# jqsl2012/RL_CTR_Prediction

Measured on NVIDIA B200. Metric: train samples/sec, higher is better.
Workload: dtype f32

## Files before the change

### include/rlctr.h

```cpp
#ifndef RLCTR_H_
#define RLCTR_H_

#include <stddef.h>
#include <stdint.h>

#ifdef __cplusplus
extern "C" {
#endif

#define RLCTR_VERSION 100

#define RLCTR_OK            0
#define RLCTR_EINVAL       (-1)
#define RLCTR_EUNSUPPORTED (-2)
#define RLCTR_EWORKSPACE   (-3)
#define RLCTR_EALIGN       (-4)

typedef struct CUstream_st* rlctr_stream_t;

#define RLCTR_MAX_WORLD 8
typedef struct rlctr_table {
    float*  data;
    int64_t n_rows;
    int32_t row_stride;
// ... 16 lines not shown
    double         beta1, beta2, eps, weight_decay;
    const float*   stage;
} rlctr_adam;

typedef struct rlctr_lookup {
    float*   stage;
    int32_t  world;
    uint32_t n_per_rank;
    float*   gathered[RLCTR_MAX_WORLD];
} rlctr_lookup;

#define RLCTR_STAGED_PARTNER 1
#define RLCTR_DZ_IN_SUMS     2
typedef struct rlctr_rowgrad {
    const float* staged;
    const float* dlogit;
    const float* sums;
    const float* extra;
    int32_t      fields;
    int32_t      flags;
    int32_t      world;
    uint32_t     n_per_rank;
    const float* peer_staged[RLCTR_MAX_WORLD];
    const float* peer_dlogit[RLCTR_MAX_WORLD];
    const float* peer_sums[RLCTR_MAX_WORLD];
    const float* peer_extra[RLCTR_MAX_WORLD];
} rlctr_rowgrad;

int         rlctr_version(void);
unsigned long long rlctr_launch_count(void);
const char* rlctr_strerror(int code);

#define RLCTR_FM_TERM 1
int rlctr_embed_fwd(const int64_t* ids, const rlctr_table* table, const float* bias,
                    float* logit, float* pctr, int64_t pctr_stride, float* sums, float* rows_out,
                    int64_t rows_pitch, int64_t batch, int32_t fields, int32_t flags, rlctr_stream_t stream);

int rlctr_pairdots_fwd(const float* rows, int64_t ld_rows, float* out, int64_t ld_out, int64_t batch,
                       int32_t fields, int32_t dim, int32_t ip_first, rlctr_stream_t stream);
int rlctr_pairdots_bwd(const float* rows, int64_t ld_rows, const float* gout, int64_t ld_g, float* grows,
                       int64_t ld_grows, int64_t batch, int32_t fields, int32_t dim, int32_t ip_first,
                       rlctr_stream_t stream);

size_t rlctr_cross_ws_bytes(int64_t batch, int32_t dim, int32_t layers);
int rlctr_cross_fwd(const float* x0, int64_t ldx, const float* w, const float* b, int32_t layers, float* out, int64_t ld_out,
                    float* s_saved, int64_t batch, int32_t dim, rlctr_stream_t stream);
int rlctr_cross_bwd(const float* x0, int64_t ldx, const float* w, const float* b, const float* s_saved, int32_t layers,
                    const float* gout, int64_t ld_g, float* gx0, int64_t ld_gx, float* dw, float* db, int64_t batch,
                    int32_t dim, void* ws, size_t ws_bytes, rlctr_stream_t stream);

int rlctr_fieldsq_fwd(const float* rows, int64_t ld_rows, float* out, int64_t ld_out, int64_t batch, int32_t fields,
                      int32_t dim, rlctr_stream_t stream);
int rlctr_fieldsq_bwd(const float* rows, int64_t ld_rows, const float* gout, int64_t ld_g, float* grows, int64_t ld_grows,
                      int64_t batch, int32_t fields, int32_t dim, rlctr_stream_t stream);

size_t rlctr_afm_ws_bytes(int64_t batch, int32_t dim);
int rlctr_afm_fwd(const float* rows, int64_t ld_rows, const float* params, float* out, int64_t batch, int32_t fields,
                  int32_t dim, float dropout_p, const uint64_t* rng_state, const float* masks, rlctr_stream_t stream);
int rlctr_afm_bwd(const float* rows, int64_t ld_rows, const float* params, const float* gout, float* grows, int64_t ld_grows,
                  float* dparams, int64_t batch, int32_t fields, int32_t dim, float dropout_p, const uint64_t* rng_state,
                  const float* masks, void* ws, size_t ws_bytes, rlctr_stream_t stream);

int rlctr_gather_rows(const int64_t* ids, int64_t n, const rlctr_table* table, float* out,
                      rlctr_stream_t stream);

int rlctr_ffm_fwd(const int64_t* ids, const rlctr_table* table, const float* bias,
                  float* logit, float* pctr, int64_t pctr_stride, float* partners,
                  int64_t batch, int32_t fields, int32_t latent, rlctr_stream_t stream);

int rlctr_featemb_fwd(const int64_t* ids, const rlctr_table* table, float* out, int64_t out_stride,
                      int64_t batch, int32_t fields, rlctr_stream_t stream);

int rlctr_bn_relu_fwd(const float* x, int64_t ldx, const float* gamma, const float* beta, float* running_mean, float* running_var,
                      float momentum, float eps, float* y, int64_t ldy, float* save_mean, float* save_invstd, int64_t batch,
                      int32_t n, int32_t relu, rlctr_stream_t stream);
int rlctr_bn_relu_bwd(const float* x, int64_t ldx, const float* y, int64_t ldy, const float* gy, int64_t ldg, const float* gamma,
                      const float* save_mean, const float* save_invstd, float* dx, int64_t lddx, float* dgamma, float* dbeta,
                      int64_t batch, int32_t n, int32_t relu, rlctr_stream_t stream);

#define RLCTR_REDUCE_WS_BYTES 16640
int rlctr_bce_fwd_bwd(const float* logit, const int64_t* labels_i64, const float* labels_f32,
                      float* pctr, float* loss, float* dlogit, float* dbias, void* ws, int64_t batch,
                      rlctr_stream_t stream);
int rlctr_sigmoid_bwd(const float* grad_p, const float* pctr, float* dlogit, float* dbias, void* ws,
                      int64_t batch, rlctr_stream_t stream);

size_t rlctr_sort_ws_bytes(int64_t n, int64_t n_rows);
int rlctr_sort_ids(const int64_t* ids, int64_t n, int64_t n_rows,
                   uint32_t* sorted_ids, uint32_t* sorted_slots,
                   void* ws, size_t ws_bytes, rlctr_stream_t stream);

size_t rlctr_rows_ws_bytes(int64_t n);
int rlctr_sort_ids_sharded(const uint32_t* ids_all, int64_t n_all, int32_t world, int32_t rank, int64_t n_rows_global,
                           uint32_t* sorted_rows, uint32_t* sorted_slots, void* ws, size_t ws_bytes,
                           rlctr_stream_t stream);

int rlctr_push_rows(const int64_t* ids, int64_t n, int32_t world, int32_t rank, int64_t n_rows_global, const float* src,
                    int32_t width, void* const* peer_recv, rlctr_stream_t stream);
size_t rlctr_route_ws_bytes(int64_t n, int32_t world);
int rlctr_route_ids(const int64_t* ids, int64_t n, int32_t world, int32_t rank, int64_t n_rows_global, int64_t cap,
                    void* const* peer_keys, void* const* peer_vals, int32_t* overflow, void* ws, size_t ws_bytes,
                    rlctr_stream_t stream);
int rlctr_sort_routed(const uint32_t* keys, const uint32_t* vals, int64_t n_in, int64_t n_rows_local, uint32_t* sorted_rows,
                      uint32_t* sorted_slots, void* ws, size_t ws_bytes, rlctr_stream_t stream);
int rlctr_sort_routed_pos(const uint32_t* keys, int64_t n_in, int64_t n_rows_local, uint32_t* sorted_rows, uint32_t* sorted_pos,
                          void* ws, size_t ws_bytes, rlctr_stream_t stream);
int rlctr_push_rows_routed(const void* route_ws, int64_t n, int32_t world, int32_t rank, int64_t cap, const float* src,
                           int32_t width, void* const* peer_recv, rlctr_stream_t stream);
int rlctr_rows_adam(const uint32_t* sorted_ids, const uint32_t* sorted_slots, int64_t n,
                    const rlctr_rowgrad* grad, const rlctr_table* table, const rlctr_adam* opt,
                    void* ws, size_t ws_bytes, rlctr_stream_t stream);
#define RLCTR_GROUP_MAX 4
typedef struct rlctr_member {
    int32_t      lin_col;
    int32_t      emb_col;
    int32_t      dim;
    int32_t      flags;
    const float* bias;
    float*       logit;
    float*       pctr;
    int64_t      pctr_stride;
    float*       rows_out;
    int64_t      rows_pitch;
    const float* dlogit;
    const float* extra;
} rlctr_member;
int rlctr_group_fwd(const int64_t* ids, const rlctr_table* table, const rlctr_member* members, int32_t n_members,
                    float* sums, int32_t sums_pitch, int64_t batch, int32_t fields, rlctr_stream_t stream);
int rlctr_group_rows_adam(const uint32_t* sorted_ids, const uint32_t* sorted_slots, int64_t n, const rlctr_table* table,
                          const rlctr_adam* opt, const rlctr_member* members, int32_t n_members, const float* sums,
                          int32_t sums_pitch, int32_t fields, int32_t world, const uint32_t* slot_of, void* ws, size_t ws_bytes,
                          rlctr_stream_t stream);

int rlctr_rows_grad_dense(const uint32_t* sorted_ids, const uint32_t* sorted_slots, int64_t n,
                          const rlctr_rowgrad* grad, const rlctr_table* table, float* dense_grad,
                          void* ws, size_t ws_bytes, rlctr_stream_t stream);
int64_t rlctr_lookup_stage_floats(const rlctr_table* table);
int rlctr_rows_lookup(const uint32_t* sorted_ids, const uint32_t* sorted_slots, int64_t n, const rlctr_table* table,
                      const rlctr_adam* opt, const rlctr_lookup* lookup, void* ws, size_t ws_bytes, rlctr_stream_t stream);
int rlctr_rows_catchup(const uint32_t* sorted_ids, int64_t n, const rlctr_table* table,
                       const rlctr_adam* opt, rlctr_stream_t stream);
size_t rlctr_rows_claim_bytes(int64_t n_rows);
int rlctr_rows_catchup_ids(const int64_t* ids, int64_t n, const rlctr_table* table, const rlctr_adam* opt, void* claim,
                           size_t claim_bytes, rlctr_stream_t stream);
int rlctr_adam_flush(const rlctr_table* table, const rlctr_adam* opt,
                     int64_t row_begin, int64_t row_end, rlctr_stream_t stream);
int rlctr_dense_adam(float* param, const float* grad, float* exp_avg, float* exp_avg_sq, int64_t n,
                     const float* sched, const int32_t* step, double beta1, double beta2, double eps,
                     double weight_decay, rlctr_stream_t stream);
#define RLCTR_DENSE_MAX 24
int rlctr_dense_adam_multi(float* const* params, const float* const* grads, float* const* exp_avgs, float* const* exp_avg_sqs,
                           const int64_t* sizes, int32_t count, const float* sched, const int32_t* steps,
                           const int32_t* step_index, double beta1, double beta2, double eps, double weight_decay,
                           rlctr_stream_t stream);
int rlctr_steps_advance(int32_t* steps, const int32_t* step_index, int32_t count, rlctr_stream_t stream);
int rlctr_step_advance(int32_t* step, int32_t delta, rlctr_stream_t stream);

int rlctr_generate_preds(const float* pctr, const float* w, const int64_t* action, const int64_t* label,
                         float* y, float* w_out, float* reward, int64_t batch, int32_t models,
                         int32_t variant, rlctr_stream_t stream);
size_t rlctr_generate_preds_v10_ws_bytes(int64_t batch);
int rlctr_generate_preds_v10(const float* pctr, const float* w, const float* c_actions, const int64_t* action,
                             const int64_t* label, float* y, float* c_out, float* reward, int64_t batch, int32_t models,
                             void* ws, size_t ws_bytes, rlctr_stream_t stream);

int rlctr_reinforce_loss_bwd(const float* logits, const int64_t* act, const float* vt,
                             float* logp, float* loss, float* dlogits, void* ws,
                             int64_t batch, int32_t actions, int32_t variant, rlctr_stream_t stream);

size_t rlctr_auc_ws_bytes(int64_t n);
int rlctr_auc_logloss(const float* pred, const int64_t* labels_i64, const float* labels_f32, int64_t n, float* out,
                      void* ws, size_t ws_bytes, rlctr_stream_t stream);

#define RLCTR_MLP_RELU 1
#define RLCTR_MLP_DROPOUT 2
#define RLCTR_MLP_DX_MASK 4
#define RLCTR_MLP_FP32 8
#define RLCTR_MLP_W_PRESPLIT 16
size_t rlctr_mlp_ws_bytes(int64_t batch, int32_t in_dim, int32_t out_dim);
int rlctr_replay_store(float* memory, int64_t memory_size, int32_t width, int64_t counter, const float* src, int64_t n,
                       int64_t ld_src, rlctr_stream_t stream);
int rlctr_replay_gather(const float* memory, int32_t width, const int64_t* idx, int64_t n, float* out, rlctr_stream_t stream);
int rlctr_replay_update(float* priorities, int32_t ld, const int64_t* idx, const float* td, int64_t n, rlctr_stream_t stream);
int rlctr_replay_sample_uniform(int64_t n_valid, int64_t batch, const uint64_t* rng_state, int64_t* out_idx, rlctr_stream_t stream);
size_t rlctr_replay_per_ws_bytes(int64_t n_valid);
int rlctr_replay_sample_per(const float* priorities, int32_t ld, int64_t n_valid, float eps, float alpha, float beta, int32_t greedy,
                            int64_t batch, const uint64_t* rng_state, int64_t* out_idx, float* out_isw, void* ws, size_t ws_bytes,
                            rlctr_stream_t stream);

size_t rlctr_gae_ws_bytes(int64_t n);
int rlctr_gae_scan(const float* deltas, int64_t n, double gamma_lambda, float* advantages, void* ws, size_t ws_bytes,
                   rlctr_stream_t stream);

int rlctr_rng_advance(uint64_t* rng_state, uint64_t delta, rlctr_stream_t stream);
int rlctr_linear_fwd(const float* x, int64_t ldx, const float* w, const float* bias, float* y, int64_t batch,
                     int32_t in_dim, int32_t out_dim, int32_t flags, float dropout_p, const uint64_t* rng_state,
                     void* ws, size_t ws_bytes, rlctr_stream_t stream);
int rlctr_linear_bwd(const float* x, int64_t ldx, const float* w, const float* y, float* gy, float* dx, float* dw,
                     float* db, int64_t batch, int32_t in_dim, int32_t out_dim, int32_t flags, float gy_scale,
                     float dx_scale, void* ws, size_t ws_bytes, rlctr_stream_t stream);

size_t rlctr_bucket_ws_bytes(int64_t n, int32_t world);
int rlctr_bucket_by_owner(const int64_t* ids, int64_t n, int32_t world, int64_t n_rows, int64_t* send_local,
                          int64_t* pos_of_slot, uint32_t* send_slots, int64_t* bucket_ends, void* ws,
                          size_t ws_bytes, rlctr_stream_t stream);

#ifdef __cplusplus
}
#endif
#endif
```

### rl_ctr_prediction_b200/_lib.py

```python
from __future__ import annotations

import ctypes as C
import os

import torch

_PKG = os.path.dirname(os.path.abspath(__file__))
LIB_PATH = os.path.join(_PKG, "librlctr_sm100a.so")

RLCTR_FM_TERM = 1
RLCTR_STAGED_PARTNER = 1
RLCTR_DZ_IN_SUMS = 2
RLCTR_REDUCE_WS_BYTES = 16640
RLCTR_DENSE_MAX = 24
RLCTR_MLP_RELU = 1
RLCTR_MLP_DROPOUT = 2
RLCTR_MLP_DX_MASK = 4
RLCTR_MLP_W_PRESPLIT = 16
RLCTR_MLP_FP32 = 8


class RlctrError(RuntimeError):
    pass


class Table(C.Structure):
    _fields_ = [("data", C.c_void_p), ("n_rows", C.c_int64), ("row_stride", C.c_int32),
                ("lin_col", C.c_int32), ("emb_col", C.c_int32), ("dim", C.c_int32), ("row_pitch", C.c_int32),
                ("world", C.c_int32), ("peers", C.c_void_p * 8)]


class Adam(C.Structure):
    _fields_ = [("exp_avg", C.c_void_p), ("exp_avg_sq", C.c_void_p), ("stamp", C.c_void_p),
                ("sched", C.c_void_p), ("step", C.c_void_p), ("sched_len", C.c_int32), ("stamp_col", C.c_int32),
                ("beta1", C.c_double), ("beta2", C.c_double), ("eps", C.c_double), ("weight_decay", C.c_double),
                ("stage", C.c_void_p)]


class Lookup(C.Structure):
    _fields_ = [("stage", C.c_void_p), ("world", C.c_int32), ("n_per_rank", C.c_uint32), ("gathered", C.c_void_p * 8)]


class RowGrad(C.Structure):
    _fields_ = [("staged", C.c_void_p), ("dlogit", C.c_void_p), ("sums", C.c_void_p),
                ("extra", C.c_void_p), ("fields", C.c_int32), ("flags", C.c_int32),
                ("world", C.c_int32), ("n_per_rank", C.c_uint32), ("peer_staged", C.c_void_p * 8),
                ("peer_dlogit", C.c_void_p * 8), ("peer_sums", C.c_void_p * 8), ("peer_extra", C.c_void_p * 8)]


class Member(C.Structure):
    _fields_ = [("lin_col", C.c_int32), ("emb_col", C.c_int32), ("dim", C.c_int32), ("flags", C.c_int32),
                ("bias", C.c_void_p), ("logit", C.c_void_p), ("pctr", C.c_void_p), ("pctr_stride", C.c_int64),
                ("rows_out", C.c_void_p), ("rows_pitch", C.c_int64), ("dlogit", C.c_void_p), ("extra", C.c_void_p)]


RLCTR_GROUP_MAX = 4

_P, _I64, _I32, _SZ, _F = C.c_void_p, C.c_int64, C.c_int32, C.c_size_t, C.c_double
_TP, _AP, _GP, _LP = C.POINTER(Table), C.POINTER(Adam), C.POINTER(RowGrad), C.POINTER(Lookup)
_MP = C.POINTER(Member)

SIGNATURES = {
    "rlctr_version": (C.c_int, []),
    "rlctr_strerror": (C.c_char_p, [C.c_int]),
    "rlctr_launch_count": (C.c_ulonglong, []),
    "rlctr_embed_fwd": (C.c_int, [_P, _TP, _P, _P, _P, _I64, _P, _P, _I64, _I64, _I32, _I32, _P]),
    "rlctr_pairdots_fwd": (C.c_int, [_P, _I64, _P, _I64, _I64, _I32, _I32, _I32, _P]),
    "rlctr_pairdots_bwd": (C.c_int, [_P, _I64, _P, _I64, _P, _I64, _I64, _I32, _I32, _I32, _P]),
    "rlctr_cross_ws_bytes": (_SZ, [_I64, _I32, _I32]),
    "rlctr_cross_fwd": (C.c_int, [_P, _I64, _P, _P, _I32, _P, _I64, _P, _I64, _I32, _P]),
    "rlctr_cross_bwd": (C.c_int, [_P, _I64, _P, _P, _P, _I32, _P, _I64, _P, _I64, _P, _P, _I64, _I32, _P, _SZ, _P]),
    "rlctr_fieldsq_fwd": (C.c_int, [_P, _I64, _P, _I64, _I64, _I32, _I32, _P]),
    "rlctr_fieldsq_bwd": (C.c_int, [_P, _I64, _P, _I64, _P, _I64, _I64, _I32, _I32, _P]),
    "rlctr_afm_ws_bytes": (_SZ, [_I64, _I32]),
    "rlctr_afm_fwd": (C.c_int, [_P, _I64, _P, _P, _I64, _I32, _I32, C.c_float, _P, _P, _P]),
    "rlctr_afm_bwd": (C.c_int, [_P, _I64, _P, _P, _P, _I64, _P, _I64, _I32, _I32, C.c_float, _P, _P, _P, _SZ, _P]),
    "rlctr_replay_store": (C.c_int, [_P, _I64, _I32, _I64, _P, _I64, _I64, _P]),
    "rlctr_replay_gather": (C.c_int, [_P, _I32, _P, _I64, _P, _P]),
    "rlctr_replay_update": (C.c_int, [_P, _I32, _P, _P, _I64, _P]),
    "rlctr_replay_sample_uniform": (C.c_int, [_I64, _I64, _P, _P, _P]),
    "rlctr_replay_per_ws_bytes": (_SZ, [_I64]),
    "rlctr_replay_sample_per": (C.c_int, [_P, _I32, _I64, C.c_float, C.c_float, C.c_float, _I32, _I64, _P, _P, _P, _P, _SZ, _P]),
    "rlctr_push_rows": (C.c_int, [_P, _I64, _I32, _I32, _I64, _P, _I32, _P, _P]),
    "rlctr_gae_ws_bytes": (_SZ, [_I64]),
    "rlctr_gae_scan": (C.c_int, [_P, _I64, _F, _P, _P, _SZ, _P]),
    "rlctr_gather_rows": (C.c_int, [_P, _I64, _TP, _P, _P]),
    "rlctr_ffm_fwd": (C.c_int, [_P, _TP, _P, _P, _P, _I64, _P, _I64, _I32, _I32, _P]),
    "rlctr_featemb_fwd": (C.c_int, [_P, _TP, _P, _I64, _I64, _I32, _P]),
    "rlctr_bn_relu_fwd": (C.c_int, [_P, _I64, _P, _P, _P, _P, C.c_float, C.c_float, _P, _I64, _P, _P, _I64, _I32, _I32, _P]),
    "rlctr_bn_relu_bwd": (C.c_int, [_P, _I64, _P, _I64, _P, _I64, _P, _P, _P, _P, _I64, _P, _P, _I64, _I32, _I32, _P]),
    "rlctr_bce_fwd_bwd": (C.c_int, [_P, _P, _P, _P, _P, _P, _P, _P, _I64, _P]),
    "rlctr_sigmoid_bwd": (C.c_int, [_P, _P, _P, _P, _P, _I64, _P]),
    "rlctr_sort_ws_bytes": (_SZ, [_I64, _I64]),
    "rlctr_sort_ids": (C.c_int, [_P, _I64, _I64, _P, _P, _P, _SZ, _P]),
    "rlctr_sort_ids_sharded": (C.c_int, [_P, _I64, _I32, _I32, _I64, _P, _P, _P, _SZ, _P]),
    "rlctr_route_ws_bytes": (_SZ, [_I64, _I32]),
    "rlctr_route_ids": (C.c_int, [_P, _I64, _I32, _I32, _I64, _I64, _P, _P, _P, _P, _SZ, _P]),
    "rlctr_sort_routed": (C.c_int, [_P, _P, _I64, _I64, _P, _P, _P, _SZ, _P]),
    "rlctr_rows_ws_bytes": (_SZ, [_I64]),
    "rlctr_rows_adam": (C.c_int, [_P, _P, _I64, _GP, _TP, _AP, _P, _SZ, _P]),
    "rlctr_group_fwd": (C.c_int, [_P, _TP, _MP, _I32, _P, _I32, _I64, _I32, _P]),
    "rlctr_group_rows_adam": (C.c_int, [_P, _P, _I64, _TP, _AP, _MP, _I32, _P, _I32, _I32, _I32, _P, _P, _SZ, _P]),
    "rlctr_sort_routed_pos": (C.c_int, [_P, _I64, _I64, _P, _P, _P, _SZ, _P]),
    "rlctr_push_rows_routed": (C.c_int, [_P, _I64, _I32, _I32, _I64, _P, _I32, _P, _P]),
    "rlctr_rows_grad_dense": (C.c_int, [_P, _P, _I64, _GP, _TP, _P, _P, _SZ, _P]),
    "rlctr_lookup_stage_floats": (_I64, [_TP]),
    "rlctr_rows_lookup": (C.c_int, [_P, _P, _I64, _TP, _AP, _LP, _P, _SZ, _P]),
    "rlctr_rows_catchup": (C.c_int, [_P, _I64, _TP, _AP, _P]),
    "rlctr_rows_claim_bytes": (_SZ, [_I64]),
    "rlctr_rows_catchup_ids": (C.c_int, [_P, _I64, _TP, _AP, _P, _SZ, _P]),
    "rlctr_adam_flush": (C.c_int, [_TP, _AP, _I64, _I64, _P]),
    "rlctr_dense_adam": (C.c_int, [_P, _P, _P, _P, _I64, _P, _P, _F, _F, _F, _F, _P]),
    "rlctr_dense_adam_multi": (C.c_int, [_P, _P, _P, _P, _P, _I32, _P, _P, _P, _F, _F, _F, _F, _P]),
    "rlctr_steps_advance": (C.c_int, [_P, _P, _I32, _P]),
    "rlctr_step_advance": (C.c_int, [_P, _I32, _P]),
    "rlctr_generate_preds": (C.c_int, [_P, _P, _P, _P, _P, _P, _P, _I64, _I32, _I32, _P]),
    "rlctr_generate_preds_v10_ws_bytes": (_SZ, [_I64]),
    "rlctr_generate_preds_v10": (C.c_int, [_P, _P, _P, _P, _P, _P, _P, _P, _I64, _I32, _P, _SZ, _P]),
    "rlctr_reinforce_loss_bwd": (C.c_int, [_P, _P, _P, _P, _P, _P, _P, _I64, _I32, _I32, _P]),
    "rlctr_auc_ws_bytes": (_SZ, [_I64]),
    "rlctr_auc_logloss": (C.c_int, [_P, _P, _P, _I64, _P, _P, _SZ, _P]),
    "rlctr_mlp_ws_bytes": (_SZ, [_I64, _I32, _I32]),
    "rlctr_rng_advance": (C.c_int, [_P, C.c_uint64, _P]),
    "rlctr_linear_fwd": (C.c_int, [_P, _I64, _P, _P, _P, _I64, _I32, _I32, _I32, C.c_float, _P, _P, _SZ, _P]),
    "rlctr_linear_bwd": (C.c_int, [_P, _I64, _P, _P, _P, _P, _P, _P, _I64, _I32, _I32, _I32, C.c_float, C.c_float, _P, _SZ, _P]),
    "rlctr_bucket_ws_bytes": (_SZ, [_I64, _I32]),
    "rlctr_bucket_by_owner": (C.c_int, [_P, _I64, _I32, _I64, _P, _P, _P, _P, _P, _SZ, _P]),
}

_lib = None


def load() -> C.CDLL:
    global _lib
    if _lib is not None:
        return _lib
    if not os.path.exists(LIB_PATH):
        raise RlctrError(
            f"{LIB_PATH} is missing: build it with `python -m rl_ctr_prediction_b200.build` "
            "(nvcc, sm_100a). There is no fallback path.")
    lib = C.CDLL(LIB_PATH)
    for name, (res, args) in SIGNATURES.items():
        fn = getattr(lib, name)
        fn.restype = res
        fn.argtypes = args
    _lib = lib
    return lib


def check(code: int, what: str) -> None:
    if code != 0:
        msg = load().rlctr_strerror(code).decode()
        raise RlctrError(f"{what} failed: {msg} (code {code})")


def ptr(t):
    if t is None:
        return None
    if not t.is_cuda:
        raise RlctrError("rlctr kernels need CUDA tensors (sm_100a); there is no CPU fallback")
    if not t.is_contiguous():
        raise RlctrError("rlctr kernels need contiguous tensors")
    return t.data_ptr()


def stream():
    return torch.cuda.current_stream().cuda_stream


class KernelTimer:

    def __init__(self):
        self.records = {}

    def add(self, key, e0, e1, meta):
        self.records.setdefault(key, []).append((e0, e1, meta))

    def summary(self, alg_fn=None):
        torch.cuda.synchronize()
        out = {}
        for key, recs in self.records.items():
            ms = [a.elapsed_time(b) for a, b, _ in recs]
            alg = 0.0
            if alg_fn is not None:
                alg = sum(alg_fn(key, m) for _, _, m in recs) / len(recs)
            out[key] = (len(recs), sum(ms) / len(ms), alg)
        return out


_timer = None


def set_timer(t):
    global _timer
    _timer = t


def timing() -> bool:
    return _timer is not None


def call(name, fn, *args, key=None, meta=None):
    t = _timer
    if t is None:
        check(fn(*args), name)
        return
    e0, e1 = torch.cuda.Event(enable_timing=True), torch.cuda.Event(enable_timing=True)
    e0.record()
# ... 5 lines not shown
```

### rl_ctr_prediction_b200/colocated.py

```python
from __future__ import annotations

import ctypes as C
import os

import torch
import torch.nn as nn

from . import _lib
from . import p_model as Model
from .tables import Geometry, round4, table_struct


MEMBER_KINDS = (Model.LR, Model.FM, Model.DeepFM, Model.WideAndDeep, Model.FNN, Model.InnerPNN, Model.OuterPNN, Model.DCN,
                Model.AFM)


UNSORTED_CATCHUP = os.environ.get("RLCTR_GROUP_UNSORTED_CATCHUP", "0") != "0"


class GroupStash:
    __slots__ = ("sorted_ids", "sorted_slots", "n", "fields", "sums", "dlogit", "extra")

    def __init__(self, **kw):
        for k in self.__slots__:
# ... 98 lines not shown
        arr = (_lib.Member * len(self.members))()
        logits, rows = [], []
        for i, (m, (lin, emb, dim)) in enumerate(zip(self.members, self._cols)):
            s = arr[i]
            s.lin_col, s.emb_col, s.dim = lin, emb, dim
            s.flags = _lib.RLCTR_FM_TERM if m._fm_term else 0
            bias = getattr(m, "bias", None)
            s.bias = _lib.ptr(bias.data) if bias is not None else None
            tail = hasattr(m, "_tail")
            table_part = lin >= 0 or bias is not None or m._fm_term
            z = torch.empty(B, dtype=torch.float32, device=dev) if table_part and (train or tail) else None
            logits.append(z)
            s.logit = _lib.ptr(z)
            if pctr is not None and not tail:
                s.pctr, s.pctr_stride = pctr.data_ptr() + 4 * i, pctr.shape[1]
            r = None
            if tail:
                pitch = round4(F * dim)
                r = torch.empty(B, pitch, dtype=torch.float32, device=dev)
                s.rows_out, s.rows_pitch = r.data_ptr(), pitch
            rows.append(r)
        return arr, logits, rows

    @torch.no_grad()
    def forward(self, x):
        lib = _lib.load()
        x = Model._check_ids(x)
        B, F = x.shape
        self.flush()
        out = torch.empty(B, len(self.members), dtype=torch.float32, device=x.device)
        arr, logits, rows = self._member_structs(B, F, x.device, False, pctr=out)
        t = table_struct(self.table.data, self._geom)
        _lib.call("rlctr_group_fwd", lib.rlctr_group_fwd, _lib.ptr(x), C.byref(t), arr, len(self.members), None, 0, B, F,
                  _lib.stream(), key="rlctr_group_fwd[infer]", meta=self._meta(B, F))
        for i, m in enumerate(self.members):
            if rows[i] is not None:
                out[:, i:i + 1] = torch.sigmoid(m._tail(self._z(logits[i], B), rows[i][:, :F * self._cols[i][2]]))
        return out

    @staticmethod
    def _z(logit, B):
        return logit.view(B, 1) if logit is not None else None

    def train_step(self, x, y, optimizer):
        lib = _lib.load()
        opt = self._opt
        if opt is None:
            raise _lib.RlctrError("build rl_ctr_prediction_b200.optim.Adam(group.parameters(), ...) before training the group")
        x = Model._check_ids(x)
        B, F = x.shape
        dev, st, g = x.device, _lib.stream(), self._geom
        yy = y.reshape(-1).contiguous()
        yi = yy if yy.dtype == torch.int64 else None
        yf = None if yi is not None else yy.float()
        t = table_struct(self.table.data, g)
        side = None
        if UNSORTED_CATCHUP and opt.lazy and opt.stamp_col >= 0 and (g.used + 3) // 4 >= 5:
            cur = torch.cuda.current_stream(dev)
            side = self._sort_stream
            if side is None or side.device != dev:
                side = self._sort_stream = torch.cuda.Stream(device=dev)
            side.wait_stream(cur)
            with torch.cuda.stream(side):
                sid, sslot = Model.sort_ids(x, g.n_rows)
            if opt.dirty:
                a = opt.struct()
                cb = lib.rlctr_rows_claim_bytes(g.n_rows)
                if self._claim is None or self._claim.numel() < cb or self._claim.device != dev:
                    self._claim = torch.empty(cb, dtype=torch.uint8, device=dev)
                _lib.call("rlctr_rows_catchup_ids", lib.rlctr_rows_catchup_ids, _lib.ptr(x), x.numel(), C.byref(t), C.byref(a),
                          _lib.ptr(self._claim), cb, st, key="rlctr_rows_catchup[group]", meta=self._meta(B, F))
        else:
            sid, sslot = Model.sort_ids(x, g.n_rows)
            if opt.lazy and opt.dirty:
                a = opt.struct()
                _lib.call("rlctr_rows_catchup", lib.rlctr_rows_catchup, _lib.ptr(sid), x.numel(), C.byref(t), C.byref(a), st,
                          key="rlctr_rows_catchup[group]", meta=self._meta(B, F))
        M = len(self.members)
        arr, logits, rows = self._member_structs(B, F, dev, True)
        sums = torch.empty(B, g.row_stride, dtype=torch.float32, device=dev)
        _lib.call("rlctr_group_fwd", lib.rlctr_group_fwd, _lib.ptr(x), C.byref(t), arr, M, _lib.ptr(sums), 0, B, F, st,
                  key="rlctr_group_fwd[train]", meta=self._meta(B, F))
        losses = torch.empty(M, dtype=torch.float32, device=dev)
        dlogits, extras = [], []
        ws = self._reduce_ws(dev)
        for i, m in enumerate(self.members):
            dl = torch.empty(B, dtype=torch.float32, device=dev)
            dbias = torch.empty(1, dtype=torch.float32, device=dev)
            bias = getattr(m, "bias", None)
            if rows[i] is None:
                _lib.check(lib.rlctr_bce_fwd_bwd(_lib.ptr(logits[i]), _lib.ptr(yi), _lib.ptr(yf), None,
                                                 losses.data_ptr() + 4 * i, _lib.ptr(dl), _lib.ptr(dbias), _lib.ptr(ws), B, st),
                           "rlctr_bce_fwd_bwd")
                extras.append(None)
            else:
                fd = F * self._cols[i][2]
                leaf = rows[i][:, :fd].detach().requires_grad_(True)
                z = m._tail(self._z(logits[i], B), leaf)
                zz = z.detach().reshape(-1).contiguous()
                _lib.check(lib.rlctr_bce_fwd_bwd(_lib.ptr(zz), _lib.ptr(yi), _lib.ptr(yf), None, losses.data_ptr() + 4 * i,
                                                 _lib.ptr(dl), _lib.ptr(dbias) if bias is not None else None, _lib.ptr(ws), B, st),
                           "rlctr_bce_fwd_bwd")
                m.zero_grad()
                z.backward(dl.view_as(z))
                extras.append(leaf.grad.contiguous())
            if bias is not None:
                bias.grad = dbias
            dlogits.append(dl)
        self._stash = GroupStash(sorted_ids=sid, sorted_slots=sslot, n=B * F, fields=F, sums=sums, dlogit=dlogits, extra=extras)
        if side is not None:
            torch.cuda.current_stream(dev).wait_stream(side)
        optimizer.step()
        return losses

    def _group_update(self, stash, opt_state, st):
        lib = _lib.load()
        arr = (_lib.Member * len(self.members))()
        for i, (m, (lin, emb, dim)) in enumerate(zip(self.members, self._cols)):
            s = arr[i]
            s.lin_col, s.emb_col, s.dim = lin, emb, dim
            s.flags = _lib.RLCTR_FM_TERM if m._fm_term else 0
            s.dlogit = _lib.ptr(stash.dlogit[i])
            s.extra = _lib.ptr(stash.extra[i])
        t, a = table_struct(self.table.data, self._geom), opt_state.struct()
        ws_bytes = lib.rlctr_rows_ws_bytes(stash.n)
        ws = self._rows_ws(ws_bytes)
        _lib.call("rlctr_group_rows_adam", lib.rlctr_group_rows_adam, _lib.ptr(stash.sorted_ids), _lib.ptr(stash.sorted_slots),
                  stash.n, C.byref(t), C.byref(a), arr, len(self.members), _lib.ptr(stash.sums), 0, stash.fields, 1, None,
                  _lib.ptr(ws), ws_bytes, st, key="rlctr_group_rows_adam", meta=self._meta(stash.n // stash.fields, stash.fields))


def colocate(models) -> ColocatedCTR:
    return ColocatedCTR(models)
```

### rl_ctr_prediction_b200/csrc/loss.cu

```cuda
#include "common.cuh"

namespace rlctr {

constexpr int RED_MAX_BLOCKS = 1024;
struct RedWs {
    unsigned int* counter;
    float* partial;
};
__host__ __device__ inline RedWs red_ws(void* ws) {
    return RedWs{reinterpret_cast<unsigned int*>(ws), reinterpret_cast<float*>(reinterpret_cast<char*>(ws) + 256)};
}

__device__ __forceinline__ float block_sum_256(float x, float* smem8) {
#pragma unroll
    for (int off = 16; off > 0; off >>= 1) x += __shfl_xor_sync(RLCTR_FULL, x, off);
    __syncthreads();
    if ((threadIdx.x & 31) == 0) smem8[threadIdx.x >> 5] = x;
    __syncthreads();
    float t = 0.f;
    if (threadIdx.x < 8) t = smem8[threadIdx.x];
    if (threadIdx.x < 32) {
#pragma unroll
        for (int off = 4; off > 0; off >>= 1) t += __shfl_xor_sync(RLCTR_FULL, t, off);
    }
    return t;
}

__device__ __forceinline__ bool last_block_arrives(unsigned int* counter) {
    __shared__ bool is_last;
    __threadfence();
    __syncthreads();
    if (threadIdx.x == 0) is_last = (atomicAdd(counter, 1u) == gridDim.x - 1);
    __syncthreads();
    return is_last;
}

__global__ void __launch_bounds__(256)
bce_kernel(const float* __restrict__ logit, const int64_t* __restrict__ yi, const float* __restrict__ yf,
           float* __restrict__ pctr, float* __restrict__ loss, float* __restrict__ dlogit, float* __restrict__ dbias,
           void* ws, int64_t batch) {
    __shared__ float sm[8];
    const float ginv = 1.0f / (float)batch;
    float acc = 0.f, dsum = 0.f;
    for (int64_t b = (int64_t)blockIdx.x * blockDim.x + threadIdx.x; b < batch; b += (int64_t)gridDim.x * blockDim.x) {
        const float z = __ldg(logit + b);
        const float y = yi ? (float)__ldg(yi + b) : __ldg(yf + b);
        const float p = sigmoidf_ref(z);
        acc += (y - 1.0f) * fmaxf(log1pf(-p), -100.0f) - y * fmaxf(logf(p), -100.0f);
        const float dp = ginv * (p - y) / fmaxf((1.0f - p) * p, 1e-12f);
        const float dz = dp * (1.0f - p) * p;
        if (pctr) pctr[b] = p;
        if (dlogit) dlogit[b] = dz;
        dsum += dz;
    }
    RedWs w = red_ws(ws);
    const float bs = block_sum_256(acc, sm), ds = block_sum_256(dsum, sm);
    if (threadIdx.x == 0) { w.partial[blockIdx.x] = bs; w.partial[RED_MAX_BLOCKS + blockIdx.x] = ds; }
    if (last_block_arrives(w.counter)) {
        float t = 0.f, d = 0.f;
        for (int i = threadIdx.x; i < (int)gridDim.x; i += 256) {
            t += __ldcg(w.partial + i);
            d += __ldcg(w.partial + RED_MAX_BLOCKS + i);
        }
        t = block_sum_256(t, sm);
        d = block_sum_256(d, sm);
        if (threadIdx.x == 0) {
            if (loss) loss[0] = t / (float)batch;
            if (dbias) dbias[0] = d;
            *w.counter = 0;
        }
    }
}

__global__ void __launch_bounds__(256)
sigmoid_bwd_kernel(const float* __restrict__ grad_p, const float* __restrict__ pctr, float* __restrict__ dlogit,
                   float* __restrict__ dbias, void* ws, int64_t batch) {
    __shared__ float sm[8];
    float dsum = 0.f;
    for (int64_t b = (int64_t)blockIdx.x * blockDim.x + threadIdx.x; b < batch; b += (int64_t)gridDim.x * blockDim.x) {
        float dz;
        if (grad_p) {
            const float p = __ldg(pctr + b);
            dz = __ldg(grad_p + b) * (1.0f - p) * p;
            dlogit[b] = dz;
        } else {
            dz = dlogit[b];
        }
        dsum += dz;
    }
    if (!dbias) return;
    RedWs w = red_ws(ws);
    const float ds = block_sum_256(dsum, sm);
    if (threadIdx.x == 0) w.partial[blockIdx.x] = ds;
    if (last_block_arrives(w.counter)) {
        float d = 0.f;
        for (int i = threadIdx.x; i < (int)gridDim.x; i += 256) d += __ldcg(w.partial + i);
        d = block_sum_256(d, sm);
        if (threadIdx.x == 0) { dbias[0] = d; *w.counter = 0; }
    }
}

constexpr int GP_MAX = 8;

__global__ void __launch_bounds__(256)
generate_preds_kernel(const float* __restrict__ pctr, const float* __restrict__ w, const int64_t* __restrict__ action,
                      const int64_t* __restrict__ label, float* __restrict__ y, float* __restrict__ w_out,
                      float* __restrict__ reward, int64_t batch, int M, int variant) {
    const int64_t b = (int64_t)blockIdx.x * blockDim.x + threadIdx.x;
    if (b >= batch) return;
    float p[GP_MAX], wt[GP_MAX], ow[GP_MAX], sw[GP_MAX], sp[GP_MAX];
    int si[GP_MAX];
#pragma unroll
    for (int m = 0; m < GP_MAX; ++m) {
        p[m] = m < M ? __ldg(pctr + b * M + m) : 0.f;
        wt[m] = m < M ? __ldg(w + b * M + m) : -INFINITY;
        ow[m] = 0.f;
        sw[m] = wt[m]; sp[m] = p[m]; si[m] = m;
    }
#pragma unroll
    for (int i = 1; i < GP_MAX; ++i) {
#pragma unroll
        for (int j = i; j > 0; --j) {
            if (sw[j] > sw[j - 1]) {
                float tw = sw[j]; sw[j] = sw[j - 1]; sw[j - 1] = tw;
                float tp = sp[j]; sp[j] = sp[j - 1]; sp[j - 1] = tp;
                int ti = si[j]; si[j] = si[j - 1]; si[j - 1] = ti;
            }
        }
    }
    const int k = (int)__ldg(action + b);
    const int lab = (int)__ldg(label + b);
    float psum = 0.f;
#pragma unroll
    for (int m = 0; m < GP_MAX; ++m) if (m < M) psum += p[m];
    const float mean_all = psum / (float)M;
    const int k_lo = variant == 0 ? 2 : 1;
    float yv = 1.0f, rv = 1.0f;
    if (k >= k_lo && k <= M) {
        float base;
        if (k == M) {
            float acc = 0.f;
#pragma unroll
            for (int m = 0; m < GP_MAX; ++m) if (m < M) { acc += wt[m] * p[m]; ow[m] = wt[m]; }
            yv = acc;
            base = mean_all;
        } else if (k == 1) {
            yv = sp[0];
#pragma unroll
            for (int m = 0; m < GP_MAX; ++m) if (si[0] == m) ow[m] = 1.0f;
            base = mean_all;
        } else {
            float e[GP_MAX], esum = 0.f;
#pragma unroll
            for (int j = 0; j < GP_MAX; ++j) { e[j] = j < k ? expf(sw[j] - sw[0]) : 0.f; esum += e[j]; }
// ... 140 lines not shown
            yv = acc;
        }
        const bool good = lab == 1 ? (yv > mean_all) : (yv < mean_all);
        rv = good ? 1.0f : 0.0f;
    }
    y[b] = yv;
    reward[b] = rv;
#pragma unroll
    for (int m = 0; m < GP_MAX; ++m) if (m < M) c_out[b * M + m] = oc[m];
}

constexpr int RF_MAX = 32;

__global__ void __launch_bounds__(256)
reinforce_fwd_kernel(const float* __restrict__ logits, const int64_t* __restrict__ act, const float* __restrict__ vt,
                     float* __restrict__ logp, float* __restrict__ loss, void* ws, int64_t batch, int A, int variant) {
    __shared__ float sm[8];
    float s_nl = 0.f, s_vt = 0.f, s_nlvt = 0.f;
    for (int64_t b = (int64_t)blockIdx.x * blockDim.x + threadIdx.x; b < batch; b += (int64_t)gridDim.x * blockDim.x) {
        const float* z = logits + b * A;
        float mx = -INFINITY;
        for (int a = 0; a < A; ++a) mx = fmaxf(mx, __ldg(z + a));
        float sum = 0.f;
        for (int a = 0; a < A; ++a) sum += expf(__ldg(z + a) - mx);
        const int ai = (int)__ldg(act + b) - 1;
        const float pa = expf(__ldg(z + ai) - mx) / sum;
        const float lp = logf(pa);
        const float v = __ldg(vt + b);
        if (logp) logp[b] = lp;
        s_nl += -lp; s_vt += v; s_nlvt += -lp * v;
    }
    RedWs w = red_ws(ws);
    float r0 = block_sum_256(s_nl, sm), r1 = block_sum_256(s_vt, sm), r2 = block_sum_256(s_nlvt, sm);
    if (threadIdx.x == 0) {
        w.partial[blockIdx.x] = r0;
        w.partial[RED_MAX_BLOCKS + blockIdx.x] = r1;
        w.partial[2 * RED_MAX_BLOCKS + blockIdx.x] = r2;
    }
    if (last_block_arrives(w.counter)) {
        float t0 = 0.f, t1 = 0.f, t2 = 0.f;
        for (int i = threadIdx.x; i < (int)gridDim.x; i += 256) {
            t0 += __ldcg(w.partial + i);
            t1 += __ldcg(w.partial + RED_MAX_BLOCKS + i);
            t2 += __ldcg(w.partial + 2 * RED_MAX_BLOCKS + i);
        }
        t0 = block_sum_256(t0, sm); t1 = block_sum_256(t1, sm); t2 = block_sum_256(t2, sm);
        if (threadIdx.x == 0) {
            const float mean_vt = t1 / (float)batch;
            if (loss) loss[0] = variant == 0 ? t0 * mean_vt : t2 / (float)batch;
            w.partial[3 * RED_MAX_BLOCKS] = mean_vt;
            *w.counter = 0;
        }
    }
}
__global__ void __launch_bounds__(256)
reinforce_bwd_kernel(const float* __restrict__ logits, const int64_t* __restrict__ act, const float* __restrict__ vt,
                     float* __restrict__ dlogits, const void* ws, int64_t batch, int A, int variant) {
    const float mean_vt = __ldcg(reinterpret_cast<const float*>(reinterpret_cast<const char*>(ws) + 256) + 3 * RED_MAX_BLOCKS);
    for (int64_t b = (int64_t)blockIdx.x * blockDim.x + threadIdx.x; b < batch; b += (int64_t)gridDim.x * blockDim.x) {
        const float* z = logits + b * A;
        float mx = -INFINITY;
        for (int a = 0; a < A; ++a) mx = fmaxf(mx, __ldg(z + a));
        float sum = 0.f;
        for (int a = 0; a < A; ++a) sum += expf(__ldg(z + a) - mx);
        const int ai = (int)__ldg(act + b) - 1;
        const float coef = variant == 0 ? mean_vt : __ldg(vt + b) / (float)batch;
        for (int a = 0; a < A; ++a) {
            const float pi = expf(__ldg(z + a) - mx) / sum;
            dlogits[b * A + a] = coef * (pi - (a == ai ? 1.0f : 0.0f));
        }
    }
}

static inline int red_grid(int64_t batch) {
    int64_t blocks = (batch + 255) / 256;
    if (blocks < 1) blocks = 1;
    return (int)(blocks < RED_MAX_BLOCKS ? blocks : RED_MAX_BLOCKS);
}

}

using namespace rlctr;

extern "C" int rlctr_bce_fwd_bwd(const float* logit, const int64_t* labels_i64, const float* labels_f32, float* pctr,
                                 float* loss, float* dlogit, float* dbias, void* ws, int64_t batch,
                                 rlctr_stream_t stream) {
    if (!logit || !ws || batch <= 0) return RLCTR_EINVAL;
    if ((labels_i64 == nullptr) == (labels_f32 == nullptr)) return RLCTR_EINVAL;
    bce_kernel<<<red_grid(batch), 256, 0, (cudaStream_t)stream>>>(logit, labels_i64, labels_f32, pctr, loss, dlogit,
                                                                  dbias, ws, batch);
    RLCTR_LAUNCH_CHECK();
    return RLCTR_OK;
}

extern "C" int rlctr_sigmoid_bwd(const float* grad_p, const float* pctr, float* dlogit, float* dbias, void* ws,
                                 int64_t batch, rlctr_stream_t stream) {
    if (!dlogit || batch <= 0 || (grad_p && !pctr) || (dbias && !ws)) return RLCTR_EINVAL;
    sigmoid_bwd_kernel<<<red_grid(batch), 256, 0, (cudaStream_t)stream>>>(grad_p, pctr, dlogit, dbias, ws, batch);
    RLCTR_LAUNCH_CHECK();
    return RLCTR_OK;
}

extern "C" int rlctr_generate_preds(const float* pctr, const float* w, const int64_t* action, const int64_t* label,
                                    float* y, float* w_out, float* reward, int64_t batch, int32_t models,
                                    int32_t variant, rlctr_stream_t stream) {
    if (!pctr || !w || !action || !label || !y || !reward || batch < 0) return RLCTR_EINVAL;
    if (models < 1 || models > GP_MAX || (variant != 0 && variant != 1)) return RLCTR_EUNSUPPORTED;
    if (batch == 0) return RLCTR_OK;
    generate_preds_kernel<<<(unsigned)((batch + 255) / 256), 256, 0, (cudaStream_t)stream>>>(
        pctr, w, action, label, y, w_out, reward, batch, models, variant);
    RLCTR_LAUNCH_CHECK();
    return RLCTR_OK;
}

extern "C" size_t rlctr_generate_preds_v10_ws_bytes(int64_t batch) {
    if (batch < 0) return 0;
    return (size_t)((batch + GP10_THREADS - 1) / GP10_THREADS + 1) * GP_MAX * sizeof(int);
}
extern "C" int rlctr_generate_preds_v10(const float* pctr, const float* w, const float* c_actions, const int64_t* action,
                                        const int64_t* label, float* y, float* c_out, float* reward, int64_t batch,
                                        int32_t models, void* ws, size_t ws_bytes, rlctr_stream_t stream) {
    if (!pctr || !w || !c_actions || !action || !label || !y || !c_out || !reward || batch < 0) return RLCTR_EINVAL;
    if (models < 1 || models > GP_MAX || batch > ((int64_t)1 << 31)) return RLCTR_EUNSUPPORTED;
    if (batch == 0) return RLCTR_OK;
    if (!ws || ws_bytes < rlctr_generate_preds_v10_ws_bytes(batch)) return RLCTR_EWORKSPACE;
    const int nblocks = (int)((batch + GP10_THREADS - 1) / GP10_THREADS);
    int* counts = reinterpret_cast<int*>(ws);
    cudaStream_t st = (cudaStream_t)stream;
    gp10_count_kernel<<<nblocks, GP10_THREADS, 0, st>>>(action, batch, models, counts);
    gp10_scan_kernel<<<1, GP_MAX * 32, 0, st>>>(counts, nblocks);
    generate_preds_v10_kernel<<<nblocks, GP10_THREADS, 0, st>>>(pctr, w, c_actions, action, label, y, c_out, reward, batch,
                                                                 models, counts);
    RLCTR_LAUNCH_CHECK();
    return RLCTR_OK;
}

extern "C" int rlctr_reinforce_loss_bwd(const float* logits, const int64_t* act, const float* vt, float* logp,
                                        float* loss, float* dlogits, void* ws, int64_t batch, int32_t actions,
                                        int32_t variant, rlctr_stream_t stream) {
    if (!logits || !act || !vt || !ws || batch <= 0) return RLCTR_EINVAL;
    if (actions < 1 || actions > RF_MAX || (variant != 0 && variant != 1)) return RLCTR_EUNSUPPORTED;
    cudaStream_t st = (cudaStream_t)stream;
    reinforce_fwd_kernel<<<red_grid(batch), 256, 0, st>>>(logits, act, vt, logp, loss, ws, batch, actions, variant);
    RLCTR_LAUNCH_CHECK();
    if (dlogits) {
        reinforce_bwd_kernel<<<red_grid(batch), 256, 0, st>>>(logits, act, vt, dlogits, ws, batch, actions, variant);
        RLCTR_LAUNCH_CHECK();
    }
    return RLCTR_OK;
}

unsigned long long g_rlctr_launches = 0;
extern "C" unsigned long long rlctr_launch_count(void) { return __atomic_load_n(&g_rlctr_launches, __ATOMIC_RELAXED); }

extern "C" int rlctr_version(void) { return RLCTR_VERSION; }

extern "C" const char* rlctr_strerror(int code) {
    switch (code) {
        case RLCTR_OK: return "ok";
        case RLCTR_EINVAL: return "invalid argument";
        case RLCTR_EUNSUPPORTED: return "unsupported shape";
        case RLCTR_EWORKSPACE: return "workspace too small";
        case RLCTR_EALIGN: return "pointer not 16-byte aligned";
        default: return code > 0 ? cudaGetErrorString((cudaError_t)code) : "unknown error";
    }
}
// ... 1 lines not shown
```

### rl_ctr_prediction_b200/csrc/mlp.cu

```cuda
#include "common.cuh"
#include "mlp_tma.cuh"

namespace rlctr {

constexpr int GEMM_BM = 128;
constexpr int GEMM_BK = 32;
constexpr int GEMM_UK = 8;
constexpr int GEMM_LOADER_WARPS = 4;
constexpr int GEMM_EPI_WARPS = 4;
constexpr int GEMM_THREADS = 32 * (GEMM_LOADER_WARPS + 1 + GEMM_EPI_WARPS);
constexpr int GEMM_MAX_STAGES = 8;
constexpr int GEMM_TMEM_COLS = 512;

struct GemmArgs {
    const float* A; int64_t sam, sak;
    const float* B; int64_t sbn, sbk;
    int mode_a, mode_b;
    float* C; int64_t ldc;
    int cvec;
    const float* bias;
    int M, N, K;
    int n_tile;
    int m_tiles, n_tiles, splits, kb_per_split;
    int stages;
// ... 295 lines not shown
#pragma unroll
                        for (int j = 0; j < 16; ++j)
                            if (n0 + j < g.N) dst[j] = v[j];
                    }
                }
            }
            tc_fence_before();
            mbar_arrive(smem_u32(&tmem_empty_bar[acc]));
            if (++acc == 2) { acc = 0; acc_phase ^= 1; }
        }
    }
    tc_fence_before();
    __syncthreads();
    if (warp == GEMM_LOADER_WARPS) tmem_dealloc(tmem_base, GEMM_TMEM_COLS);
}

__global__ void __launch_bounds__(256)
splitk_reduce_kernel(const float* __restrict__ part, float* __restrict__ out, int64_t mn, int splits) {
    for (int64_t i = (int64_t)blockIdx.x * blockDim.x + threadIdx.x; i < mn; i += (int64_t)gridDim.x * blockDim.x) {
        float s = 0.f;
        for (int k = 0; k < splits; ++k) s += __ldg(part + (int64_t)k * mn + i);
        out[i] = s;
    }
}

__global__ void __launch_bounds__(256)
splitk_reduce2_kernel(const float* __restrict__ part_a, float* __restrict__ out_a, int64_t n_a, const float* __restrict__ part_b,
                      float* __restrict__ out_b, int64_t n_b, int splits) {
    for (int64_t i = (int64_t)blockIdx.x * blockDim.x + threadIdx.x; i < n_a + n_b; i += (int64_t)gridDim.x * blockDim.x) {
        const bool a = i < n_a;
        const float* src = a ? part_a + i : part_b + (i - n_a);
        const int64_t stride = a ? n_a : n_b;
        float s = 0.f;
        int k = 0;
        for (; k + 8 <= splits; k += 8) {
            float v[8];
#pragma unroll
            for (int u = 0; u < 8; ++u) v[u] = __ldg(src + (int64_t)(k + u) * stride);
#pragma unroll
            for (int u = 0; u < 8; ++u) s += v[u];
        }
        for (; k < splits; ++k) s += __ldg(src + (int64_t)k * stride);
        if (a) out_a[i] = s; else out_b[i - n_a] = s;
    }
}

__global__ void __launch_bounds__(256)
colsum_partial_kernel(const float* __restrict__ Y, int64_t ldy, const float* __restrict__ wt, float* __restrict__ part,
                      int64_t rows, int N, int rows_per_block) {
    __shared__ float red[8][33];
    const int lane = threadIdx.x & 31, w = threadIdx.x >> 5;
    const int n = blockIdx.x * 32 + lane;
    const int64_t r0 = (int64_t)blockIdx.y * rows_per_block;
    const int64_t r1 = r0 + rows_per_block < rows ? r0 + rows_per_block : rows;
    float s = 0.f;
    if (n < N)
#pragma unroll 4
        for (int64_t r = r0 + w; r < r1; r += 8) s += wt ? __ldg(wt + r) * __ldg(Y + r * ldy + n) : __ldg(Y + r * ldy + n);
    red[w][lane] = s;
    __syncthreads();
    if (w == 0) {
        float t = 0.f;
#pragma unroll
        for (int k = 0; k < 8; ++k) t += red[k][lane];
        if (n < N) part[(int64_t)blockIdx.y * N + n] = t;
    }
}

__global__ void __launch_bounds__(256)
relu_bwd_kernel(const float* g, const float* __restrict__ out, float* dy, int64_t n, float scale) {
    for (int64_t i = (int64_t)blockIdx.x * blockDim.x + threadIdx.x; i < n; i += (int64_t)gridDim.x * blockDim.x)
        dy[i] = __ldg(out + i) > 0.f ? g[i] * scale : 0.f;
}
__global__ void __launch_bounds__(256)
mask_rows_kernel(float* __restrict__ dx, const float* __restrict__ x, int64_t ldx, int64_t rows, int K, float scale) {
    const int64_t total = rows * K;
    for (int64_t i = (int64_t)blockIdx.x * blockDim.x + threadIdx.x; i < total; i += (int64_t)gridDim.x * blockDim.x) {
        const int64_t r = i / K;
        const int k = (int)(i - r * K);
        dx[i] = __ldg(x + r * ldx + k) > 0.f ? dx[i] * scale : 0.f;
    }
}
__global__ void __launch_bounds__(256)
dropout_kernel(float* __restrict__ y, int64_t n, const uint64_t* __restrict__ state, uint32_t thresh, float scale) {
    const uint64_t seed = state[0], ctr = state[1];
    for (int64_t i = (int64_t)blockIdx.x * blockDim.x + threadIdx.x; i < n; i += (int64_t)gridDim.x * blockDim.x)
        y[i] = dropout_keep(seed, ctr + (uint64_t)i, thresh) ? y[i] * scale : 0.f;
}
__global__ void rng_advance_kernel(uint64_t* state, uint64_t delta) { state[1] += delta; }

__global__ void __launch_bounds__(256)
gemv_rows_kernel(const float* __restrict__ x, int64_t ldx, const float* __restrict__ w, const float* __restrict__ bias,
                 float* __restrict__ y, int64_t rows, int K, int relu) {
    const int lane = threadIdx.x & 31;
    const int64_t warp0 = (int64_t)blockIdx.x * (blockDim.x >> 5) + (threadIdx.x >> 5);
    const int64_t nwarps = (int64_t)gridDim.x * (blockDim.x >> 5);
    const float b0 = bias ? __ldg(bias) : 0.f;
    for (int64_t r = warp0; r < rows; r += nwarps) {
        float s = 0.f;
        for (int k = lane; k < K; k += 32) s = fmaf(__ldg(x + r * ldx + k), __ldg(w + k), s);
#pragma unroll
        for (int off = 16; off > 0; off >>= 1) s += __shfl_xor_sync(RLCTR_FULL, s, off);
        if (lane == 0) {
            float v = s + b0;
            if (relu) v = fmaxf(v, 0.f);
            y[r] = v;
        }
    }
}
__global__ void __launch_bounds__(256)
gemv_rows4_kernel(const float* __restrict__ x, int64_t ldx, const float* __restrict__ w, const float* __restrict__ bias,
                  float* __restrict__ y, int64_t rows, int K4, int relu) {
    const int lane = threadIdx.x & 31;
    const int64_t warp0 = (int64_t)blockIdx.x * (blockDim.x >> 5) + (threadIdx.x >> 5);
    const int64_t nwarps = (int64_t)gridDim.x * (blockDim.x >> 5);
    const float4 zero = make_float4(0.f, 0.f, 0.f, 0.f);
    const float4* w4 = reinterpret_cast<const float4*>(w);
    const bool on0 = lane < K4, on1 = lane + 32 < K4;
    const float4 w0 = on0 ? __ldg(w4 + lane) : zero, w1 = on1 ? __ldg(w4 + lane + 32) : zero;
    const float b0 = bias ? __ldg(bias) : 0.f;
    for (int64_t r = warp0 * 4; r < rows; r += nwarps * 4) {
        float4 a[4], b[4];
#pragma unroll
        for (int u = 0; u < 4; ++u) {
            const float4* xr = reinterpret_cast<const float4*>(x + (r + u) * ldx);
            const bool ok = r + u < rows;
            a[u] = (ok && on0) ? __ldg(xr + lane) : zero;
            b[u] = (ok && on1) ? __ldg(xr + lane + 32) : zero;
        }
        float s[4];
#pragma unroll
        for (int u = 0; u < 4; ++u) {
            float t = a[u].x * w0.x;
            t = fmaf(a[u].y, w0.y, t); t = fmaf(a[u].z, w0.z, t); t = fmaf(a[u].w, w0.w, t);
            t = fmaf(b[u].x, w1.x, t); t = fmaf(b[u].y, w1.y, t); t = fmaf(b[u].z, w1.z, t); t = fmaf(b[u].w, w1.w, t);
            s[u] = t;
        }
#pragma unroll
        for (int off = 16; off > 0; off >>= 1) {
#pragma unroll
            for (int u = 0; u < 4; ++u) s[u] += __shfl_xor_sync(RLCTR_FULL, s[u], off);
        }
        if (lane < 4 && r + lane < rows) {
            float v = (lane == 0 ? s[0] : lane == 1 ? s[1] : lane == 2 ? s[2] : s[3]) + b0;
            if (relu) v = fmaxf(v, 0.f);
            y[r + lane] = v;
        }
    }
}
__global__ void __launch_bounds__(256)
outer_rows_kernel(const float* __restrict__ gy, const float* __restrict__ w, float* __restrict__ dx, int64_t rows, int K,
                  const float* __restrict__ x, int64_t ldx, float scale) {
    const int64_t total = rows * K;
    for (int64_t i = (int64_t)blockIdx.x * blockDim.x + threadIdx.x; i < total; i += (int64_t)gridDim.x * blockDim.x) {
        const int64_t r = i / K;
        const int k = (int)(i - r * K);
        float v = __ldg(gy + r) * __ldg(w + k);
        if (x) v = __ldg(x + r * ldx + k) > 0.f ? v * scale : 0.f;
        dx[i] = v;
    }
}


template <int CMAX>
__global__ void __launch_bounds__(256)
gemv_bwd_kernel(const float* __restrict__ x, int64_t ldx, const float* __restrict__ gy, const float* __restrict__ w,
                float* __restrict__ dx, float* __restrict__ part, int64_t rows, int K, int rows_per_block, int dx_mask,
                float dx_scale) {
    __shared__ float red[8][CMAX * 32 + 1];
    const int lane = threadIdx.x & 31, wib = threadIdx.x >> 5;
    const int64_t r0 = (int64_t)blockIdx.x * rows_per_block;
    const int64_t r1 = r0 + rows_per_block < rows ? r0 + rows_per_block : rows;
// ... 174 lines not shown
        sgemm_kernel<32, 32><<<grid, 64, 0, st>>>(A, sam, sak, B, sbn, sbk, C, ldc, bias, M, N, K, relu);
    }
    RLCTR_LAUNCH_CHECK();
    return RLCTR_OK;
}
}

static int launch_gemm(const float* A, int64_t sam, int64_t sak, const float* B, int64_t sbn, int64_t sbk, float* C,
                       int64_t ldc, const float* bias, int M, int N, int K, int relu, const GemmPlan& p, cudaStream_t st) {
    GemmArgs g;
    g.A = A; g.sam = sam; g.sak = sak;
    g.B = B; g.sbn = sbn; g.sbk = sbk;
    g.C = C; g.ldc = ldc; g.bias = bias;
    g.M = M; g.N = N; g.K = K;
    g.n_tile = p.n_tile; g.m_tiles = p.m_tiles; g.n_tiles = p.n_tiles; g.splits = p.splits; g.kb_per_split = p.kb_per_split;
    g.stages = p.stages; g.relu = relu;
    g.cvec = vec_of(C, ldc);
    g.mode_a = sak == 1 ? vec_of(A, sam) : 0;
    g.mode_b = sbk == 1 ? vec_of(B, sbn) : 0;
    RLCTR_CUDA(cudaFuncSetAttribute(gemm3x_tf32_kernel, cudaFuncAttributeMaxDynamicSharedMemorySize, (int)p.smem));
    const int total = p.m_tiles * p.n_tiles * p.splits;
    const int grid = total < RLCTR_SMS ? total : RLCTR_SMS;
    gemm3x_tf32_kernel<<<grid, GEMM_THREADS, p.smem, st>>>(g);
    RLCTR_LAUNCH_CHECK();
    return RLCTR_OK;
}

constexpr int COLSUM_ROWS_PER_BLOCK = 128;

static inline size_t align256(size_t b) { return (b + 255) & ~(size_t)255; }
static inline int round4(int n) { return (n + 3) / 4 * 4; }

struct MlpWs {
    size_t wgrad, colsum, wsplit, total;
    int in_pitch;
};
static MlpWs mlp_ws(int64_t batch, int in_dim, int out_dim) {
    MlpWs w;
    const GemmPlan p = plan_gemm(out_dim, in_dim, (int)batch, true);
    int splits = p.splits;
    const int s2 = tma::plan_splits(out_dim, in_dim, (int)batch, true);
    if (s2 > splits) splits = s2;
    w.wgrad = align256((size_t)splits * out_dim * in_dim * sizeof(float));
    const size_t yb = (size_t)((batch + COLSUM_ROWS_PER_BLOCK - 1) / COLSUM_ROWS_PER_BLOCK);
    w.colsum = align256(yb * ((size_t)out_dim + (out_dim == 1 ? (size_t)in_dim : 0)) * sizeof(float));
    w.in_pitch = round4(in_dim);
    w.wsplit = align256((size_t)out_dim * w.in_pitch * sizeof(float));
    w.total = w.wgrad + w.colsum + 2 * w.wsplit + 256;
    return w;
}

}

using namespace rlctr;

extern "C" size_t rlctr_mlp_ws_bytes(int64_t batch, int32_t in_dim, int32_t out_dim) {
    if (batch <= 0 || in_dim <= 0 || out_dim <= 0) return 256;
    return mlp_ws(batch, in_dim, out_dim).total;
}

static bool split_weights_into(void* ws, size_t ws_bytes, const MlpWs& l, const float* w, int in_dim, int out_dim,
                               cudaStream_t st, float** whi, float** wlo, int* rc, bool reuse = false) {
    *rc = RLCTR_OK;
    if (!tma::enabled() || !ws || ws_bytes < l.total || !rlctr_aligned16(ws) || out_dim == 1) return false;
    char* base = reinterpret_cast<char*>(ws) + l.wgrad + l.colsum;
    *whi = reinterpret_cast<float*>(base);
    *wlo = reinterpret_cast<float*>(base + l.wsplit);
    if (!reuse) *rc = tma::split_weight(w, *whi, *wlo, out_dim, in_dim, l.in_pitch, st);
    return *rc == RLCTR_OK;
}

static int grid_elems(int64_t n) {
    int64_t blocks = (n + 255) / 256;
    return (int)(blocks < RLCTR_SMS * 8 ? (blocks < 1 ? 1 : blocks) : RLCTR_SMS * 8);
}

extern "C" int rlctr_rng_advance(uint64_t* state, uint64_t delta, rlctr_stream_t stream) {
    if (!state) return RLCTR_EINVAL;
    rng_advance_kernel<<<1, 1, 0, (cudaStream_t)stream>>>(state, delta);
    RLCTR_LAUNCH_CHECK();
    return RLCTR_OK;
}

extern "C" int rlctr_linear_fwd(const float* x, int64_t ldx, const float* w, const float* bias, float* y, int64_t batch,
                                int32_t in_dim, int32_t out_dim, int32_t flags, float dropout_p, const uint64_t* rng_state,
                                void* ws, size_t ws_bytes, rlctr_stream_t stream) {
    if (!x || !w || !y || batch < 0 || in_dim <= 0 || out_dim <= 0) return RLCTR_EINVAL;
    if (ldx == 0) ldx = in_dim;
    if (ldx < in_dim) return RLCTR_EINVAL;
    const bool drop = (flags & RLCTR_MLP_DROPOUT) != 0 && dropout_p > 0.f;
    if (drop && (!rng_state || !(dropout_p < 1.f))) return RLCTR_EINVAL;
    if (batch == 0) return RLCTR_OK;
    if (batch > 0x7fffffff) return RLCTR_EUNSUPPORTED;
    cudaStream_t st = (cudaStream_t)stream;
    const int relu = (flags & RLCTR_MLP_RELU) ? 1 : 0;
    const uint32_t thresh = dropout_thresh(dropout_p);
    const float dscale = drop ? 1.0f / (1.0f - dropout_p) : 1.f;
    bool fused_drop = false;
    int rc = RLCTR_OK;
    if (out_dim == 1) {
        if (in_dim % 4 == 0 && in_dim <= 256 && ldx % 4 == 0 && ((uintptr_t)x & 15) == 0 && ((uintptr_t)w & 15) == 0) {
            const int64_t blocks = (batch + 31) / 32;
            gemv_rows4_kernel<<<(unsigned)(blocks < RLCTR_SMS * 8 ? blocks : RLCTR_SMS * 8), 256, 0, st>>>(
                x, ldx, w, bias, y, batch, in_dim / 4, relu);
        } else {
            const int64_t blocks = (batch + 7) / 8;
            gemv_rows_kernel<<<(unsigned)(blocks < RLCTR_SMS * 8 ? blocks : RLCTR_SMS * 8), 256, 0, st>>>(
                x, ldx, w, bias, y, batch, in_dim, relu);
        }
        RLCTR_LAUNCH_CHECK();
    } else if (flags & RLCTR_MLP_FP32) {
        rc = simt::gemm(x, ldx, 1, w, in_dim, 1, y, out_dim, bias, (int)batch, out_dim, in_dim, relu, st);
        if (rc) return rc;
    } else {
        const MlpWs l = mlp_ws(batch, in_dim, out_dim);
        float *whi = nullptr, *wlo = nullptr;
        rc = RLCTR_EUNSUPPORTED;
        int src = RLCTR_OK;
        if (split_weights_into(ws, ws_bytes, l, w, in_dim, out_dim, st, &whi, &wlo, &src)) {
            tma::Epilogue epi;
            if (drop) { epi.drop_state = rng_state; epi.drop_thresh = thresh; epi.drop_scale = dscale; }
            rc = tma::gemm(tma::Operand{x, nullptr, ldx, false}, tma::Operand{whi, wlo, l.in_pitch, false}, y, out_dim, bias,
                           (int)batch, out_dim, in_dim, relu, false, st, &epi);
            if (rc == RLCTR_OK) fused_drop = drop;
        } else if (src) {
            return src;
        }
        if (rc == RLCTR_EUNSUPPORTED) {
            GemmPlan p = plan_gemm((int)batch, out_dim, in_dim, false);
            rc = launch_gemm(x, ldx, 1, w, in_dim, 1, y, out_dim, bias, (int)batch, out_dim, in_dim, relu, p, st);
        }
        if (rc) return rc;
    }
    if (drop && !fused_drop) {
        const int64_t n = batch * out_dim;
        dropout_kernel<<<grid_elems(n), 256, 0, st>>>(y, n, rng_state, thresh, dscale);
        RLCTR_LAUNCH_CHECK();
    }
    return RLCTR_OK;
}

extern "C" int rlctr_linear_bwd(const float* x, int64_t ldx, const float* w, const float* y, float* gy, float* dx, float* dw,
                                float* db, int64_t batch, int32_t in_dim, int32_t out_dim, int32_t flags, float gy_scale,
                                float dx_scale, void* ws, size_t ws_bytes, rlctr_stream_t stream) {
    if (!x || !w || !gy || batch <= 0 || in_dim <= 0 || out_dim <= 0) return RLCTR_EINVAL;
    if (ldx == 0) ldx = in_dim;
    if (ldx < in_dim) return RLCTR_EINVAL;
    if (batch > 0x7fffffff) return RLCTR_EUNSUPPORTED;
    if ((flags & RLCTR_MLP_RELU) && !y) return RLCTR_EINVAL;
    cudaStream_t st = (cudaStream_t)stream;
    const float* dy = gy;
    if (flags & RLCTR_MLP_RELU) {
        const int64_t n = batch * out_dim;
        int64_t blocks = (n + 255) / 256;
        int grid = (int)(blocks < RLCTR_SMS * 8 ? blocks : RLCTR_SMS * 8);
        relu_bwd_kernel<<<grid, 256, 0, st>>>(gy, y, gy, n, gy_scale);
        RLCTR_LAUNCH_CHECK();
    }
    const bool dx_mask = (flags & RLCTR_MLP_DX_MASK) != 0;
    const MlpWs l = mlp_ws(batch, in_dim, out_dim);
    if ((dw || db) && (!ws || ws_bytes < l.total)) return RLCTR_EWORKSPACE;
    float* part = reinterpret_cast<float*>(ws);
    float* cpart = ws ? reinterpret_cast<float*>(reinterpret_cast<char*>(ws) + l.wgrad) : nullptr;
    const int yb = (int)((batch + COLSUM_ROWS_PER_BLOCK - 1) / COLSUM_ROWS_PER_BLOCK);
    if (out_dim == 1 && in_dim <= 512) {
        if (!ws || ws_bytes < l.total) return RLCTR_EWORKSPACE;
        if (in_dim <= 256)
            gemv_bwd_kernel<8><<<yb, 256, 0, st>>>(x, ldx, dy, w, dx, cpart, batch, in_dim, COLSUM_ROWS_PER_BLOCK, dx_mask ? 1 : 0,
                                                   dx_scale);
        else
            gemv_bwd_kernel<16><<<yb, 256, 0, st>>>(x, ldx, dy, w, dx, cpart, batch, in_dim, COLSUM_ROWS_PER_BLOCK, dx_mask ? 1 : 0,
                                                    dx_scale);
        RLCTR_LAUNCH_CHECK();
        if (dw || db) {
            colsum_parts_kernel<<<colsum_parts_grid(in_dim + 1), 256, 0, st>>>(cpart, dw, db, in_dim, 1, in_dim + 1, yb);
            RLCTR_LAUNCH_CHECK();
        }
        return RLCTR_OK;
    }
    if (out_dim == 1) {
        if (dx) {
            const int64_t n = batch * in_dim;
            int64_t blocks = (n + 255) / 256;
            outer_rows_kernel<<<(unsigned)(blocks < RLCTR_SMS * 8 ? blocks : RLCTR_SMS * 8), 256, 0, st>>>(
                dy, w, dx, batch, in_dim, dx_mask ? x : nullptr, ldx, dx_scale);
            RLCTR_LAUNCH_CHECK();
        }
        if (dw) {
            dim3 grid((in_dim + 31) / 32, yb);
            colsum_partial_kernel<<<grid, 256, 0, st>>>(x, ldx, dy, cpart, batch, in_dim, COLSUM_ROWS_PER_BLOCK);
            RLCTR_LAUNCH_CHECK();
            colsum_parts_kernel<<<colsum_parts_grid(in_dim), 256, 0, st>>>(cpart, dw, nullptr, in_dim, 0, in_dim, yb);
            RLCTR_LAUNCH_CHECK();
        }
        if (db) {
            float* part2 = cpart + (size_t)yb * in_dim;
            dim3 grid(1, yb);
            colsum_partial_kernel<<<grid, 256, 0, st>>>(dy, 1, nullptr, part2, batch, 1, COLSUM_ROWS_PER_BLOCK);
            RLCTR_LAUNCH_CHECK();
            colsum_parts_kernel<<<1, 256, 0, st>>>(part2, db, nullptr, 1, 0, 1, yb);
            RLCTR_LAUNCH_CHECK();
        }
        return RLCTR_OK;
    }
    const bool fp32 = (flags & RLCTR_MLP_FP32) != 0;
    if (dx && fp32) {
        int rc = simt::gemm(dy, out_dim, 1, w, 1, in_dim, dx, in_dim, nullptr, (int)batch, in_dim, out_dim, 0, st);
        if (rc) return rc;
        if (dx_mask) {
            mask_rows_kernel<<<grid_elems(batch * in_dim), 256, 0, st>>>(dx, x, ldx, batch, in_dim, dx_scale);
            RLCTR_LAUNCH_CHECK();
        }
    } else if (dx) {
        float *whi = nullptr, *wlo = nullptr;
        int rc = RLCTR_OK;
        bool done = false;
        if (split_weights_into(ws, ws_bytes, l, w, in_dim, out_dim, st, &whi, &wlo, &rc, (flags & RLCTR_MLP_W_PRESPLIT) != 0)) {
            tma::Epilogue epi;
            if (dx_mask) { epi.mask_src = x; epi.mask_ld = ldx; epi.mask_scale = dx_scale; }
            rc = tma::gemm(tma::Operand{dy, nullptr, out_dim, false}, tma::Operand{whi, wlo, l.in_pitch, true}, dx, in_dim,
                           nullptr, (int)batch, in_dim, out_dim, 0, false, st, &epi);
            if (rc == RLCTR_OK) done = true;
            else if (rc != RLCTR_EUNSUPPORTED) return rc;
        } else if (rc) {
            return rc;
        }
        if (!done) {
            GemmPlan p = plan_gemm((int)batch, in_dim, out_dim, false);
            rc = launch_gemm(dy, out_dim, 1, w, 1, in_dim, dx, in_dim, nullptr, (int)batch, in_dim, out_dim, 0, p, st);
            if (rc) return rc;
            if (dx_mask) {
                mask_rows_kernel<<<grid_elems(batch * in_dim), 256, 0, st>>>(dx, x, ldx, batch, in_dim, dx_scale);
                RLCTR_LAUNCH_CHECK();
            }
        }
    }
    bool db_done = false;
    const float* dbp_pending = nullptr;
    if (dw && fp32) {
        int rc = simt::gemm(dy, 1, out_dim, x, 1, ldx, dw, in_dim, nullptr, out_dim, in_dim, (int)batch, 0, st);
        if (rc) return rc;
    } else if (dw) {
        const int64_t mn = (int64_t)out_dim * in_dim;
        int splits = tma::enabled() ? tma::plan_splits(out_dim, in_dim, (int)batch, true) : 0;
        int rc = RLCTR_EUNSUPPORTED;
        if (splits >= 1) {
            float* dbp = (db && (size_t)splits * out_dim * sizeof(float) <= l.colsum) ? cpart : nullptr;
            rc = tma::gemm(tma::Operand{dy, nullptr, out_dim, true}, tma::Operand{x, nullptr, ldx, true}, splits == 1 ? dw : part,
                           in_dim, nullptr, out_dim, in_dim, (int)batch, 0, true, st, nullptr, dbp);
            if (rc == RLCTR_OK && dbp) {
                if (splits > 1) {
                    dbp_pending = dbp;
                } else {
                    splitk_reduce_kernel<<<(out_dim + 255) / 256, 256, 0, st>>>(dbp, db, out_dim, splits);
                    RLCTR_LAUNCH_CHECK();
                }
                db_done = true;
            }
        }
        if (rc == RLCTR_EUNSUPPORTED) {
            GemmPlan p = plan_gemm(out_dim, in_dim, (int)batch, true);
            splits = p.splits;
            rc = launch_gemm(dy, 1, out_dim, x, 1, ldx, splits == 1 ? dw : part, in_dim, nullptr, out_dim, in_dim, (int)batch,
                             0, p, st);
        }
        if (rc) return rc;
        if (splits > 1 && dbp_pending) {
            int64_t blocks = (mn + out_dim + 255) / 256;
            splitk_reduce2_kernel<<<(unsigned)(blocks < 1184 ? blocks : 1184), 256, 0, st>>>(part, dw, mn, dbp_pending, db, out_dim, splits);
            RLCTR_LAUNCH_CHECK();
        } else if (splits > 1) {
            int64_t blocks = (mn + 255) / 256;
            splitk_reduce_kernel<<<(unsigned)(blocks < 1184 ? blocks : 1184), 256, 0, st>>>(part, dw, mn, splits);
            RLCTR_LAUNCH_CHECK();
        }
    }
    if (db && !db_done) {
        dim3 grid((out_dim + 31) / 32, yb);
        colsum_partial_kernel<<<grid, 256, 0, st>>>(dy, out_dim, nullptr, cpart, batch, out_dim, COLSUM_ROWS_PER_BLOCK);
        RLCTR_LAUNCH_CHECK();
        colsum_parts_kernel<<<colsum_parts_grid(out_dim), 256, 0, st>>>(cpart, db, nullptr, out_dim, 0, out_dim, yb);
        RLCTR_LAUNCH_CHECK();
    }
    return RLCTR_OK;
}
```

### rl_ctr_prediction_b200/csrc/mlp_tma.cu

```cuda
#include <cuda.h>
#include <stdio.h>
#include <stdlib.h>

#include "common.cuh"
#include "mlp_tma.cuh"

namespace rlctr {
namespace tma {

constexpr int BM = 128;
constexpr int BK = 32;
constexpr int UK = 8;
constexpr int CONV_WARPS = 4;
constexpr int EPI_WARPS = 4;
constexpr int PRODUCER_WARP = CONV_WARPS;
constexpr int MMA_WARP = CONV_WARPS + 1;
constexpr int THREADS = 32 * (CONV_WARPS + 2 + EPI_WARPS);
constexpr int MAX_STAGES = 8;
constexpr int TMEM_COLS = 512;
constexpr uint32_t A_TILE_BYTES = BM * 128;
constexpr int BIAS_SMEM = 1024;

struct Args {
    float* C; int64_t ldc;
    int cvec;
    const float* bias;
    int M, N, K;
    int n_tile, m_tiles, n_tiles, splits, kb_per_split, stages;
    int a_mn, b_mn;
    int b_presplit;
    int relu;
    int a_tmem;
    int acc_stride, a_col0;
    int pair;
    int cluster;
    int l2_ahead;
    int c_tma;
    int m_tma;
    long long* dbg;
    float* colsum_part;
    Epilogue epi;
};

__device__ __forceinline__ uint32_t smem_u32(const void* p) { return (uint32_t)__cvta_generic_to_shared(p); }
__device__ __forceinline__ void mbar_init(uint32_t bar, uint32_t count) {
    asm volatile("mbarrier.init.shared::cta.b64 [%0], %1;" ::"r"(bar), "r"(count));
}
__device__ __forceinline__ void mbar_arrive(uint32_t bar) {
    asm volatile("mbarrier.arrive.shared::cta.b64 _, [%0];" ::"r"(bar) : "memory");
}
__device__ __forceinline__ void mbar_expect_tx(uint32_t bar, uint32_t bytes) {
    asm volatile("mbarrier.arrive.expect_tx.shared::cta.b64 _, [%0], %1;" ::"r"(bar), "r"(bytes) : "memory");
}
__device__ __forceinline__ bool mbar_try(uint32_t bar, uint32_t parity) {
    uint32_t ok;
    asm volatile(
        "{\n\t.reg .pred p;\n\t"
        "mbarrier.try_wait.parity.shared::cta.b64 p, [%1], %2;\n\t"
        "selp.u32 %0, 1, 0, p;\n\t}"
        : "=r"(ok) : "r"(bar), "r"(parity) : "memory");
    return ok != 0;
}
__device__ __noinline__ void mbar_timeout(uint32_t bar, uint32_t parity) {
    printf("rlctr gemm3x_tma_kernel: mbarrier wait timed out (block %d thread %d bar 0x%x parity %u)\n", (int)blockIdx.x,
           (int)threadIdx.x, bar, parity);
    __trap();
}
__device__ __forceinline__ void mbar_wait(uint32_t bar, uint32_t parity) {
    if (mbar_try(bar, parity)) return;
    uint64_t t0 = 0;
    uint32_t spins = 0;
    while (!mbar_try(bar, parity)) {
        if ((++spins & 0x3fffu) == 0) {
            uint64_t now;
            asm volatile("mov.u64 %0, %%globaltimer;" : "=l"(now));
            if (t0 == 0) t0 = now;
            else if (now - t0 > 4000000000ull) mbar_timeout(bar, parity);
        }
    }
}
__device__ __forceinline__ void fence_proxy_async() { asm volatile("fence.proxy.async.shared::cta;" ::: "memory"); }
__device__ __forceinline__ void fence_barrier_init() { asm volatile("fence.mbarrier_init.release.cluster;" ::: "memory"); }
__device__ __forceinline__ void tc_fence_before() { asm volatile("tcgen05.fence::before_thread_sync;" ::: "memory"); }
__device__ __forceinline__ void tc_fence_after() { asm volatile("tcgen05.fence::after_thread_sync;" ::: "memory"); }
__device__ __forceinline__ void tmem_alloc(uint32_t dst_smem, uint32_t cols) {
    asm volatile("tcgen05.alloc.cta_group::1.sync.aligned.shared::cta.b32 [%0], %1;" ::"r"(dst_smem), "r"(cols) : "memory");
    asm volatile("tcgen05.relinquish_alloc_permit.cta_group::1.sync.aligned;" ::: "memory");
}
__device__ __forceinline__ void tmem_dealloc(uint32_t taddr, uint32_t cols) {
    asm volatile("tcgen05.dealloc.cta_group::1.sync.aligned.b32 %0, %1;" ::"r"(taddr), "r"(cols) : "memory");
}
__device__ __forceinline__ void umma_tf32(uint32_t tmem_d, uint64_t adesc, uint64_t bdesc, uint32_t idesc, uint32_t accumulate) {
    asm volatile(
        "{\n\t.reg .pred p;\n\t"
        "setp.ne.b32 p, %4, 0;\n\t"
        "tcgen05.mma.cta_group::1.kind::tf32 [%0], %1, %2, %3, p;\n\t}" ::"r"(tmem_d), "l"(adesc), "l"(bdesc), "r"(idesc),
        "r"(accumulate) : "memory");
}
__device__ __forceinline__ void umma_tf32_ts(uint32_t tmem_d, uint32_t tmem_a, uint64_t bdesc, uint32_t idesc, uint32_t accumulate) {
    asm volatile(
        "{\n\t.reg .pred p;\n\t"
        "setp.ne.b32 p, %4, 0;\n\t"
        "tcgen05.mma.cta_group::1.kind::tf32 [%0], [%1], %2, %3, p;\n\t}" ::"r"(tmem_d), "r"(tmem_a), "l"(bdesc), "r"(idesc),
        "r"(accumulate) : "memory");
}
__device__ __forceinline__ void tmem_st32(uint32_t taddr, const uint32_t* r) {
    asm volatile(
        "tcgen05.st.sync.aligned.32x32b.x32.b32 [%0], {%1,%2,%3,%4,%5,%6,%7,%8,%9,%10,%11,%12,%13,%14,%15,%16,"
        "%17,%18,%19,%20,%21,%22,%23,%24,%25,%26,%27,%28,%29,%30,%31,%32};" ::"r"(taddr),
        "r"(r[0]), "r"(r[1]), "r"(r[2]), "r"(r[3]), "r"(r[4]), "r"(r[5]), "r"(r[6]), "r"(r[7]), "r"(r[8]), "r"(r[9]), "r"(r[10]),
        "r"(r[11]), "r"(r[12]), "r"(r[13]), "r"(r[14]), "r"(r[15]), "r"(r[16]), "r"(r[17]), "r"(r[18]), "r"(r[19]), "r"(r[20]),
        "r"(r[21]), "r"(r[22]), "r"(r[23]), "r"(r[24]), "r"(r[25]), "r"(r[26]), "r"(r[27]), "r"(r[28]), "r"(r[29]), "r"(r[30]),
        "r"(r[31]) : "memory");
}
__device__ __forceinline__ void tmem_st_wait() { asm volatile("tcgen05.wait::st.sync.aligned;" ::: "memory"); }
__device__ __forceinline__ float lds32(uint32_t a) {
    float v;
    asm volatile("ld.shared.f32 %0, [%1];" : "=f"(v) : "r"(a) : "memory");
    return v;
}
__device__ __forceinline__ void umma_commit(uint32_t bar) {
// ... 100 lines not shown
}
__device__ __forceinline__ uint32_t cluster_ctarank() {
    uint32_t r;
    asm volatile("mov.u32 %0, %%cluster_ctarank;" : "=r"(r));
    return r;
}
__device__ __forceinline__ void cluster_sync_all() {
    asm volatile("barrier.cluster.arrive.release.aligned;" ::: "memory");
    asm volatile("barrier.cluster.wait.acquire.aligned;" ::: "memory");
}
__device__ __forceinline__ void tma_prefetch_desc(const CUtensorMap* map) {
    asm volatile("prefetch.tensormap [%0];" ::"l"(reinterpret_cast<uint64_t>(map)) : "memory");
}

__device__ __forceinline__ uint64_t desc_k_major(uint32_t saddr) {
    uint64_t d = 0;
    d |= (uint64_t)((saddr & 0x3FFFF) >> 4);
    d |= (uint64_t)(1024 >> 4) << 32;
    d |= (uint64_t)1 << 46;
    d |= (uint64_t)2 << 61;
    return d;
}
__device__ __forceinline__ uint64_t desc_mn_major(uint32_t saddr) {
    uint64_t d = 0;
    d |= (uint64_t)((saddr & 0x3FFFF) >> 4);
    d |= (uint64_t)(4096 >> 4) << 16;
    d |= (uint64_t)(512 >> 4) << 32;
    d |= (uint64_t)1 << 46;
    d |= (uint64_t)1 << 61;
    return d;
}

__device__ __forceinline__ float tf32_rn(float x) {
    return __uint_as_float((__float_as_uint(x) + 0x1000u) & 0xFFFFE000u);
}
__device__ __forceinline__ float4 lds128(uint32_t a) {
    float4 v;
    asm volatile("ld.shared.v4.f32 {%0,%1,%2,%3}, [%4];" : "=f"(v.x), "=f"(v.y), "=f"(v.z), "=f"(v.w) : "r"(a) : "memory");
    return v;
}
__device__ __forceinline__ void sts128(uint32_t a, const float4& v) {
    asm volatile("st.shared.v4.f32 [%0], {%1,%2,%3,%4};" ::"r"(a), "f"(v.x), "f"(v.y), "f"(v.z), "f"(v.w) : "memory");
}
__device__ __forceinline__ void split4(const float4& x, float4& h, float4& l) {
    h = make_float4(tf32_rn(x.x), tf32_rn(x.y), tf32_rn(x.z), tf32_rn(x.w));
    l = make_float4(x.x - h.x, x.y - h.y, x.z - h.z, x.w - h.w);
}
__device__ __forceinline__ void split_tile(uint32_t hi, uint32_t lo, int bytes, int tid) {
    constexpr int STEP = CONV_WARPS * 32 * 16;
    for (int off = tid * 16; off < bytes; off += 2 * STEP) {
        const bool two = off + STEP < bytes;
        const float4 x0 = lds128(hi + off);
        float4 x1 = make_float4(0.f, 0.f, 0.f, 0.f);
        if (two) x1 = lds128(hi + off + STEP);
        float4 h, l;
        split4(x0, h, l);
        sts128(hi + off, h);
        sts128(lo + off, l);
        if (two) {
            split4(x1, h, l);
            sts128(hi + off + STEP, h);
            sts128(lo + off + STEP, l);
        }
    }
}

__device__ __forceinline__ void split_tile_colsum(uint32_t hi, uint32_t lo, int tid, float4 (&acc)[BM / 32]) {
    constexpr int STEP = CONV_WARPS * 32 * 16;
#pragma unroll
    for (int j = 0; j < BM / 32; ++j) {
        const int off = tid * 16 + j * 4096;
        const float4 x0 = lds128(hi + off), x1 = lds128(hi + off + STEP);
        float4 h, l;
        split4(x0, h, l);
        sts128(hi + off, h);
        sts128(lo + off, l);
        split4(x1, h, l);
        sts128(hi + off + STEP, h);
        sts128(lo + off + STEP, l);
        acc[j].x += x0.x + x1.x; acc[j].y += x0.y + x1.y; acc[j].z += x0.z + x1.z; acc[j].w += x0.w + x1.w;
    }
}

__device__ __forceinline__ float split_row_to_tmem(uint32_t raw, bool a_mn, int t, uint32_t taddr) {
    uint32_t hi[BK], lo[BK];
    float sum = 0.f;
    if (!a_mn) {
        const uint32_t row = raw + (uint32_t)t * 128u;
#pragma unroll
        for (int c = 0; c < BK / 4; ++c) {
            const float4 x = lds128(row + (uint32_t)((c ^ (t & 7)) << 4));
            float4 h, l;
            split4(x, h, l);
            hi[4 * c] = __float_as_uint(h.x); hi[4 * c + 1] = __float_as_uint(h.y);
            hi[4 * c + 2] = __float_as_uint(h.z); hi[4 * c + 3] = __float_as_uint(h.w);
            lo[4 * c] = __float_as_uint(l.x); lo[4 * c + 1] = __float_as_uint(l.y);
            lo[4 * c + 2] = __float_as_uint(l.z); lo[4 * c + 3] = __float_as_uint(l.w);
        }
    } else {
        const int mm = t & 31;
        const uint32_t blk = raw + (uint32_t)(t >> 5) * 4096u + (uint32_t)((mm & 7) << 2);
#pragma unroll
        for (int k = 0; k < BK; ++k) {
            const float x = lds32(blk + (uint32_t)k * 128u + (uint32_t)((((mm >> 3) ^ (k & 3))) << 5));
            const float h = tf32_rn(x);
            hi[k] = __float_as_uint(h);
            lo[k] = __float_as_uint(x - h);
            sum += x;
        }
    }
    tmem_st32(taddr, hi);
    tmem_st32(taddr + (uint32_t)BK, lo);
    tmem_st_wait();
    return sum;
}

#define DBG_STAMP(it, slot)                                                                         \
    do {                                                                                           \
        if (g.dbg && blockIdx.x == 0 && (it) < 256) g.dbg[(it) * 16 + (slot)] = clock64();          \
    } while (0)

struct TileWalk {
    int tile, kb0, kb1, mt, nt, split;
};
__device__ __forceinline__ bool tile_decode(TileWalk& w, const Args& g, int total_tiles, int rank = 0) {
    if (w.tile >= total_tiles) return false;
    const int mtc = (g.m_tiles + g.cluster - 1) / g.cluster;
    const int mn = mtc * g.n_tiles;
    w.split = w.tile / mn;
    const int r = w.tile - w.split * mn;
    w.mt = r / g.n_tiles;
    w.nt = r - w.mt * g.n_tiles;
    w.mt = w.mt * g.cluster + rank;
    const int kb_total = (g.K + BK - 1) / BK;
    w.kb0 = w.split * g.kb_per_split;
    w.kb1 = min(w.kb0 + g.kb_per_split, kb_total);
    return true;
}


struct EpiCtx {
    float* crow;
    const float* bias;
    const float* sbias;
    int N, cvec;
    bool row_ok, relu, zero;
    bool drop;
    uint64_t drop_seed, drop_base;
    uint32_t drop_thresh;
    float drop_scale;
    const float* mask_row;
    int mvec;
    float mask_scale;
    uint32_t mbuf;
};
template <int W>
__device__ __forceinline__ void epilogue_compute(const EpiCtx& e, const uint32_t* r, int n0, float (&v)[W]) {
#pragma unroll
    for (int j = 0; j < W; ++j) v[j] = e.zero ? 0.f : __uint_as_float(r[j]);
    if (e.sbias) {
#pragma unroll
        for (int j = 0; j < W; j += 4) {
            const float4 b = *reinterpret_cast<const float4*>(e.sbias + n0 + j);
            v[j] += b.x; v[j + 1] += b.y; v[j + 2] += b.z; v[j + 3] += b.w;
        }
    } else if (e.bias) {
#pragma unroll
        for (int j = 0; j < W; ++j)
            if (n0 + j < e.N) v[j] += __ldg(e.bias + n0 + j);
    }
    if (e.relu) {
#pragma unroll
        for (int j = 0; j < W; ++j) v[j] = fmaxf(v[j], 0.f);
    }
    if (e.drop) {
        const uint64_t i0 = e.drop_base + (uint64_t)n0;
        const uint64_t p0 = i0 >> 1, p1 = (i0 + (uint64_t)(W - 1)) >> 1;
        if (!(i0 & 1) && (p0 >> 32) == (p1 >> 32)) {
            const uint32_t key = dropout_key(e.drop_seed, (uint32_t)(p0 >> 32)), lo = (uint32_t)p0;
#pragma unroll
            for (int j = 0; j < W; j += 2) {
                const uint32_t h = dropout_bits(key, lo + (uint32_t)(j >> 1));
                v[j] = (h & 0xffffu) >= e.drop_thresh ? v[j] * e.drop_scale : 0.f;
                v[j + 1] = (h >> 16) >= e.drop_thresh ? v[j + 1] * e.drop_scale : 0.f;
            }
        } else {
#pragma unroll
            for (int j = 0; j < W; ++j)
                v[j] = dropout_keep(e.drop_seed, i0 + (uint64_t)j, e.drop_thresh) ? v[j] * e.drop_scale : 0.f;
        }
    }
    if (e.mask_row && e.row_ok && !(W == 32 && e.mbuf)) {
        const float* mr = e.mask_row + n0;
        if (n0 + W <= e.N && e.mvec == 4) {
#pragma unroll
            for (int j = 0; j < W; j += 4) {
                const float4 x = __ldg(reinterpret_cast<const float4*>(mr + j));
                v[j] = x.x > 0.f ? v[j] * e.mask_scale : 0.f;
                v[j + 1] = x.y > 0.f ? v[j + 1] * e.mask_scale : 0.f;
                v[j + 2] = x.z > 0.f ? v[j + 2] * e.mask_scale : 0.f;
                v[j + 3] = x.w > 0.f ? v[j + 3] * e.mask_scale : 0.f;
            }
        } else {
#pragma unroll
            for (int j = 0; j < W; ++j)
                if (n0 + j < e.N) v[j] = __ldg(mr + j) > 0.f ? v[j] * e.mask_scale : 0.f;
        }
    }
}
template <int W>
__device__ __forceinline__ void epilogue_emit(const EpiCtx& e, const uint32_t* r, int n0) {
    if (!e.row_ok || n0 >= e.N) return;
    float v[W];
    epilogue_compute<W>(e, r, n0, v);
    float* dst = e.crow + n0;
    if (n0 + W <= e.N && e.cvec == 4) {
#pragma unroll
        for (int j = 0; j < W; j += 4) *reinterpret_cast<float4*>(dst + j) = make_float4(v[j], v[j + 1], v[j + 2], v[j + 3]);
    } else if (n0 + W <= e.N && e.cvec == 2) {
#pragma unroll
        for (int j = 0; j < W; j += 2) *reinterpret_cast<float2*>(dst + j) = make_float2(v[j], v[j + 1]);
    } else {
#pragma unroll
        for (int j = 0; j < W; ++j)
            if (n0 + j < e.N) dst[j] = v[j];
    }
}
template <bool MASK>
__device__ __forceinline__ void epilogue_stage(const EpiCtx& e, const uint32_t* r, int n0, uint32_t buf, int lane) {
    float v[32];
    epilogue_compute<32>(e, r, n0, v);
    const uint32_t row = buf + (uint32_t)lane * 128u;
    if (MASK && e.mbuf) {
        const uint32_t mrow = e.mbuf + (uint32_t)lane * 128u;
#pragma unroll
        for (int c = 0; c < 8; ++c) {
            const uint32_t off = (uint32_t)((c ^ (lane & 7)) << 4);
            const float4 x = lds128(mrow + off);
            sts128(row + off, make_float4(x.x > 0.f ? v[4 * c] * e.mask_scale : 0.f, x.y > 0.f ? v[4 * c + 1] * e.mask_scale : 0.f,
                                          x.z > 0.f ? v[4 * c + 2] * e.mask_scale : 0.f, x.w > 0.f ? v[4 * c + 3] * e.mask_scale : 0.f));
        }
        return;
    }
#pragma unroll
    for (int c = 0; c < 8; ++c)
        sts128(row + (uint32_t)((c ^ (lane & 7)) << 4), make_float4(v[4 * c], v[4 * c + 1], v[4 * c + 2], v[4 * c + 3]));
}
template <int W>
__device__ __forceinline__ void epilogue_tile(const EpiCtx& e, uint32_t taddr, int n_base, int n_tile) {
    uint32_t ra[W], rb[W];
    const int nch = n_tile / W;
    tmem_ld<W>(taddr, ra);
    for (int c = 0; c < nch; c += 2) {
        tmem_ld_fence<W>(ra);
        if (c + 1 < nch) tmem_ld<W>(taddr + (uint32_t)((c + 1) * W), rb);
        epilogue_emit<W>(e, ra, n_base + c * W);
        if (c + 1 < nch) {
            tmem_ld_fence<W>(rb);
            if (c + 2 < nch) tmem_ld<W>(taddr + (uint32_t)((c + 2) * W), ra);
            epilogue_emit<W>(e, rb, n_base + (c + 1) * W);
        }
    }
}

template <bool MASK>
__device__ __forceinline__ void epilogue_chunk_tma(const EpiCtx& e, const uint32_t* r, int n0, const CUtensorMap* mapC,
                                                   uint32_t stage0, int& buf, int m0, int lane) {
    if (n0 >= e.N) return;
    if (lane == 0) bulk_wait_read<1>();
    __syncwarp();
    const uint32_t sb = stage0 + (uint32_t)buf * 4096u;
    epilogue_stage<MASK>(e, r, n0, sb, lane);
    fence_proxy_async();
    __syncwarp();
    if (lane == 0) { tma_store_2d(mapC, sb, n0, m0); bulk_commit(); }
    buf ^= 1;
}
__device__ __forceinline__ void mask_request(const CUtensorMap* mapM, uint32_t mbuf, uint32_t mbar, int n0, int m0, int lane) {
    if (lane == 0) {
        mbar_expect_tx(mbar, 4096u);
        tma_load_2d(mbuf, mapM, n0, m0, mbar);
    }
}
template <bool MASK>
__device__ __forceinline__ void epilogue_tile_tma(const EpiCtx& e, uint32_t taddr, int n_base, int n_tile, const CUtensorMap* mapC,
                                                  uint32_t stage0, int& buf, int m0, int lane, const CUtensorMap* mapM,
                                                  uint32_t mbar, uint32_t& mphase) {
    const int nch = n_tile / 32;
    for (int c = 0; c < nch; ++c) {
        uint32_t ra[32];
        tmem_ld<32>(taddr + (uint32_t)(c * 32), ra);
        tmem_ld_fence<32>(ra);
        const int n0 = n_base + c * 32;
        if (MASK && e.mbuf && n0 < e.N) {
            mbar_wait(mbar, mphase);
            mphase ^= 1;
        }
        epilogue_chunk_tma<MASK>(e, ra, n0, mapC, stage0, buf, m0, lane);
        if (MASK && e.mbuf && c + 1 < nch && n0 + 32 < e.N) mask_request(mapM, e.mbuf, mbar, n0 + 32, m0, lane);
    }
    if (n_tile & 31) {
        uint32_t rt[16];
        tmem_ld<16>(taddr + (uint32_t)(nch * 32), rt);
        tmem_ld_fence<16>(rt);
        epilogue_emit<16>(e, rt, n_base + nch * 32);
    }
}

template <bool PAIR, bool MASK>
__global__ void __launch_bounds__(THREADS, 1)
gemm3x_tma_kernel(const __grid_constant__ CUtensorMap mapA, const __grid_constant__ CUtensorMap mapB,
                  const __grid_constant__ CUtensorMap mapBlo, const __grid_constant__ CUtensorMap mapC,
                  const __grid_constant__ CUtensorMap mapM, const Args g) {
    extern __shared__ __align__(1024) unsigned char smem_raw[];
    __shared__ __align__(8) uint64_t raw_bar[MAX_STAGES], full_bar[MAX_STAGES], empty_bar[MAX_STAGES];
    __shared__ __align__(8) uint64_t tmem_full_bar[2], tmem_empty_bar[2];
    __shared__ __align__(8) uint64_t mask_bar[EPI_WARPS];
    __shared__ uint32_t tmem_base_smem;
    __shared__ __align__(16) float s_bias[BIAS_SMEM];

    unsigned char* smem = reinterpret_cast<unsigned char*>((reinterpret_cast<uintptr_t>(smem_raw) + 1023) & ~(uintptr_t)1023);
    const int warp = threadIdx.x >> 5, lane = threadIdx.x & 31;
    const bool bias_in_smem = g.bias != nullptr && g.n_tiles * g.n_tile <= BIAS_SMEM;
    if (bias_in_smem)
        for (int i = threadIdx.x; i < g.n_tiles * g.n_tile; i += THREADS) s_bias[i] = i < g.N ? __ldg(g.bias + i) : 0.f;
    const uint32_t b_bytes = (uint32_t)g.n_tile * (PAIR ? 64u : 128u);
    const uint32_t a_bytes = g.a_tmem ? A_TILE_BYTES : 2 * A_TILE_BYTES;
    const uint32_t stage_bytes = a_bytes + 2 * b_bytes;
    const int rank = g.cluster > 1 ? (int)cluster_ctarank() : 0;
    const int cluster_id = (int)blockIdx.x / g.cluster, n_clusters = (int)gridDim.x / g.cluster;
    const int total_tiles = ((g.m_tiles + g.cluster - 1) / g.cluster) * g.n_tiles * g.splits;
    const uint16_t cmask = (uint16_t)((1u << g.cluster) - 1u);

    if (threadIdx.x == 0) {
        for (int s = 0; s < g.stages; ++s) {
            mbar_init(smem_u32(&raw_bar[s]), 1);
            mbar_init(smem_u32(&full_bar[s]), (uint32_t)(CONV_WARPS * 32 * (PAIR ? 2 : 1)));
            mbar_init(smem_u32(&empty_bar[s]), (uint32_t)(PAIR ? 1 : g.cluster));
        }
        for (int s = 0; s < EPI_WARPS; ++s) mbar_init(smem_u32(&mask_bar[s]), 1);
        for (int s = 0; s < 2; ++s) {
            mbar_init(smem_u32(&tmem_full_bar[s]), 1);
            mbar_init(smem_u32(&tmem_empty_bar[s]), (uint32_t)(EPI_WARPS * 32 * (PAIR ? 2 : 1)));
        }
        fence_barrier_init();
    }
    if (warp == PRODUCER_WARP && lane == 0) {
        tma_prefetch_desc(&mapA);
        tma_prefetch_desc(&mapB);
        if (g.b_presplit) tma_prefetch_desc(&mapBlo);
        if (g.c_tma) tma_prefetch_desc(&mapC);
        if (g.m_tma) tma_prefetch_desc(&mapM);
    }
    if (warp == MMA_WARP) {
        if (PAIR) tmem_alloc2(smem_u32(&tmem_base_smem), TMEM_COLS);
        else tmem_alloc(smem_u32(&tmem_base_smem), TMEM_COLS);
    }
    tc_fence_before();
    __syncthreads();
    if (g.cluster > 1) cluster_sync_all();
    tc_fence_after();
    const uint32_t tmem_base = tmem_base_smem;
    if (g.dbg && threadIdx.x == 0) {
        uint64_t now; uint32_t sm;
        asm volatile("mov.u64 %0, %%globaltimer;" : "=l"(now));
        asm volatile("mov.u32 %0, %%smid;" : "=r"(sm));
        g.dbg[4096 + 4 * blockIdx.x] = (long long)now;
        g.dbg[4096 + 4 * blockIdx.x + 2] = (long long)sm;
    }

    if (warp < CONV_WARPS) {
        const int tid = threadIdx.x;
        int stage = 0, dbg_it = 0;
        uint32_t phase = 0;
        TileWalk w{cluster_id, 0, 0, 0, 0, 0};
        const bool colsum = g.colsum_part != nullptr && g.a_mn;
        for (; tile_decode(w, g, total_tiles, rank); w.tile += n_clusters) {
            const bool sum_tile = colsum && w.nt == 0;
            float4 acc[BM / 32];
#pragma unroll
            for (int j = 0; j < BM / 32; ++j) acc[j] = make_float4(0.f, 0.f, 0.f, 0.f);
            float row_sum = 0.f;
            for (int kb = w.kb0; kb < w.kb1; ++kb) {
                mbar_wait(smem_u32(&raw_bar[stage]), phase);
                if (tid == 0) DBG_STAMP(dbg_it, 1);
                if (tid == 96) DBG_STAMP(dbg_it, 12);
                const uint32_t st = smem_u32(smem + (size_t)stage * stage_bytes);
                if (g.a_tmem) {
                    tc_fence_after();
                    const uint32_t ta = tmem_base + ((uint32_t)(warp * 32) << 16) + (uint32_t)(g.a_col0 + stage * 2 * BK);
                    row_sum += split_row_to_tmem(st, g.a_mn != 0, tid, ta);
                    if (!g.b_presplit) split_tile(st + a_bytes, st + a_bytes + b_bytes, b_bytes, tid);
                    tc_fence_before();
                } else {
                    if (sum_tile) split_tile_colsum(st, st + A_TILE_BYTES, tid, acc);
                    else split_tile(st, st + A_TILE_BYTES, A_TILE_BYTES, tid);
                    if (!g.b_presplit) split_tile(st + a_bytes, st + a_bytes + b_bytes, b_bytes, tid);
                }
                if (!(g.a_tmem && g.b_presplit)) fence_proxy_async();
                if (tid == 0) DBG_STAMP(dbg_it, 2);
                if (tid == 96) DBG_STAMP(dbg_it, 11);
                ++dbg_it;
                if (PAIR && rank != 0) mbar_arrive_remote(smem_u32(&full_bar[stage]), 0);
                else mbar_arrive(smem_u32(&full_bar[stage]));
                if (++stage == g.stages) { stage = 0; phase ^= 1; }
            }
            if (sum_tile && g.a_tmem) {
                const int m = w.mt * BM + tid;
                if (m < g.M) g.colsum_part[(int64_t)w.split * g.M + m] = row_sum;
            } else if (sum_tile) {
                const int r = (tid >> 3) & 3, half = tid & 1, lc = ((tid & 7) >> 1) ^ r, wq = tid >> 5;
#pragma unroll
                for (int step = 1; step <= 2; step <<= 1) {
                    const int rp = r ^ step;
                    const int src = rp * 8 + (((lc ^ rp) << 1) | half);
#pragma unroll
                    for (int j = 0; j < BM / 32; ++j) {
                        acc[j].x += __shfl_sync(RLCTR_FULL, acc[j].x, src);
                        acc[j].y += __shfl_sync(RLCTR_FULL, acc[j].y, src);
                        acc[j].z += __shfl_sync(RLCTR_FULL, acc[j].z, src);
                        acc[j].w += __shfl_sync(RLCTR_FULL, acc[j].w, src);
                    }
                }
                asm volatile("bar.sync 1, %0;" ::"n"(CONV_WARPS * 32) : "memory");
                if (r == 0) {
#pragma unroll
                    for (int j = 0; j < BM / 32; ++j)
                        *reinterpret_cast<float4*>(&s_bias[wq * BM + j * 32 + lc * 8 + half * 4]) = acc[j];
                }
                asm volatile("bar.sync 1, %0;" ::"n"(CONV_WARPS * 32) : "memory");
                const int m = w.mt * BM + tid;
                if (m < g.M) g.colsum_part[(int64_t)w.split * g.M + m] = s_bias[tid] + s_bias[BM + tid] + s_bias[2 * BM + tid] + s_bias[3 * BM + tid];
            }
        }
    } else if (warp == PRODUCER_WARP) {
        int stage = 0;
        uint32_t phase = 0;
        const uint32_t tx = A_TILE_BYTES + (g.b_presplit ? 2 * b_bytes : b_bytes);
        int dbg_it = 0;
        TileWalk pw{cluster_id, 0, 0, 0, 0, 0};
        bool pw_ok = g.l2_ahead > 0 && tile_decode(pw, g, total_tiles, rank);
        int pkb = pw.kb0;
        auto prefetch_next = [&]() {
            if (!pw_ok) return;
            if (pkb < pw.kb1) {
                const int pm0 = pw.mt * BM, pk0 = pkb * BK;
                if (g.a_mn) { for (int j = 0; j < BM / 32; ++j) tma_prefetch_l2_2d(&mapA, pm0 + 32 * j, pk0); }
                else tma_prefetch_l2_2d(&mapA, pk0, pm0);
            }
            if (++pkb >= pw.kb1) {
                pw.tile += n_clusters;
                pw_ok = tile_decode(pw, g, total_tiles, rank);
                pkb = pw.kb0;
            }
        };
        if (lane == 0)
            for (int i = 0; i < g.l2_ahead; ++i) prefetch_next();
        TileWalk w{cluster_id, 0, 0, 0, 0, 0};
        for (; tile_decode(w, g, total_tiles, rank); w.tile += n_clusters) {
            const int m0 = w.mt * BM, n0 = w.nt * g.n_tile;
            for (int kb = w.kb0; kb < w.kb1; ++kb) {
                if (lane == 0) prefetch_next();
                mbar_wait(smem_u32(&empty_bar[stage]), phase ^ 1);
                if (lane == 0) {
                    DBG_STAMP(dbg_it, 0);
                    const uint32_t bar = smem_u32(&raw_bar[stage]);
                    const uint32_t sa = smem_u32(smem + (size_t)stage * stage_bytes);
                    const uint32_t sb = sa + a_bytes;
                    const int k0 = kb * BK;
                    mbar_expect_tx(bar, tx);
                    if (g.a_mn) {
                        for (int j = 0; j < BM / 32; ++j) tma_load_2d(sa + j * 4096, &mapA, m0 + 32 * j, k0, bar);
                    } else {
                        tma_load_2d(sa, &mapA, k0, m0, bar);
// ... 42 lines not shown
        TileWalk w{cluster_id, 0, 0, 0, 0, 0};
        if (PAIR && rank != 0) w.tile = total_tiles;
        for (; tile_decode(w, g, total_tiles, rank); w.tile += n_clusters) {
            if (lane == 0) DBG_STAMP(dbg_it, 5);
            if (PAIR) mbar_wait_cluster(smem_u32(&tmem_empty_bar[acc]), acc_phase ^ 1);
            else mbar_wait(smem_u32(&tmem_empty_bar[acc]), acc_phase ^ 1);
            if (lane == 0) DBG_STAMP(dbg_it, 6);
            tc_fence_after();
            const uint32_t d_tmem = tmem_base + (uint32_t)(acc * g.acc_stride);
            for (int kb = w.kb0; kb < w.kb1; ++kb) {
                mbar_wait(smem_u32(&raw_bar[stage]), phase);
                if (lane == 0) DBG_STAMP(dbg_it, 8);
                if (PAIR) mbar_wait_cluster(smem_u32(&full_bar[stage]), phase);
                else mbar_wait(smem_u32(&full_bar[stage]), phase);
                if (lane == 0) DBG_STAMP(dbg_it, 9);
                tc_fence_after();
                if (lane == 0) DBG_STAMP(dbg_it, 3);
                if (lane == 0) {
                    const uint32_t sa = smem_u32(smem + (size_t)stage * stage_bytes);
                    const uint32_t a_hi = sa, a_lo = sa + A_TILE_BYTES, b_hi = sa + a_bytes, b_lo = b_hi + b_bytes;
                    const int ksteps = min(BK / UK, (g.K - kb * BK + UK - 1) / UK);
                    if (g.a_tmem) {
                        const uint32_t ta_hi = tmem_base + (uint32_t)(g.a_col0 + stage * 2 * BK), ta_lo = ta_hi + (uint32_t)BK;
#pragma unroll
                        for (int k = 0; k < BK / UK; ++k) {
                            if (k >= ksteps) break;
                            const uint32_t bo = (uint32_t)k * b_step;
                            const uint64_t dbh = g.b_mn ? desc_mn_major(b_hi + bo) : desc_k_major(b_hi + bo);
                            const uint64_t dbl = g.b_mn ? desc_mn_major(b_lo + bo) : desc_k_major(b_lo + bo);
                            const uint32_t first = (kb > w.kb0 || k > 0) ? 1u : 0u;
                            if (PAIR) {
                                umma_tf32_ts2(d_tmem, ta_lo + (uint32_t)(k * UK), dbh, idesc, first);
                                umma_tf32_ts2(d_tmem, ta_hi + (uint32_t)(k * UK), dbl, idesc, 1u);
                                umma_tf32_ts2(d_tmem, ta_hi + (uint32_t)(k * UK), dbh, idesc, 1u);
                            } else {
                                umma_tf32_ts(d_tmem, ta_lo + (uint32_t)(k * UK), dbh, idesc, first);
                                umma_tf32_ts(d_tmem, ta_hi + (uint32_t)(k * UK), dbl, idesc, 1u);
                                umma_tf32_ts(d_tmem, ta_hi + (uint32_t)(k * UK), dbh, idesc, 1u);
                            }
                        }
                    } else
#pragma unroll
                    for (int k = 0; k < BK / UK; ++k) {
                        if (k >= ksteps) break;
                        const uint32_t ao = (uint32_t)k * a_step, bo = (uint32_t)k * b_step;
                        const uint64_t dah = g.a_mn ? desc_mn_major(a_hi + ao) : desc_k_major(a_hi + ao);
                        const uint64_t dal = g.a_mn ? desc_mn_major(a_lo + ao) : desc_k_major(a_lo + ao);
                        const uint64_t dbh = g.b_mn ? desc_mn_major(b_hi + bo) : desc_k_major(b_hi + bo);
                        const uint64_t dbl = g.b_mn ? desc_mn_major(b_lo + bo) : desc_k_major(b_lo + bo);
                        const uint32_t first = (kb > w.kb0 || k > 0) ? 1u : 0u;
                        umma_tf32(d_tmem, dal, dbh, idesc, first);
                        umma_tf32(d_tmem, dah, dbl, idesc, 1u);
                        umma_tf32(d_tmem, dah, dbh, idesc, 1u);
                    }
                    DBG_STAMP(dbg_it, 10);
                    if (PAIR) {
                        umma_commit2_mc(smem_u32(&empty_bar[stage]), cmask);
                        if (kb == w.kb1 - 1) umma_commit2_mc(smem_u32(&tmem_full_bar[acc]), cmask);
                    } else {
                        if (g.cluster > 1) umma_commit_mc(smem_u32(&empty_bar[stage]), cmask);
                        else umma_commit(smem_u32(&empty_bar[stage]));
                        if (kb == w.kb1 - 1) umma_commit(smem_u32(&tmem_full_bar[acc]));
                    }
                    DBG_STAMP(dbg_it, 4);
                }
                ++dbg_it;
                __syncwarp();
                if (++stage == g.stages) { stage = 0; phase ^= 1; }
            }
            if (w.kb1 <= w.kb0 && lane == 0) {
                if (PAIR) umma_commit2_mc(smem_u32(&tmem_full_bar[acc]), cmask);
                else umma_commit(smem_u32(&tmem_full_bar[acc]));
            }
            __syncwarp();
            if (++acc == 2) { acc = 0; acc_phase ^= 1; }
        }
    } else {
        const int q = warp & 3;
        uint64_t drop_seed = 0, drop_ctr = 0;
        if (g.epi.drop_state) { drop_seed = g.epi.drop_state[0]; drop_ctr = g.epi.drop_state[1]; }
        int acc = 0, dbg_tile = 0, cbuf = 0;
        const uint32_t cstage = smem_u32(smem + (size_t)g.stages * stage_bytes) + (uint32_t)q * 8192u;
        uint32_t acc_phase = 0;
        uint32_t mphase = 0;
        TileWalk w{cluster_id, 0, 0, 0, 0, 0};
        for (; tile_decode(w, g, total_tiles, rank); w.tile += n_clusters) {
            const bool empty_split = w.kb1 <= w.kb0;
            const uint32_t mbuf = (MASK && g.m_tma) ? cstage + (uint32_t)((EPI_WARPS - q) * 8192 + q * 4096) : 0u;
            if (MASK && mbuf && w.nt * g.n_tile < g.N && g.n_tile >= 32)
                mask_request(&mapM, mbuf, smem_u32(&mask_bar[q]), w.nt * g.n_tile, w.mt * BM + q * 32, lane);
            mbar_wait(smem_u32(&tmem_full_bar[acc]), acc_phase);
            tc_fence_after();
            if (warp == CONV_WARPS + 2 && lane == 0) DBG_STAMP(dbg_tile * (w.kb1 - w.kb0), 7);
            const int m = w.mt * BM + q * 32 + lane;
            EpiCtx e;
            e.crow = g.C + ((int64_t)w.split * g.M + m) * g.ldc;
            e.row_ok = m < g.M;
            e.N = g.N;
            e.cvec = g.cvec;
            e.relu = (g.splits == 1) && g.relu;
            e.bias = (g.splits == 1) ? g.bias : nullptr;
            e.sbias = (g.splits == 1 && g.bias && bias_in_smem) ? s_bias : nullptr;
            e.zero = empty_split;
            e.drop = g.epi.drop_state != nullptr && g.splits == 1;
            e.drop_seed = drop_seed;
            e.drop_base = drop_ctr + (uint64_t)m * (uint64_t)g.N;
            e.drop_thresh = g.epi.drop_thresh;
            e.drop_scale = g.epi.drop_scale;
            e.mask_row = (g.epi.mask_src && g.splits == 1) ? g.epi.mask_src + (int64_t)m * g.epi.mask_ld : nullptr;
            e.mvec = g.epi.mvec;
            e.mask_scale = g.epi.mask_scale;
            e.mbuf = mbuf;
            const uint32_t taddr = tmem_base + (uint32_t)(acc * g.acc_stride) + ((uint32_t)(q * 32) << 16);
            if (g.c_tma) epilogue_tile_tma<MASK>(e, taddr, w.nt * g.n_tile, g.n_tile, &mapC, cstage, cbuf, w.mt * BM + q * 32, lane, &mapM,
                                           smem_u32(&mask_bar[q]), mphase);
            else if (g.n_tile % 32 == 0) epilogue_tile<32>(e, taddr, w.nt * g.n_tile, g.n_tile);
            else epilogue_tile<16>(e, taddr, w.nt * g.n_tile, g.n_tile);
            tc_fence_before();
            if (warp == CONV_WARPS + 2 && lane == 0) DBG_STAMP(dbg_tile * (w.kb1 - w.kb0) + 1, 7);
            ++dbg_tile;
            if (PAIR && rank != 0) mbar_arrive_remote(smem_u32(&tmem_empty_bar[acc]), 0);
            else mbar_arrive(smem_u32(&tmem_empty_bar[acc]));
            if (++acc == 2) { acc = 0; acc_phase ^= 1; }
        }
        if (g.c_tma && lane == 0) bulk_wait_read<0>();
    }
    tc_fence_before();
    __syncthreads();
    if (g.dbg && threadIdx.x == 0) {
        uint64_t now;
        asm volatile("mov.u64 %0, %%globaltimer;" : "=l"(now));
        g.dbg[4096 + 4 * blockIdx.x + 1] = (long long)now;
    }
    if (g.cluster > 1) cluster_sync_all();
    if (warp == MMA_WARP) {
        if (PAIR) tmem_dealloc2(tmem_base, TMEM_COLS);
        else tmem_dealloc(tmem_base, TMEM_COLS);
    }
}

__global__ void __launch_bounds__(256)
split_weight_kernel(const float* __restrict__ w, float* __restrict__ hi, float* __restrict__ lo, int rows, int cols, int pitch) {
    const int64_t total = (int64_t)rows * pitch;
    for (int64_t i = (int64_t)blockIdx.x * blockDim.x + threadIdx.x; i < total; i += (int64_t)gridDim.x * blockDim.x) {
        const int r = (int)(i / pitch), c = (int)(i - (int64_t)r * pitch);
        const float x = c < cols ? __ldg(w + (int64_t)r * cols + c) : 0.f;
        const float h = tf32_rn(x);
        hi[i] = h;
        lo[i] = x - h;
    }
}

typedef CUresult (*EncodeTiledFn)(CUtensorMap*, CUtensorMapDataType, cuuint32_t, void*, const cuuint64_t*, const cuuint64_t*,
                                  const cuuint32_t*, const cuuint32_t*, CUtensorMapInterleave, CUtensorMapSwizzle,
                                  CUtensorMapL2promotion, CUtensorMapFloatOOBfill);
static EncodeTiledFn encode_fn() {
    static EncodeTiledFn fn = nullptr;
    static bool tried = false;
    if (!tried) {
        tried = true;
        void* p = nullptr;
        cudaDriverEntryPointQueryResult q;
        if (cudaGetDriverEntryPoint("cuTensorMapEncodeTiled", &p, cudaEnableDefault, &q) == cudaSuccess &&
            q == cudaDriverEntryPointSuccess)
            fn = reinterpret_cast<EncodeTiledFn>(p);
    }
    return fn;
}
static bool make_map(CUtensorMap* map, const float* ptr, int64_t dim0, int64_t dim1, int64_t pitch, int box1,
                     bool mn_major = false) {
    EncodeTiledFn fn = encode_fn();
    if (!fn) return false;
    cuuint64_t dims[2] = {(cuuint64_t)dim0, (cuuint64_t)dim1};
    cuuint64_t strides[1] = {(cuuint64_t)pitch * sizeof(float)};
    cuuint32_t box[2] = {32u, (cuuint32_t)box1};
    cuuint32_t estr[2] = {1u, 1u};
    CUresult r = fn(map, CU_TENSOR_MAP_DATA_TYPE_FLOAT32, 2, const_cast<float*>(ptr), dims, strides, box, estr,
                    CU_TENSOR_MAP_INTERLEAVE_NONE, mn_major ? CU_TENSOR_MAP_SWIZZLE_128B_ATOM_32B : CU_TENSOR_MAP_SWIZZLE_128B,
                    CU_TENSOR_MAP_L2_PROMOTION_L2_128B,
                    CU_TENSOR_MAP_FLOAT_OOB_FILL_NONE);
    return r == CUDA_SUCCESS;
}
static bool tma_ok(const float* p, int64_t pitch) { return p && (((uintptr_t)p) & 15u) == 0 && pitch % 4 == 0 && pitch > 0; }

static int env_int(const char* name, int dflt) {
    const char* s = getenv(name);
    return s && *s ? atoi(s) : dflt;
}
int enabled() {
    return env_int("RLCTR_GEMM_TMA", 1) != 0 && encode_fn() != nullptr;
}

static int round_to(int n, int q) { return (n + q - 1) / q * q; }

struct Plan {
    int n_tile, n_tiles, m_tiles, splits, kb_per_split, stages;
    int a_tmem, acc_stride, a_col0, c_tma, cluster, pair;
    size_t smem;
};
constexpr size_t C_STAGE_BYTES = (size_t)EPI_WARPS * 2 * 4096;
constexpr size_t M_STAGE_BYTES = (size_t)EPI_WARPS * 4096;
static Plan make_plan(int M, int N, int K, bool b_mn, bool allow_split, bool c_tma_ok = false, bool b_presplit = false) {
    Plan p;
    const int nt_max = env_int("RLCTR_GEMM_NT_MAX", 160);
    const int q = b_mn ? 32 : 16;
    p.n_tiles = (N + nt_max - 1) / nt_max;
    p.n_tile = round_to((N + p.n_tiles - 1) / p.n_tiles, q);
    if (p.n_tile > 256) { p.n_tile = 256; p.n_tiles = (N + 255) / 256; }
    p.m_tiles = (M + BM - 1) / BM;
    const int kb_total = (K + BK - 1) / BK;
    p.splits = 1;
    if (allow_split) {
        const int tiles = p.m_tiles * p.n_tiles;
        int s = RLCTR_SMS / (tiles > 0 ? tiles : 1);
        if (s < 1) s = 1;
        int max_s = kb_total / 8;
        if (max_s < 1) max_s = 1;
        p.splits = s < max_s ? s : max_s;
    }
    p.kb_per_split = (kb_total + p.splits - 1) / p.splits;
    if (p.kb_per_split < 1) p.kb_per_split = 1;
    p.splits = (kb_total + p.kb_per_split - 1) / p.kb_per_split;
    if (p.splits < 1) p.splits = 1;
    p.acc_stride = round_to(p.n_tile, 32);
    p.a_col0 = 2 * p.acc_stride;
    const int tmem_stages = (TMEM_COLS - p.a_col0) / (2 * BK);
    p.a_tmem = (env_int("RLCTR_GEMM_A_TMEM", 1) != 0 && tmem_stages >= 2) ? 1 : 0;
    if (!p.a_tmem) { p.acc_stride = 256; p.a_col0 = 0; }
    p.pair = (env_int("RLCTR_GEMM_PAIR", 0) != 0 && p.a_tmem && b_presplit && !b_mn && p.splits == 1 && p.m_tiles >= 2 &&
              p.n_tile % 32 == 0) ? 1 : 0;
    const size_t stage_bytes = (p.a_tmem ? 1 : 2) * (size_t)A_TILE_BYTES + 2 * (size_t)p.n_tile * (p.pair ? 64 : 128);
    int st = (int)((size_t)(220 * 1024) / stage_bytes);
    if (st > MAX_STAGES) st = MAX_STAGES;
    if (p.a_tmem && st > tmem_stages) st = tmem_stages;
    if (st < 1) st = 1;
    p.stages = st;
    p.c_tma = (c_tma_ok && p.splits == 1 && env_int("RLCTR_GEMM_C_TMA", 1) != 0 &&
               stage_bytes * st + C_STAGE_BYTES <= (size_t)(220 * 1024)) ? 1 : 0;
    p.smem = stage_bytes * st + (p.c_tma ? C_STAGE_BYTES : 0) + 1024;
    p.cluster = p.pair ? 2 : 1;
    if (!p.pair && env_int("RLCTR_GEMM_CLUSTER", 1) >= 2 && p.m_tiles >= 2 && (b_mn || p.n_tile % 16 == 0))
        p.cluster = 2;
    return p;
}
int plan_splits(int M, int N, int K, bool b_mn) { return make_plan(M, N, K, b_mn, true).splits; }

static int vec_of(const float* p, int64_t pitch) {
    const uintptr_t a = (uintptr_t)p;
    if (pitch % 4 == 0 && a % 16 == 0) return 4;
    if (pitch % 2 == 0 && a % 8 == 0) return 2;
    return 1;
}

int split_weight(const float* w, float* hi, float* lo, int rows, int cols, int pitch, cudaStream_t st) {
    const int64_t total = (int64_t)rows * pitch;
    int64_t blocks = (total + 255) / 256;
    split_weight_kernel<<<(unsigned)(blocks < RLCTR_SMS * 4 ? blocks : RLCTR_SMS * 4), 256, 0, st>>>(w, hi, lo, rows, cols, pitch);
    RLCTR_LAUNCH_CHECK();
    return RLCTR_OK;
}

int gemm(const Operand& A, const Operand& B, float* C, int64_t ldc, const float* bias, int M, int N, int K, int relu,
         bool allow_split, cudaStream_t st, const Epilogue* epi, float* colsum_part) {
    if (!enabled()) return RLCTR_EUNSUPPORTED;
    if (!tma_ok(A.ptr, A.pitch) || !tma_ok(B.ptr, B.pitch) || (B.lo && !tma_ok(B.lo, B.pitch))) return RLCTR_EUNSUPPORTED;
    if (A.lo) return RLCTR_EUNSUPPORTED;
    const Plan p = make_plan(M, N, K, B.mn_major, allow_split, tma_ok(C, ldc), B.lo != nullptr);
    if (p.n_tile > 256 || (B.mn_major && p.n_tile % 32 != 0)) return RLCTR_EUNSUPPORTED;
    CUtensorMap mA, mB, mBlo;
    bool ok = A.mn_major ? make_map(&mA, A.ptr, M, K, A.pitch, 32, true) : make_map(&mA, A.ptr, K, M, A.pitch, BM);
    const int b_box = p.n_tile / p.cluster;
    ok = ok && (B.mn_major ? make_map(&mB, B.ptr, N, K, B.pitch, 32, true) : make_map(&mB, B.ptr, K, N, B.pitch, b_box));
    if (B.lo) ok = ok && (B.mn_major ? make_map(&mBlo, B.lo, N, K, B.pitch, 32, true) : make_map(&mBlo, B.lo, K, N, B.pitch, b_box));
    else mBlo = mB;
    CUtensorMap mC = mA, mM = mA;
    if (p.c_tma) ok = ok && make_map(&mC, C, N, M, ldc, 32);
    if (!ok) return RLCTR_EUNSUPPORTED;
    size_t smem = p.smem;
    int m_tma = 0;
    if (epi && epi->mask_src && p.c_tma && p.splits == 1 && tma_ok(epi->mask_src, epi->mask_ld) && p.smem + M_STAGE_BYTES <= (size_t)(221 * 1024) &&
        env_int("RLCTR_GEMM_M_TMA", 1) != 0 && make_map(&mM, epi->mask_src, N, M, epi->mask_ld, 32)) {
        m_tma = 1;
        smem += M_STAGE_BYTES;
    }
    Args g;
    g.C = C; g.ldc = ldc; g.cvec = vec_of(C, ldc); g.bias = bias;
    g.M = M; g.N = N; g.K = K;
    g.n_tile = p.n_tile; g.m_tiles = p.m_tiles; g.n_tiles = p.n_tiles; g.splits = p.splits; g.kb_per_split = p.kb_per_split;
    g.stages = p.stages;
    g.a_tmem = p.a_tmem; g.acc_stride = p.acc_stride; g.a_col0 = p.a_col0; g.c_tma = p.c_tma; g.m_tma = m_tma;
    g.cluster = p.cluster; g.pair = p.pair;
    g.l2_ahead = env_int("RLCTR_GEMM_L2_AHEAD", 0);
    g.a_mn = A.mn_major ? 1 : 0; g.b_mn = B.mn_major ? 1 : 0; g.b_presplit = B.lo ? 1 : 0; g.relu = relu;
    g.colsum_part = (colsum_part && A.mn_major && !bias) ? colsum_part : nullptr;
    if (colsum_part && !g.colsum_part) return RLCTR_EUNSUPPORTED;
    {
        const char* d = getenv("RLCTR_GEMM_DBG");
        g.dbg = (d && *d) ? reinterpret_cast<long long*>(strtoull(d, nullptr, 16)) : nullptr;
    }
    g.epi = epi ? *epi : Epilogue{};
    if ((g.epi.drop_state || g.epi.mask_src) && p.splits != 1) return RLCTR_EUNSUPPORTED;
    if (g.epi.mask_src) g.epi.mvec = vec_of(g.epi.mask_src, g.epi.mask_ld);
    if (p.pair) RLCTR_CUDA(cudaFuncSetAttribute(gemm3x_tma_kernel<true, false>, cudaFuncAttributeMaxDynamicSharedMemorySize, (int)smem));
    else if (m_tma) RLCTR_CUDA(cudaFuncSetAttribute(gemm3x_tma_kernel<false, true>, cudaFuncAttributeMaxDynamicSharedMemorySize, (int)smem));
    else RLCTR_CUDA(cudaFuncSetAttribute(gemm3x_tma_kernel<false, false>, cudaFuncAttributeMaxDynamicSharedMemorySize, (int)smem));
    const int total = ((p.m_tiles + p.cluster - 1) / p.cluster) * p.n_tiles * p.splits;
    cudaLaunchConfig_t cfg = {};
    cfg.gridDim = dim3((unsigned)(RLCTR_SMS / p.cluster * p.cluster));
    cfg.blockDim = dim3(THREADS);
    cfg.dynamicSmemBytes = smem;
    cfg.stream = st;
    cudaLaunchAttribute attr[1];
    attr[0].id = cudaLaunchAttributeClusterDimension;
    attr[0].val.clusterDim.x = (unsigned)p.cluster;
    attr[0].val.clusterDim.y = 1;
    attr[0].val.clusterDim.z = 1;
    cfg.attrs = attr;
    cfg.numAttrs = 1;
    int max_clusters = RLCTR_SMS / p.cluster;
    if (p.cluster > 1) {
        static int cached_smem = -1, cached = 0;
        if (cached_smem != (int)smem * 2 + p.pair) {
            int n = 0;
            if ((p.pair ? cudaOccupancyMaxActiveClusters(&n, gemm3x_tma_kernel<true, false>, &cfg)
                        : cudaOccupancyMaxActiveClusters(&n, gemm3x_tma_kernel<false, false>, &cfg)) == cudaSuccess && n > 0) cached = n;
            else cached = RLCTR_SMS / p.cluster;
            cached_smem = (int)smem * 2 + p.pair;
        }
        if (cached < max_clusters) max_clusters = cached;
    }
    const int grid = (total < max_clusters ? total : max_clusters) * p.cluster;
    cfg.gridDim = dim3((unsigned)grid);
    if (p.pair) RLCTR_CUDA(cudaLaunchKernelEx(&cfg, gemm3x_tma_kernel<true, false>, mA, mB, mBlo, mC, mM, g));
    else if (m_tma) RLCTR_CUDA(cudaLaunchKernelEx(&cfg, gemm3x_tma_kernel<false, true>, mA, mB, mBlo, mC, mM, g));
    else RLCTR_CUDA(cudaLaunchKernelEx(&cfg, gemm3x_tma_kernel<false, false>, mA, mB, mBlo, mC, mM, g));
    RLCTR_LAUNCH_CHECK();
    return RLCTR_OK;
}

}
}
```

### rl_ctr_prediction_b200/csrc/mlp_tma.cuh

```cuda
#pragma once
#include <cuda_runtime.h>
#include <stdint.h>

namespace rlctr {
namespace tma {

struct Operand {
    const float* ptr;
    const float* lo;
    int64_t pitch;
    bool mn_major;
};

struct Epilogue {
    const uint64_t* drop_state = nullptr;
    uint32_t drop_thresh = 0;
    float drop_scale = 1.f;
    const float* mask_src = nullptr;
    int64_t mask_ld = 0;
    int mvec = 1;
    float mask_scale = 1.f;
};

int enabled();
int plan_splits(int M, int N, int K, bool b_mn);
int split_weight(const float* w, float* hi, float* lo, int rows, int cols, int pitch, cudaStream_t st);
int gemm(const Operand& A, const Operand& B, float* C, int64_t ldc, const float* bias, int M, int N, int K, int relu,
         bool allow_split, cudaStream_t st, const Epilogue* epi = nullptr, float* colsum_part = nullptr);

}
}
```

### rl_ctr_prediction_b200/mlp.py

```python
from __future__ import annotations

import torch
import torch.nn as nn

import os

from . import _lib

FP32_MAX_BATCH = int(os.environ.get("RLCTR_FP32_MAX_BATCH", "1024"))


REUSE_SPLIT = os.environ.get("RLCTR_MLP_REUSE_SPLIT", "1") != "0"


def _fp32_flag(B):
    return _lib.RLCTR_MLP_FP32 if B <= FP32_MAX_BATCH else 0


def _rows_view(x):
    if not x.is_cuda:
        raise _lib.RlctrError("rl_ctr_prediction_b200.mlp.Linear runs on a CUDA (sm_100a) device only")
    K = x.shape[-1]
    if x.dim() == 2 and x.dtype == torch.float32 and x.stride(1) == 1 and x.stride(0) >= K and x.shape[0] > 1:
        return x, x.stride(0)
    x2 = x.reshape(-1, K).contiguous().float()
    return x2, K


def _fwd(lib, x2, ldx, w, bias, relu, drop_p=0.0, rng=None, keep_ws=False):
    B, K = x2.shape
    N = w.shape[0]
    y = torch.empty(B, N, dtype=torch.float32, device=x2.device)
    flags = (_lib.RLCTR_MLP_RELU if relu else 0) | (_lib.RLCTR_MLP_DROPOUT if drop_p > 0.0 else 0) | _fp32_flag(B)
    ws_bytes = lib.rlctr_mlp_ws_bytes(B, K, N)
    ws = torch.empty(ws_bytes, dtype=torch.uint8, device=x2.device)
    _lib.call("rlctr_linear_fwd", lib.rlctr_linear_fwd, x2.data_ptr(), ldx, _lib.ptr(w), _lib.ptr(bias), _lib.ptr(y), B, K, N,
              flags, float(drop_p), _lib.ptr(rng) if drop_p > 0.0 else None, _lib.ptr(ws), ws_bytes, _lib.stream(),
              key=f"rlctr_linear_fwd[{K}x{N}]", meta={"B": B, "K": K, "N": N})
    if drop_p > 0.0:
        _lib.check(lib.rlctr_rng_advance(_lib.ptr(rng), B * N, _lib.stream()), "rlctr_rng_advance")
    if keep_ws:
        return y, (ws if (N > 1 and not (flags & _lib.RLCTR_MLP_FP32)) else None)
    return y


def _bwd(lib, x2, ldx, w, y, gy2, need_dx, need_dw, need_db, relu, gy_scale=1.0, dx_mask=False, dx_scale=1.0, fwd_ws=None):
    B, K = x2.shape
    N = w.shape[0]
    dev = x2.device
    dx = torch.empty(B, K, dtype=torch.float32, device=dev) if need_dx else None
    dw = torch.empty(N, K, dtype=torch.float32, device=dev) if need_dw else None
    db = torch.empty(N, dtype=torch.float32, device=dev) if need_db else None
    ws_bytes = lib.rlctr_mlp_ws_bytes(B, K, N)
    reuse = REUSE_SPLIT and fwd_ws is not None and fwd_ws.numel() >= ws_bytes and not _fp32_flag(B)
    ws = fwd_ws if reuse else torch.empty(ws_bytes, dtype=torch.uint8, device=dev)
    flags = ((_lib.RLCTR_MLP_RELU if relu else 0) | (_lib.RLCTR_MLP_DX_MASK if dx_mask else 0) | _fp32_flag(B) |
             (_lib.RLCTR_MLP_W_PRESPLIT if reuse else 0))
    _lib.call("rlctr_linear_bwd", lib.rlctr_linear_bwd, x2.data_ptr(), ldx, _lib.ptr(w), _lib.ptr(y) if relu else None,
              _lib.ptr(gy2), _lib.ptr(dx), _lib.ptr(dw), _lib.ptr(db), B, K, N, flags, float(gy_scale), float(dx_scale),
              _lib.ptr(ws), ws_bytes, _lib.stream(), key=f"rlctr_linear_bwd[{K}x{N}]",
              meta={"B": B, "K": K, "N": N, "dx": need_dx})
    return dx, dw, db


class _LinearFn(torch.autograd.Function):
    @staticmethod
    def forward(ctx, x, weight, bias, relu):
        lib = _lib.load()
        x2, ldx = _rows_view(x)
        N = weight.shape[0]
        w = weight.detach().contiguous()
        y = _fwd(lib, x2, ldx, w, bias.detach() if bias is not None else None, relu)
        ctx.relu = relu
        ctx.ldx = ldx
        ctx.has_bias = bias is not None
        ctx.save_for_backward(x2, w, y if relu else None)
        ctx.in_shape = x.shape
        return y.reshape(*x.shape[:-1], N)

    @staticmethod
    def backward(ctx, gy):
        lib = _lib.load()
        x2, w, y = ctx.saved_tensors
        B, K = x2.shape
        N = w.shape[0]
        gy2 = gy.reshape(B, N).contiguous().float()
        if ctx.relu:
            gy2 = gy2.clone() if gy2.data_ptr() == gy.data_ptr() else gy2
        need_dx, need_dw, need_db = ctx.needs_input_grad[0], ctx.needs_input_grad[1], ctx.has_bias and ctx.needs_input_grad[2]
        dx, dw, db = _bwd(lib, x2, ctx.ldx, w, y, gy2, need_dx, need_dw, need_db, ctx.relu)
        if dx is not None:
            dx = dx.reshape(ctx.in_shape)
        return dx, dw, db, None


class Linear(nn.Linear):

    def forward(self, x, relu: bool = False):
        return _LinearFn.apply(x, self.weight, self.bias, relu)


BN_FUSED_MAX_BATCH = 1 << 16


class _BnReluFn(torch.autograd.Function):

    @staticmethod
    def forward(ctx, x, weight, bias, running_mean, running_var, momentum, eps, relu):
        lib = _lib.load()
        x2, ldx = _rows_view(x)
        B, N = x2.shape
        dev = x2.device
        y = torch.empty(B, N, dtype=torch.float32, device=dev)
        mean = torch.empty(N, dtype=torch.float32, device=dev)
        invstd = torch.empty(N, dtype=torch.float32, device=dev)
        _lib.call("rlctr_bn_relu_fwd", lib.rlctr_bn_relu_fwd, x2.data_ptr(), ldx, _lib.ptr(weight.detach() if weight is not None else None),
                  _lib.ptr(bias.detach() if bias is not None else None), _lib.ptr(running_mean), _lib.ptr(running_var),
                  float(momentum), float(eps), _lib.ptr(y), N, _lib.ptr(mean), _lib.ptr(invstd), B, N, 1 if relu else 0,
                  _lib.stream(), meta={"B": B, "N": N})
        ctx.save_for_backward(x2, y, weight, mean, invstd)
        ctx.ldx, ctx.relu, ctx.in_shape, ctx.has_bias = ldx, relu, x.shape, bias is not None
        return y.reshape(*x.shape[:-1], N)

    @staticmethod
    def backward(ctx, gy):
        lib = _lib.load()
        x2, y, weight, mean, invstd = ctx.saved_tensors
        B, N = y.shape
        dev = y.device
        g2 = gy.reshape(B, N).contiguous().float()
        dx = torch.empty(B, N, dtype=torch.float32, device=dev) if ctx.needs_input_grad[0] else None
        dgamma = torch.empty(N, dtype=torch.float32, device=dev) if (weight is not None and ctx.needs_input_grad[1]) else None
        dbeta = torch.empty(N, dtype=torch.float32, device=dev) if (ctx.has_bias and ctx.needs_input_grad[2]) else None
        _lib.call("rlctr_bn_relu_bwd", lib.rlctr_bn_relu_bwd, x2.data_ptr(), ctx.ldx, _lib.ptr(y), N, _lib.ptr(g2), N,
                  _lib.ptr(weight.detach() if weight is not None else None), _lib.ptr(mean), _lib.ptr(invstd), _lib.ptr(dx), N,
                  _lib.ptr(dgamma), _lib.ptr(dbeta), B, N, 1 if ctx.relu else 0, _lib.stream(), meta={"B": B, "N": N})
        if dx is not None:
            dx = dx.reshape(ctx.in_shape)
        return dx, dgamma, dbeta, None, None, None, None, None


def bn_relu(bn: nn.BatchNorm1d, x, relu: bool):
    momentum = 0.0 if bn.momentum is None else bn.momentum
    if bn.track_running_stats and bn.num_batches_tracked is not None:
        bn.num_batches_tracked.add_(1)
        if bn.momentum is None:
            momentum = 1.0 / float(bn.num_batches_tracked)
    rm, rv = (bn.running_mean, bn.running_var) if bn.track_running_stats else (None, None)
    return _BnReluFn.apply(x, bn.weight if bn.affine else None, bn.bias if bn.affine else None, rm, rv, momentum, bn.eps, relu)


def apply_bn(bn, x):
    if (type(bn) is nn.BatchNorm1d and bn.training and x.is_cuda and x.dim() == 2 and x.dtype == torch.float32
            and 1 < x.shape[0] <= BN_FUSED_MAX_BATCH):
        return bn_relu(bn, x, False)
    return bn(x)


class _TowerFn(torch.autograd.Function):

    @staticmethod
    def forward(ctx, x, spec, rng, *params):
        lib = _lib.load()
        h, ld = _rows_view(x)
        acts, lds, ws_, fwd_ws = [], [], [], []
        for i, (relu, drop_p, has_bias) in enumerate(spec):
            w = params[2 * i].detach().contiguous()
            b = params[2 * i + 1].detach() if has_bias else None
            acts.append(h)
            lds.append(ld)
            ws_.append(w)
            h, fws = _fwd(lib, h, ld, w, b, relu, drop_p, rng, keep_ws=True)
            fwd_ws.append(fws)
            ld = h.shape[1]
        ctx.spec, ctx.lds = spec, lds
        ctx.fwd_ws = fwd_ws
        ctx.in_shape = x.shape
        ctx.n_layers = len(spec)
        last_relu = spec[-1][0]
        ctx.save_for_backward(*acts, *ws_, *( [h] if last_relu else [] ))
        return h.reshape(*x.shape[:-1], h.shape[1])

    @staticmethod
    def backward(ctx, gy):
        lib = _lib.load()
        L = ctx.n_layers
        saved = ctx.saved_tensors
        acts, ws_ = saved[:L], saved[L:2 * L]
        spec = ctx.spec
        B = acts[0].shape[0]
        g = gy.reshape(B, -1).contiguous().float()
        grads = [None] * (2 * L)
        for i in range(L - 1, -1, -1):
            relu, drop_p, has_bias = spec[i]
            own_mask = relu and i == L - 1
            if own_mask and g.data_ptr() == gy.data_ptr():
                g = g.clone()
            below = spec[i - 1] if i > 0 else None
            dx_mask = below is not None and below[0]
            dx_scale = 1.0 / (1.0 - below[1]) if (below is not None and below[1] > 0.0) else 1.0
            if below is not None and not below[0] and below[1] > 0.0:
                raise _lib.RlctrError("Dropout without a preceding ReLU is not fused; use separate modules")
            need_dx = i > 0 or ctx.needs_input_grad[0]
            need_dw = ctx.needs_input_grad[3 + 2 * i]
            need_db = has_bias and ctx.needs_input_grad[3 + 2 * i + 1]
            gy_scale = 1.0 / (1.0 - drop_p) if (own_mask and drop_p > 0.0) else 1.0
            dx, dw, db = _bwd(lib, acts[i], ctx.lds[i], ws_[i], saved[2 * L] if own_mask else None, g, need_dx, need_dw,
                              need_db, own_mask, gy_scale, dx_mask, dx_scale, fwd_ws=ctx.fwd_ws[i])
            ctx.fwd_ws[i] = None
            grads[2 * i], grads[2 * i + 1] = dw, db
            g = dx
        dx0 = g.reshape(ctx.in_shape) if (g is not None and ctx.needs_input_grad[0]) else None
        return (dx0, None, None, *grads)


class Tower(nn.Sequential):

    def _groups(self):
        mods, i, out = list(self), 0, []
        while i < len(mods):
            if not isinstance(mods[i], Linear):
                return None
            lin, relu, drop = mods[i], False, None
            i += 1
            if i < len(mods) and isinstance(mods[i], nn.ReLU):
                relu = True
                i += 1
            if i < len(mods) and isinstance(mods[i], nn.Dropout):
                if not relu:
                    return None
                drop = mods[i]
                i += 1
            out.append((lin, relu, drop))
        return out

    def _rng_state(self, device):
        st = getattr(self, "_rlctr_rng", None)
        if st is None or st.device != device:
            seed = int(torch.randint(0, 2 ** 62, (1,)).item())
            st = torch.tensor([seed, 0], dtype=torch.int64, device=device)
            self._rlctr_rng = st
        return st

    def forward(self, x):
        groups = self._groups()
        if groups is None or not x.is_cuda:
            return self._forward_modules(x)
        spec, params, any_drop = [], [], False
        for lin, relu, drop in groups:
            p = float(drop.p) if (drop is not None and drop.training and drop.p > 0.0) else 0.0
            any_drop = any_drop or p > 0.0
            spec.append((relu, p, lin.bias is not None))
            params += [lin.weight, lin.bias]
        rng = self._rng_state(x.device) if any_drop else None
        return _TowerFn.apply(x, tuple(spec), rng, *params)

    def _forward_modules(self, x):
        mods = list(self)
        i = 0
        while i < len(mods):
            m = mods[i]
            nxt = mods[i + 1] if i + 1 < len(mods) else None
            if (isinstance(m, Linear) and isinstance(nxt, nn.BatchNorm1d) and not nxt.training and nxt.track_running_stats
                    and not torch.is_grad_enabled() and x.is_cuda):
                scale = nxt.weight / torch.sqrt(nxt.running_var + nxt.eps) if nxt.affine else torch.rsqrt(nxt.running_var + nxt.eps)
                bias0 = m.bias if m.bias is not None else torch.zeros_like(nxt.running_mean)
                shift = (bias0 - nxt.running_mean) * scale + (nxt.bias if nxt.affine else 0.0)
                relu = i + 2 < len(mods) and isinstance(mods[i + 2], nn.ReLU)
                x2, ldx = _rows_view(x)
                y = _fwd(_lib.load(), x2, ldx, (m.weight * scale[:, None]).contiguous(), shift.contiguous(), relu)
                x = y.reshape(*x.shape[:-1], y.shape[1])
                i += 3 if relu else 2
                continue
            if (type(m) is nn.BatchNorm1d and m.training and x.is_cuda and x.dim() == 2 and x.dtype == torch.float32
                    and 1 < x.shape[0] <= BN_FUSED_MAX_BATCH):
                relu = isinstance(nxt, nn.ReLU)
                x = bn_relu(m, x, relu)
                i += 2 if relu else 1
                continue
            if isinstance(m, Linear) and i + 1 < len(mods) and isinstance(mods[i + 1], nn.ReLU):
                x = m(x, relu=True)
                i += 2
            else:
                x = m(x)
                i += 1
        return x
```

### rl_ctr_prediction_b200/p_model.py

```python
from __future__ import annotations

import ctypes as C

import torch
import torch.nn as nn

from . import _lib
from .tables import Geometry, table_struct
from . import mlp as _mlp


class RowsStash:
    __slots__ = ("sorted_ids", "sorted_slots", "n", "dlogit", "sums", "extra", "staged", "fields", "flags", "peer", "stage")

    def __init__(self, **kw):
        for k in self.__slots__:
            setattr(self, k, kw.get(k))


def _check_ids(x: torch.Tensor) -> torch.Tensor:
    if not x.is_cuda:
        raise _lib.RlctrError("rl_ctr_prediction_b200 models run on a CUDA (sm_100a) device only; "
                              "move the features with .to(device) -- there is no CPU fallback")
    if x.dtype != torch.int64:
# ... 284 lines not shown
        return super().zero_grad(set_to_none)


class LR(_TableModel):
    _kind = "lr"

    def __init__(self, feature_nums, output_dim=1, device=None):
        super().__init__()
        assert output_dim == 1
        self.feature_nums = feature_nums
        self._init_table(Geometry.lr(feature_nums), [(0, 1)], device)
        self.bias = nn.Parameter(torch.zeros((output_dim,), device=device))

    def _ref_items(self):
        return [("linear.weight", self._geom.lin_col, 1)]

    def forward(self, x):
        return self._run(x, False, True)[0]


class FM(_TableModel):
    _kind = "fm"
    _fm_term = True

    def __init__(self, feature_nums, latent_dims, output_dim=1, device=None):
        super().__init__()
        assert output_dim == 1
        self.feature_nums, self.latent_dims = feature_nums, int(latent_dims)
        g = Geometry.fm(feature_nums, self.latent_dims)
        self._init_table(g, [(g.lin_col, 1), (g.emb_col, g.dim)], device)
        self.bias = nn.Parameter(torch.zeros((output_dim,), device=device))

    def _ref_items(self):
        g = self._geom
        return [("linear.weight", g.lin_col, 1), ("feature_embedding.weight", g.emb_col, g.dim)]

    def forward(self, x):
        return self._run(x, False, True)[0]


class FFM(_TableModel):
    _kind = "ffm"

    def __init__(self, feature_nums, field_nums, latent_dims, output_dim=1, device=None):
        super().__init__()
        assert output_dim == 1
        self.feature_nums, self.field_nums, self.latent_dims = feature_nums, int(field_nums), int(latent_dims)
        g = Geometry.ffm(feature_nums, self.field_nums, self.latent_dims)
        cols = [(g.lin_col, 1)] + [(g.emb_col + t * self.latent_dims, self.latent_dims) for t in range(self.field_nums)]
        self._init_table(g, cols, device)
        self.bias = nn.Parameter(torch.zeros((output_dim,), device=device))

    def _ref_items(self):
        g, D = self._geom, self.latent_dims
        return [("linear.weight", g.lin_col, 1)] + \
               [(f"field_feature_embeddings.{t}.weight", g.emb_col + t * D, D) for t in range(self.field_nums)]

    def forward(self, x):
        return self._run(x, False, True)[0]


def colocate(models):
    from .colocated import ColocatedCTR
    return ColocatedCTR(models)


def _tower(in_dims: int, device=None) -> nn.Sequential:
    mods, d = [], in_dims
    for width in (300, 200):
        mods += [_mlp.Linear(d, width, device=device), nn.ReLU(), nn.Dropout(p=0.2)]
        d = width
    mods.append(_mlp.Linear(d, 1, device=device))
    return _mlp.Tower(*mods)


class DeepFM(FM):

    def __init__(self, feature_nums, field_nums, latent_dims, output_dim=1, device=None):
        super().__init__(feature_nums, latent_dims, output_dim, device)
        self.field_nums = int(field_nums)
        self.mlp = _tower(self.field_nums * self.latent_dims, device)

    def _tail(self, z, rows):
        return z + self.mlp(rows)

    def logit(self, x):
        return self._tail(*self._run(x, True, False))

    def forward(self, x):
        return torch.sigmoid(self.logit(x))


class _PairDots(torch.autograd.Function):

    @staticmethod
    def forward(ctx, rows, fields, dim):
        lib = _lib.load()
        B, fd = rows.shape
        npair = fields * (fields - 1) // 2
        ld_rows = rows.stride(0) if (rows.stride(1) == 1 and B > 1) else fd
        if not (rows.stride(1) == 1 and (B == 1 or rows.stride(0) >= fd)):
            rows, ld_rows = rows.contiguous(), fd
        pitch = (fd + npair + 3) // 4 * 4
        out = torch.empty(B, pitch, dtype=torch.float32, device=rows.device)
        _lib.call("rlctr_pairdots_fwd", lib.rlctr_pairdots_fwd, rows.data_ptr(), ld_rows, _lib.ptr(out), pitch, B, fields, dim, 0,
                  _lib.stream(), meta={"B": B})
        ctx.save_for_backward(rows)
        ctx.geom = (fields, dim, ld_rows, pitch)
        return out[:, :fd + npair] if pitch != fd + npair else out

    @staticmethod
    def backward(ctx, gout):
        lib = _lib.load()
        (rows,) = ctx.saved_tensors
        fields, dim, ld_rows, pitch = ctx.geom
        B, fd = rows.shape
        gout = gout.contiguous()
        grows = torch.empty(B, fd, dtype=torch.float32, device=rows.device)
        _lib.call("rlctr_pairdots_bwd", lib.rlctr_pairdots_bwd, rows.data_ptr(), ld_rows, _lib.ptr(gout), gout.shape[1],
                  _lib.ptr(grows), fd, B, fields, dim, 0, _lib.stream(), meta={"B": B})
        return grows, None, None


class WideAndDeep(_TableModel):
    _kind = "fm"
    _fm_term = False

    def __init__(self, feature_nums, field_nums, latent_dims, output_dim=1, device=None):
        super().__init__()
        assert output_dim == 1
        self.feature_nums, self.field_nums, self.latent_dims = feature_nums, int(field_nums), int(latent_dims)
        g = Geometry.fm(feature_nums, self.latent_dims)
        self._init_table(g, [(g.lin_col, 1), (g.emb_col, g.dim)], device)
        self.bias = nn.Parameter(torch.zeros((output_dim,), device=device))
        self.mlp = _tower(self.field_nums * self.latent_dims, device)

    def _ref_items(self):
        g = self._geom
        return [("linear.weight", g.lin_col, 1), ("embedding.weight", g.emb_col, g.dim)]

    def _tail(self, z, rows):
        return z + self.mlp(rows)

    def logit(self, x):
        return self._tail(*self._run(x, True, False))

    def forward(self, x):
        return torch.sigmoid(self.logit(x))


class FNN(_TableModel):
    _kind = "fm"
    _fm_term = False

    def __init__(self, feature_nums, field_nums, latent_dims, device=None):
        super().__init__()
        self.feature_nums, self.field_nums, self.latent_dims = feature_nums, int(field_nums), int(latent_dims)
        g = Geometry.fm(feature_nums, self.latent_dims, with_linear=False)
        self._init_table(g, [(g.emb_col, g.dim)], device)
        self.mlp = self._make_tower(device)

    def _make_tower(self, device):
        return _tower(self.field_nums * self.latent_dims, device)

    def _ref_items(self):
        g = self._geom
        return [("feature_embedding.weight", g.emb_col, g.dim)]

    def load_embedding(self, pretrain_params):
        self.flush()
        g = self._geom
        with torch.no_grad():
            self.table.data[:, g.emb_col:g.emb_col + g.dim].copy_(pretrain_params["feature_embedding.weight"])

    def _tower_input(self, rows):
        return rows

    def _tail(self, z, rows):
        return self.mlp(self._tower_input(rows))

    def logit(self, x):
        return self._tail(*self._run(x, True, False))

    def forward(self, x):
        return torch.sigmoid(self.logit(x))


class InnerPNN(FNN):

    def _make_tower(self, device):
        F = self.field_nums
        return _tower(F * self.latent_dims + F * (F - 1) // 2, device)

    def _tower_input(self, rows):
        return _PairDots.apply(rows, self.field_nums, self.latent_dims)


class _FieldSq(torch.autograd.Function):

    @staticmethod
    def forward(ctx, rows, fields, dim):
        lib = _lib.load()
        rows, ld_rows = _mlp._rows_view(rows)
        B, fd = rows.shape
        pitch = (fd + dim + 3) // 4 * 4
        out = torch.empty(B, pitch, dtype=torch.float32, device=rows.device)
        _lib.call("rlctr_fieldsq_fwd", lib.rlctr_fieldsq_fwd, rows.data_ptr(), ld_rows, _lib.ptr(out), pitch, B, fields, dim,
                  _lib.stream(), meta={"B": B})
        ctx.save_for_backward(rows)
        ctx.geom = (fields, dim, ld_rows)
        return out[:, :fd + dim] if pitch != fd + dim else out
    @staticmethod
    def backward(ctx, gout):
        lib = _lib.load()
        (rows,) = ctx.saved_tensors
        fields, dim, ld_rows = ctx.geom
        B, fd = rows.shape
        gout = gout.contiguous()
        grows = torch.empty(B, fd, dtype=torch.float32, device=rows.device)
        _lib.call("rlctr_fieldsq_bwd", lib.rlctr_fieldsq_bwd, rows.data_ptr(), ld_rows, _lib.ptr(gout), gout.shape[1],
                  _lib.ptr(grows), fd, B, fields, dim, _lib.stream(), meta={"B": B})
        return grows, None, None


class OuterPNN(FNN):
# ... 175 lines not shown
```

Measured before the change: 48.56 million.

## Fuse tower output layer and residual add, batch BCE heads, bit-pack ReLU masks

Batches the per-head BCE loss kernels of colocated models into a single multi-head launch (grid y indexes heads). Folds the final 1-wide linear layer of the MLP tower into the previous GEMM epilogue as per-part partial dot products, which a small reduction kernel then sums with the bias and the FM logit add. Dropout now uses a running RNG offset with a single advance call, and ReLU masks are stored as packed bits for the backward pass. The goal is fewer kernel launches and less activation traffic, at the cost of more complex epilogue and autograd plumbing.

```diff
diff --git a/include/rlctr.h b/include/rlctr.h
--- a/include/rlctr.h
+++ b/include/rlctr.h
@@ -122,6 +122,9 @@
 int rlctr_bce_fwd_bwd(const float* logit, const int64_t* labels_i64, const float* labels_f32,
                       float* pctr, float* loss, float* dlogit, float* dbias, void* ws, int64_t batch,
                       rlctr_stream_t stream);
+int rlctr_bce_fwd_bwd_multi(const float* const* logits, const int64_t* labels_i64, const float* labels_f32,
+                            float* const* losses, float* const* dlogits, float* const* dbiases, int32_t heads, void* ws,
+                            int64_t batch, rlctr_stream_t stream);
 int rlctr_sigmoid_bwd(const float* grad_p, const float* pctr, float* dlogit, float* dbias, void* ws,
                       int64_t batch, rlctr_stream_t stream);
 
@@ -239,6 +242,16 @@
 int rlctr_linear_bwd(const float* x, int64_t ldx, const float* w, const float* y, float* gy, float* dx, float* dw,
                      float* db, int64_t batch, int32_t in_dim, int32_t out_dim, int32_t flags, float gy_scale,
                      float dx_scale, void* ws, size_t ws_bytes, rlctr_stream_t stream);
+int rlctr_linear_fwd_ex(const float* x, int64_t ldx, const float* w, const float* bias, float* y, int64_t batch,
+                        int32_t in_dim, int32_t out_dim, int32_t flags, float dropout_p, const uint64_t* rng_state,
+                        uint64_t rng_offset, uint32_t* mask_bits, const float* w_out, float* out_part,
+                        void* ws, size_t ws_bytes, rlctr_stream_t stream);
+int rlctr_linear_bwd_ex(const float* x, int64_t ldx, const float* w, const float* y, float* gy, float* dx, float* dw,
+                        float* db, int64_t batch, int32_t in_dim, int32_t out_dim, int32_t flags, float gy_scale,
+                        float dx_scale, const uint32_t* mask_bits, void* ws, size_t ws_bytes, rlctr_stream_t stream);
+int32_t rlctr_mlp_out_parts(int64_t batch, int32_t in_dim, int32_t out_dim);
+int rlctr_tower_out(const float* out_part, int32_t n_parts, const float* bias, const float* add, float* y, int64_t batch,
+                    rlctr_stream_t stream);
 
 size_t rlctr_bucket_ws_bytes(int64_t n, int32_t world);
 int rlctr_bucket_by_owner(const int64_t* ids, int64_t n, int32_t world, int64_t n_rows, int64_t* send_local,
diff --git a/rl_ctr_prediction_b200/_lib.py b/rl_ctr_prediction_b200/_lib.py
--- a/rl_ctr_prediction_b200/_lib.py
+++ b/rl_ctr_prediction_b200/_lib.py
@@ -90,6 +90,7 @@
     "rlctr_bn_relu_fwd": (C.c_int, [_P, _I64, _P, _P, _P, _P, C.c_float, C.c_float, _P, _I64, _P, _P, _I64, _I32, _I32, _P]),
     "rlctr_bn_relu_bwd": (C.c_int, [_P, _I64, _P, _I64, _P, _I64, _P, _P, _P, _P, _I64, _P, _P, _I64, _I32, _I32, _P]),
     "rlctr_bce_fwd_bwd": (C.c_int, [_P, _P, _P, _P, _P, _P, _P, _P, _I64, _P]),
+    "rlctr_bce_fwd_bwd_multi": (C.c_int, [_P, _P, _P, _P, _P, _P, _I32, _P, _I64, _P]),
     "rlctr_sigmoid_bwd": (C.c_int, [_P, _P, _P, _P, _P, _I64, _P]),
     "rlctr_sort_ws_bytes": (_SZ, [_I64, _I64]),
     "rlctr_sort_ids": (C.c_int, [_P, _I64, _I64, _P, _P, _P, _SZ, _P]),
@@ -124,6 +125,12 @@
     "rlctr_rng_advance": (C.c_int, [_P, C.c_uint64, _P]),
     "rlctr_linear_fwd": (C.c_int, [_P, _I64, _P, _P, _P, _I64, _I32, _I32, _I32, C.c_float, _P, _P, _SZ, _P]),
     "rlctr_linear_bwd": (C.c_int, [_P, _I64, _P, _P, _P, _P, _P, _P, _I64, _I32, _I32, _I32, C.c_float, C.c_float, _P, _SZ, _P]),
+    "rlctr_linear_fwd_ex": (C.c_int, [_P, _I64, _P, _P, _P, _I64, _I32, _I32, _I32, C.c_float, _P, C.c_uint64, _P, _P, _P, _P, _SZ,
+                                      _P]),
+    "rlctr_linear_bwd_ex": (C.c_int, [_P, _I64, _P, _P, _P, _P, _P, _P, _I64, _I32, _I32, _I32, C.c_float, C.c_float, _P, _P, _SZ,
+                                      _P]),
+    "rlctr_mlp_out_parts": (C.c_int32, [_I64, _I32, _I32]),
+    "rlctr_tower_out": (C.c_int, [_P, _I32, _P, _P, _P, _I64, _P]),
     "rlctr_bucket_ws_bytes": (_SZ, [_I64, _I32]),
     "rlctr_bucket_by_owner": (C.c_int, [_P, _I64, _I32, _I64, _P, _P, _P, _P, _P, _SZ, _P]),
 }
diff --git a/rl_ctr_prediction_b200/colocated.py b/rl_ctr_prediction_b200/colocated.py
--- a/rl_ctr_prediction_b200/colocated.py
+++ b/rl_ctr_prediction_b200/colocated.py
@@ -204,16 +204,25 @@
         _lib.call("rlctr_group_fwd", lib.rlctr_group_fwd, _lib.ptr(x), C.byref(t), arr, M, _lib.ptr(sums), 0, B, F, st,
                   key="rlctr_group_fwd[train]", meta=self._meta(B, F))
         losses = torch.empty(M, dtype=torch.float32, device=dev)
+        dls = [torch.empty(B, dtype=torch.float32, device=dev) for _ in range(M)]
+        dbiases = [torch.empty(1, dtype=torch.float32, device=dev) for _ in range(M)]
+        ws = self._reduce_ws(dev)
+        heads = [i for i in range(M) if rows[i] is None]
+        if heads:
+            arr = lambda xs: (C.c_void_p * len(heads))(*xs)
+            wsm = self._ws.get("reduce_multi")
+            if wsm is None or wsm.device != dev:
+                wsm = self._ws["reduce_multi"] = torch.zeros(_lib.RLCTR_GROUP_MAX * _lib.RLCTR_REDUCE_WS_BYTES, dtype=torch.uint8,
+                                                             device=dev)
+            _lib.check(lib.rlctr_bce_fwd_bwd_multi(arr([_lib.ptr(logits[i]) for i in heads]), _lib.ptr(yi), _lib.ptr(yf),
+                                                   arr([losses.data_ptr() + 4 * i for i in heads]), arr([_lib.ptr(dls[i]) for i in heads]),
+                                                   arr([_lib.ptr(dbiases[i]) for i in heads]), len(heads), _lib.ptr(wsm), B, st),
+                       "rlctr_bce_fwd_bwd_multi")
         dlogits, extras = [], []
-        ws = self._reduce_ws(dev)
         for i, m in enumerate(self.members):
-            dl = torch.empty(B, dtype=torch.float32, device=dev)
-            dbias = torch.empty(1, dtype=torch.float32, device=dev)
+            dl, dbias = dls[i], dbiases[i]
             bias = getattr(m, "bias", None)
             if rows[i] is None:
-                _lib.check(lib.rlctr_bce_fwd_bwd(_lib.ptr(logits[i]), _lib.ptr(yi), _lib.ptr(yf), None,
-                                                 losses.data_ptr() + 4 * i, _lib.ptr(dl), _lib.ptr(dbias), _lib.ptr(ws), B, st),
-                           "rlctr_bce_fwd_bwd")
                 extras.append(None)
             else:
                 fd = F * self._cols[i][2]
diff --git a/rl_ctr_prediction_b200/csrc/loss.cu b/rl_ctr_prediction_b200/csrc/loss.cu
--- a/rl_ctr_prediction_b200/csrc/loss.cu
+++ b/rl_ctr_prediction_b200/csrc/loss.cu
@@ -35,10 +35,9 @@
     return is_last;
 }
 
-__global__ void __launch_bounds__(256)
-bce_kernel(const float* __restrict__ logit, const int64_t* __restrict__ yi, const float* __restrict__ yf,
-           float* __restrict__ pctr, float* __restrict__ loss, float* __restrict__ dlogit, float* __restrict__ dbias,
-           void* ws, int64_t batch) {
+__device__ __forceinline__ void bce_head(const float* __restrict__ logit, const int64_t* __restrict__ yi, const float* __restrict__ yf,
+                                         float* __restrict__ pctr, float* __restrict__ loss, float* __restrict__ dlogit,
+                                         float* __restrict__ dbias, void* ws, int64_t batch) {
     __shared__ float sm[8];
     const float ginv = 1.0f / (float)batch;
     float acc = 0.f, dsum = 0.f;
@@ -70,6 +69,24 @@
             *w.counter = 0;
         }
     }
+}
+__global__ void __launch_bounds__(256)
+bce_kernel(const float* __restrict__ logit, const int64_t* __restrict__ yi, const float* __restrict__ yf,
+           float* __restrict__ pctr, float* __restrict__ loss, float* __restrict__ dlogit, float* __restrict__ dbias,
+           void* ws, int64_t batch) {
+    bce_head(logit, yi, yf, pctr, loss, dlogit, dbias, ws, batch);
+}
+struct BceHeads {
+    const float* logit[RLCTR_GROUP_MAX];
+    float* loss[RLCTR_GROUP_MAX];
+    float* dlogit[RLCTR_GROUP_MAX];
+    float* dbias[RLCTR_GROUP_MAX];
+};
+__global__ void __launch_bounds__(256)
+bce_multi_kernel(const BceHeads h, const int64_t* __restrict__ yi, const float* __restrict__ yf, void* ws, int64_t batch) {
+    const int k = blockIdx.y;
+    bce_head(h.logit[k], yi, yf, nullptr, h.loss[k], h.dlogit[k], h.dbias[k],
+             reinterpret_cast<char*>(ws) + (size_t)k * RLCTR_REDUCE_WS_BYTES, batch);
 }
 
 __global__ void __launch_bounds__(256)
@@ -376,6 +393,25 @@
 
 using namespace rlctr;
 
+extern "C" int rlctr_bce_fwd_bwd_multi(const float* const* logits, const int64_t* labels_i64, const float* labels_f32,
+                                       float* const* losses, float* const* dlogits, float* const* dbiases, int32_t heads, void* ws,
+                                       int64_t batch, rlctr_stream_t stream) {
+    if (!logits || !losses || !dlogits || !ws || heads <= 0 || heads > RLCTR_GROUP_MAX || batch <= 0) return RLCTR_EINVAL;
+    if ((labels_i64 == nullptr) == (labels_f32 == nullptr)) return RLCTR_EINVAL;
+    BceHeads h;
+    for (int k = 0; k < heads; ++k) {
+        if (!logits[k]) return RLCTR_EINVAL;
+        h.logit[k] = logits[k];
+        h.loss[k] = losses[k];
+        h.dlogit[k] = dlogits[k];
+        h.dbias[k] = dbiases ? dbiases[k] : nullptr;
+    }
+    bce_multi_kernel<<<dim3((unsigned)red_grid(batch), (unsigned)heads), 256, 0, (cudaStream_t)stream>>>(h, labels_i64, labels_f32, ws,
+                                                                                                       batch);
+    RLCTR_LAUNCH_CHECK();
+    return RLCTR_OK;
+}
+
 extern "C" int rlctr_bce_fwd_bwd(const float* logit, const int64_t* labels_i64, const float* labels_f32, float* pctr,
                                  float* loss, float* dlogit, float* dbias, void* ws, int64_t batch,
                                  rlctr_stream_t stream) {
diff --git a/rl_ctr_prediction_b200/csrc/mlp.cu b/rl_ctr_prediction_b200/csrc/mlp.cu
--- a/rl_ctr_prediction_b200/csrc/mlp.cu
+++ b/rl_ctr_prediction_b200/csrc/mlp.cu
@@ -401,12 +401,33 @@
     }
 }
 __global__ void __launch_bounds__(256)
-dropout_kernel(float* __restrict__ y, int64_t n, const uint64_t* __restrict__ state, uint32_t thresh, float scale) {
-    const uint64_t seed = state[0], ctr = state[1];
+dropout_kernel(float* __restrict__ y, int64_t n, const uint64_t* __restrict__ state, uint64_t offset, uint32_t thresh, float scale) {
+    const uint64_t seed = state[0], ctr = state[1] + offset;
     for (int64_t i = (int64_t)blockIdx.x * blockDim.x + threadIdx.x; i < n; i += (int64_t)gridDim.x * blockDim.x)
         y[i] = dropout_keep(seed, ctr + (uint64_t)i, thresh) ? y[i] * scale : 0.f;
 }
 __global__ void rng_advance_kernel(uint64_t* state, uint64_t delta) { state[1] += delta; }
+__global__ void __launch_bounds__(256)
+mask_bits_kernel(const float* __restrict__ y, int64_t ldy, int64_t rows, int N, uint32_t* __restrict__ bits) {
+    const int64_t total = rows * ((N + 31) / 32);
+    for (int64_t i = (int64_t)blockIdx.x * blockDim.x + threadIdx.x; i < total; i += (int64_t)gridDim.x * blockDim.x) {
+        const int c = (int)(i / rows);
+        const int64_t r = i - (int64_t)c * rows;
+        uint32_t b = 0;
+        for (int j = 0; j < 32 && 32 * c + j < N; ++j) b |= __ldg(y + r * ldy + 32 * c + j) > 0.f ? (1u << j) : 0u;
+        bits[i] = b;
+    }
+}
+__global__ void __launch_bounds__(256)
+tower_out_kernel(const float* __restrict__ part, int n_parts, const float* __restrict__ bias, const float* __restrict__ add,
+                 float* __restrict__ y, int64_t rows) {
+    const float b0 = bias ? __ldg(bias) : 0.f;
+    for (int64_t r = (int64_t)blockIdx.x * blockDim.x + threadIdx.x; r < rows; r += (int64_t)gridDim.x * blockDim.x) {
+        float t = b0;
+        for (int k = 0; k < n_parts; ++k) t += __ldg(part + (int64_t)k * rows + r);
+        y[r] = add ? __ldg(add + r) + t : t;
+    }
+}
 
 __global__ void __launch_bounds__(256)
 gemv_rows_kernel(const float* __restrict__ x, int64_t ldx, const float* __restrict__ w, const float* __restrict__ bias,
@@ -747,33 +768,56 @@
     return RLCTR_OK;
 }
 
-extern "C" int rlctr_linear_fwd(const float* x, int64_t ldx, const float* w, const float* bias, float* y, int64_t batch,
-                                int32_t in_dim, int32_t out_dim, int32_t flags, float dropout_p, const uint64_t* rng_state,
-                                void* ws, size_t ws_bytes, rlctr_stream_t stream) {
+static int launch_gemv(const float* x, int64_t ldx, const float* w, const float* bias, float* y, int64_t batch, int in_dim, int relu,
+                       cudaStream_t st) {
+    if (in_dim % 4 == 0 && in_dim <= 256 && ldx % 4 == 0 && ((uintptr_t)x & 15) == 0 && ((uintptr_t)w & 15) == 0) {
+        const int64_t blocks = (batch + 31) / 32;
+        gemv_rows4_kernel<<<(unsigned)(blocks < RLCTR_SMS * 8 ? blocks : RLCTR_SMS * 8), 256, 0, st>>>(
+            x, ldx, w, bias, y, batch, in_dim / 4, relu);
+    } else {
+        const int64_t blocks = (batch + 7) / 8;
+        gemv_rows_kernel<<<(unsigned)(blocks < RLCTR_SMS * 8 ? blocks : RLCTR_SMS * 8), 256, 0, st>>>(
+            x, ldx, w, bias, y, batch, in_dim, relu);
+    }
+    RLCTR_LAUNCH_CHECK();
+    return RLCTR_OK;
+}
+
+extern "C" int32_t rlctr_mlp_out_parts(int64_t batch, int32_t in_dim, int32_t out_dim) {
+    if (batch <= 0 || batch > 0x7fffffff || in_dim <= 0 || out_dim <= 1) return 1;
+    return tma::plan_out_parts((int)batch, out_dim, in_dim);
+}
+
+extern "C" int rlctr_tower_out(const float* part, int32_t n_parts, const float* bias, const float* add, float* y, int64_t batch,
+                               rlctr_stream_t stream) {
+    if (!part || !y || n_parts <= 0 || batch < 0) return RLCTR_EINVAL;
+    if (batch == 0) return RLCTR_OK;
+    tower_out_kernel<<<grid_elems(batch), 256, 0, (cudaStream_t)stream>>>(part, n_parts, bias, add, y, batch);
+    RLCTR_LAUNCH_CHECK();
+    return RLCTR_OK;
+}
+
+extern "C" int rlctr_linear_fwd_ex(const float* x, int64_t ldx, const float* w, const float* bias, float* y, int64_t batch,
+                                   int32_t in_dim, int32_t out_dim, int32_t flags, float dropout_p, const uint64_t* rng_state,
+                                   uint64_t rng_offset, uint32_t* mask_bits, const float* w_out, float* out_part, void* ws,
+                                   size_t ws_bytes, rlctr_stream_t stream) {
     if (!x || !w || !y || batch < 0 || in_dim <= 0 || out_dim <= 0) return RLCTR_EINVAL;
     if (ldx == 0) ldx = in_dim;
     if (ldx < in_dim) return RLCTR_EINVAL;
     const bool drop = (flags & RLCTR_MLP_DROPOUT) != 0 && dropout_p > 0.f;
     if (drop && (!rng_state || !(dropout_p < 1.f))) return RLCTR_EINVAL;
+    if ((w_out != nullptr) != (out_part != nullptr) || (out_dim == 1 && (w_out || mask_bits))) return RLCTR_EINVAL;
     if (batch == 0) return RLCTR_OK;
     if (batch > 0x7fffffff) return RLCTR_EUNSUPPORTED;
     cudaStream_t st = (cudaStream_t)stream;
     const int relu = (flags & RLCTR_MLP_RELU) ? 1 : 0;
     const uint32_t thresh = dropout_thresh(dropout_p);
     const float dscale = drop ? 1.0f / (1.0f - dropout_p) : 1.f;
-    bool fused_drop = false;
+    bool fused = false;
     int rc = RLCTR_OK;
     if (out_dim == 1) {
-        if (in_dim % 4 == 0 && in_dim <= 256 && ldx % 4 == 0 && ((uintptr_t)x & 15) == 0 && ((uintptr_t)w & 15) == 0) {
-            const int64_t blocks = (batch + 31) / 32;
-            gemv_rows4_kernel<<<(unsigned)(blocks < RLCTR_SMS * 8 ? blocks : RLCTR_SMS * 8), 256, 0, st>>>(
-                x, ldx, w, bias, y, batch, in_dim / 4, relu);
-        } else {
-            const int64_t blocks = (batch + 7) / 8;
-            gemv_rows_kernel<<<(unsigned)(blocks < RLCTR_SMS * 8 ? blocks : RLCTR_SMS * 8), 256, 0, st>>>(
-                x, ldx, w, bias, y, batch, in_dim, relu);
-        }
-        RLCTR_LAUNCH_CHECK();
+        rc = launch_gemv(x, ldx, w, bias, y, batch, in_dim, relu, st);
+        if (rc) return rc;
     } else if (flags & RLCTR_MLP_FP32) {
         rc = simt::gemm(x, ldx, 1, w, in_dim, 1, y, out_dim, bias, (int)batch, out_dim, in_dim, relu, st);
         if (rc) return rc;
@@ -784,10 +828,13 @@
         int src = RLCTR_OK;
         if (split_weights_into(ws, ws_bytes, l, w, in_dim, out_dim, st, &whi, &wlo, &src)) {
             tma::Epilogue epi;
-            if (drop) { epi.drop_state = rng_state; epi.drop_thresh = thresh; epi.drop_scale = dscale; }
+            if (drop) { epi.drop_state = rng_state; epi.drop_offset = rng_offset; epi.drop_thresh = thresh; epi.drop_scale = dscale; }
+            epi.a_bits = mask_bits;
+            epi.out_w = w_out;
+            epi.out_part = out_part;
             rc = tma::gemm(tma::Operand{x, nullptr, ldx, false}, tma::Operand{whi, wlo, l.in_pitch, false}, y, out_dim, bias,
                            (int)batch, out_dim, in_dim, relu, false, st, &epi);
-            if (rc == RLCTR_OK) fused_drop = drop;
+            if (rc == RLCTR_OK) fused = true;
         } else if (src) {
             return src;
         }
@@ -797,17 +844,36 @@
         }
         if (rc) return rc;
     }
-    if (drop && !fused_drop) {
-        const int64_t n = batch * out_dim;
-        dropout_kernel<<<grid_elems(n), 256, 0, st>>>(y, n, rng_state, thresh, dscale);
-        RLCTR_LAUNCH_CHECK();
+    if (!fused) {
+        if (drop) {
+            const int64_t n = batch * out_dim;
+            dropout_kernel<<<grid_elems(n), 256, 0, st>>>(y, n, rng_state, rng_offset, thresh, dscale);
+            RLCTR_LAUNCH_CHECK();
+        }
+        if (mask_bits) {
+            mask_bits_kernel<<<grid_elems(batch * ((in_dim + 31) / 32)), 256, 0, st>>>(x, ldx, batch, in_dim, mask_bits);
+            RLCTR_LAUNCH_CHECK();
+        }
+        if (out_part) {
+            const int parts = rlctr_mlp_out_parts(batch, in_dim, out_dim);
+            if (parts > 1) RLCTR_CUDA(cudaMemsetAsync(out_part + batch, 0, (size_t)(parts - 1) * batch * sizeof(float), st));
+            rc = launch_gemv(y, out_dim, w_out, nullptr, out_part, batch, out_dim, 0, st);
+            if (rc) return rc;
+        }
     }
     return RLCTR_OK;
 }
 
-extern "C" int rlctr_linear_bwd(const float* x, int64_t ldx, const float* w, const float* y, float* gy, float* dx, float* dw,
-                                float* db, int64_t batch, int32_t in_dim, int32_t out_dim, int32_t flags, float gy_scale,
-                                float dx_scale, void* ws, size_t ws_bytes, rlctr_stream_t stream) {
+extern "C" int rlctr_linear_fwd(const float* x, int64_t ldx, const float* w, const float* bias, float* y, int64_t batch,
+                                int32_t in_dim, int32_t out_dim, int32_t flags, float dropout_p, const uint64_t* rng_state,
+                                void* ws, size_t ws_bytes, rlctr_stream_t stream) {
+    return rlctr_linear_fwd_ex(x, ldx, w, bias, y, batch, in_dim, out_dim, flags, dropout_p, rng_state, 0, nullptr, nullptr, nullptr,
+                               ws, ws_bytes, stream);
+}
+
+extern "C" int rlctr_linear_bwd_ex(const float* x, int64_t ldx, const float* w, const float* y, float* gy, float* dx, float* dw,
+                                   float* db, int64_t batch, int32_t in_dim, int32_t out_dim, int32_t flags, float gy_scale,
+                                   float dx_scale, const uint32_t* mask_bits, void* ws, size_t ws_bytes, rlctr_stream_t stream) {
     if (!x || !w || !gy || batch <= 0 || in_dim <= 0 || out_dim <= 0) return RLCTR_EINVAL;
     if (ldx == 0) ldx = in_dim;
     if (ldx < in_dim) return RLCTR_EINVAL;
@@ -880,12 +946,13 @@
         float *whi = nullptr, *wlo = nullptr;
         int rc = RLCTR_OK;
         bool done = false;
+        bool masked = false;
         if (split_weights_into(ws, ws_bytes, l, w, in_dim, out_dim, st, &whi, &wlo, &rc, (flags & RLCTR_MLP_W_PRESPLIT) != 0)) {
             tma::Epilogue epi;
-            if (dx_mask) { epi.mask_src = x; epi.mask_ld = ldx; epi.mask_scale = dx_scale; }
+            if (dx_mask && mask_bits) { epi.mask_bits = mask_bits; epi.mask_scale = dx_scale; }
             rc = tma::gemm(tma::Operand{dy, nullptr, out_dim, false}, tma::Operand{whi, wlo, l.in_pitch, true}, dx, in_dim,
                            nullptr, (int)batch, in_dim, out_dim, 0, false, st, &epi);
-            if (rc == RLCTR_OK) done = true;
+            if (rc == RLCTR_OK) { done = true; masked = epi.mask_bits != nullptr; }
             else if (rc != RLCTR_EUNSUPPORTED) return rc;
         } else if (rc) {
             return rc;
@@ -894,10 +961,10 @@
             GemmPlan p = plan_gemm((int)batch, in_dim, out_dim, false);
             rc = launch_gemm(dy, out_dim, 1, w, 1, in_dim, dx, in_dim, nullptr, (int)batch, in_dim, out_dim, 0, p, st);
             if (rc) return rc;
-            if (dx_mask) {
-                mask_rows_kernel<<<grid_elems(batch * in_dim), 256, 0, st>>>(dx, x, ldx, batch, in_dim, dx_scale);
-                RLCTR_LAUNCH_CHECK();
-            }
+        }
+        if (dx_mask && !masked) {
+            mask_rows_kernel<<<grid_elems(batch * in_dim), 256, 0, st>>>(dx, x, ldx, batch, in_dim, dx_scale);
+            RLCTR_LAUNCH_CHECK();
         }
     }
     bool db_done = false;
@@ -949,3 +1016,10 @@
     }
     return RLCTR_OK;
 }
+
+extern "C" int rlctr_linear_bwd(const float* x, int64_t ldx, const float* w, const float* y, float* gy, float* dx, float* dw,
+                                float* db, int64_t batch, int32_t in_dim, int32_t out_dim, int32_t flags, float gy_scale,
+                                float dx_scale, void* ws, size_t ws_bytes, rlctr_stream_t stream) {
+    return rlctr_linear_bwd_ex(x, ldx, w, y, gy, dx, dw, db, batch, in_dim, out_dim, flags, gy_scale, dx_scale, nullptr, ws, ws_bytes,
+                               stream);
+}
diff --git a/rl_ctr_prediction_b200/csrc/mlp_tma.cu b/rl_ctr_prediction_b200/csrc/mlp_tma.cu
--- a/rl_ctr_prediction_b200/csrc/mlp_tma.cu
+++ b/rl_ctr_prediction_b200/csrc/mlp_tma.cu
@@ -36,7 +36,6 @@
     int cluster;
     int l2_ahead;
     int c_tma;
-    int m_tma;
     long long* dbg;
     float* colsum_part;
     Epilogue epi;
@@ -303,9 +302,10 @@
     }
 }
 
-__device__ __forceinline__ float split_row_to_tmem(uint32_t raw, bool a_mn, int t, uint32_t taddr) {
+__device__ __forceinline__ float split_row_to_tmem(uint32_t raw, bool a_mn, int t, uint32_t taddr, uint32_t* bits = nullptr) {
     uint32_t hi[BK], lo[BK];
     float sum = 0.f;
+    uint32_t b = 0;
     if (!a_mn) {
         const uint32_t row = raw + (uint32_t)t * 128u;
 #pragma unroll
@@ -317,7 +317,11 @@
             hi[4 * c + 2] = __float_as_uint(h.z); hi[4 * c + 3] = __float_as_uint(h.w);
             lo[4 * c] = __float_as_uint(l.x); lo[4 * c + 1] = __float_as_uint(l.y);
             lo[4 * c + 2] = __float_as_uint(l.z); lo[4 * c + 3] = __float_as_uint(l.w);
-        }
+            if (bits)
+                b |= (x.x > 0.f ? 1u : 0u) << (4 * c) | (x.y > 0.f ? 2u : 0u) << (4 * c) | (x.z > 0.f ? 4u : 0u) << (4 * c) |
+                     (x.w > 0.f ? 8u : 0u) << (4 * c);
+        }
+        if (bits) *bits = b;
     } else {
         const int mm = t & 31;
         const uint32_t blk = raw + (uint32_t)(t >> 5) * 4096u + (uint32_t)((mm & 7) << 2);
@@ -370,10 +374,11 @@
     uint64_t drop_seed, drop_base;
     uint32_t drop_thresh;
     float drop_scale;
-    const float* mask_row;
-    int mvec;
+    const float* s_wout;
+    mutable float dot;
+    const uint32_t* mask_row;
+    int64_t M;
     float mask_scale;
-    uint32_t mbuf;
 };
 template <int W>
 __device__ __forceinline__ void epilogue_compute(const EpiCtx& e, const uint32_t* r, int n0, float (&v)[W]) {
@@ -411,21 +416,25 @@
                 v[j] = dropout_keep(e.drop_seed, i0 + (uint64_t)j, e.drop_thresh) ? v[j] * e.drop_scale : 0.f;
         }
     }
-    if (e.mask_row && e.row_ok && !(W == 32 && e.mbuf)) {
-        const float* mr = e.mask_row + n0;
-        if (n0 + W <= e.N && e.mvec == 4) {
-#pragma unroll
-            for (int j = 0; j < W; j += 4) {
-                const float4 x = __ldg(reinterpret_cast<const float4*>(mr + j));
-                v[j] = x.x > 0.f ? v[j] * e.mask_scale : 0.f;
-                v[j + 1] = x.y > 0.f ? v[j + 1] * e.mask_scale : 0.f;
-                v[j + 2] = x.z > 0.f ? v[j + 2] * e.mask_scale : 0.f;
-                v[j + 3] = x.w > 0.f ? v[j + 3] * e.mask_scale : 0.f;
+    if (e.s_wout) {
+        float d = e.dot;
+#pragma unroll
+        for (int j = 0; j < W; ++j) d = fmaf(v[j], e.s_wout[n0 + j], d);
+        e.dot = d;
+    }
+    if (e.mask_row && e.row_ok) {
+        if (W == 32 && !(n0 & 31)) {
+            if (n0 < e.N) {
+                const uint32_t b = __ldg(e.mask_row + (int64_t)(n0 >> 5) * e.M);
+#pragma unroll
+                for (int j = 0; j < W; ++j) v[j] = (b >> j) & 1u ? v[j] * e.mask_scale : 0.f;
             }
         } else {
 #pragma unroll
-            for (int j = 0; j < W; ++j)
-                if (n0 + j < e.N) v[j] = __ldg(mr + j) > 0.f ? v[j] * e.mask_scale : 0.f;
+            for (int j = 0; j < W; ++j) {
+                const int n = n0 + j;
+                if (n < e.N) v[j] = (__ldg(e.mask_row + (int64_t)(n >> 5) * e.M) >> (n & 31)) & 1u ? v[j] * e.mask_scale : 0.f;
+            }
         }
     }
 }
@@ -447,22 +456,10 @@
             if (n0 + j < e.N) dst[j] = v[j];
     }
 }
-template <bool MASK>
 __device__ __forceinline__ void epilogue_stage(const EpiCtx& e, const uint32_t* r, int n0, uint32_t buf, int lane) {
     float v[32];
     epilogue_compute<32>(e, r, n0, v);
     const uint32_t row = buf + (uint32_t)lane * 128u;
-    if (MASK && e.mbuf) {
-        const uint32_t mrow = e.mbuf + (uint32_t)lane * 128u;
-#pragma unroll
-        for (int c = 0; c < 8; ++c) {
-            const uint32_t off = (uint32_t)((c ^ (lane & 7)) << 4);
-            const float4 x = lds128(mrow + off);
-            sts128(row + off, make_float4(x.x > 0.f ? v[4 * c] * e.mask_scale : 0.f, x.y > 0.f ? v[4 * c + 1] * e.mask_scale : 0.f,
-                                          x.z > 0.f ? v[4 * c + 2] * e.mask_scale : 0.f, x.w > 0.f ? v[4 * c + 3] * e.mask_scale : 0.f));
-        }
-        return;
-    }
 #pragma unroll
     for (int c = 0; c < 8; ++c)
         sts128(row + (uint32_t)((c ^ (lane & 7)) << 4), make_float4(v[4 * c], v[4 * c + 1], v[4 * c + 2], v[4 * c + 3]));
@@ -484,41 +481,26 @@
     }
 }
 
-template <bool MASK>
 __device__ __forceinline__ void epilogue_chunk_tma(const EpiCtx& e, const uint32_t* r, int n0, const CUtensorMap* mapC,
                                                    uint32_t stage0, int& buf, int m0, int lane) {
     if (n0 >= e.N) return;
     if (lane == 0) bulk_wait_read<1>();
     __syncwarp();
     const uint32_t sb = stage0 + (uint32_t)buf * 4096u;
-    epilogue_stage<MASK>(e, r, n0, sb, lane);
+    epilogue_stage(e, r, n0, sb, lane);
     fence_proxy_async();
     __syncwarp();
     if (lane == 0) { tma_store_2d(mapC, sb, n0, m0); bulk_commit(); }
     buf ^= 1;
 }
-__device__ __forceinline__ void mask_request(const CUtensorMap* mapM, uint32_t mbuf, uint32_t mbar, int n0, int m0, int lane) {
-    if (lane == 0) {
-        mbar_expect_tx(mbar, 4096u);
-        tma_load_2d(mbuf, mapM, n0, m0, mbar);
-    }
-}
-template <bool MASK>
 __device__ __forceinline__ void epilogue_tile_tma(const EpiCtx& e, uint32_t taddr, int n_base, int n_tile, const CUtensorMap* mapC,
-                                                  uint32_t stage0, int& buf, int m0, int lane, const CUtensorMap* mapM,
-                                                  uint32_t mbar, uint32_t& mphase) {
+                                                  uint32_t stage0, int& buf, int m0, int lane) {
     const int nch = n_tile / 32;
     for (int c = 0; c < nch; ++c) {
         uint32_t ra[32];
         tmem_ld<32>(taddr + (uint32_t)(c * 32), ra);
         tmem_ld_fence<32>(ra);
-        const int n0 = n_base + c * 32;
-        if (MASK && e.mbuf && n0 < e.N) {
-            mbar_wait(mbar, mphase);
-            mphase ^= 1;
-        }
-        epilogue_chunk_tma<MASK>(e, ra, n0, mapC, stage0, buf, m0, lane);
-        if (MASK && e.mbuf && c + 1 < nch && n0 + 32 < e.N) mask_request(mapM, e.mbuf, mbar, n0 + 32, m0, lane);
+        epilogue_chunk_tma(e, ra, n_base + c * 32, mapC, stage0, buf, m0, lane);
     }
     if (n_tile & 31) {
         uint32_t rt[16];
@@ -528,23 +510,24 @@
     }
 }
 
-template <bool PAIR, bool MASK>
+template <bool PAIR>
 __global__ void __launch_bounds__(THREADS, 1)
 gemm3x_tma_kernel(const __grid_constant__ CUtensorMap mapA, const __grid_constant__ CUtensorMap mapB,
-                  const __grid_constant__ CUtensorMap mapBlo, const __grid_constant__ CUtensorMap mapC,
-                  const __grid_constant__ CUtensorMap mapM, const Args g) {
+                  const __grid_constant__ CUtensorMap mapBlo, const __grid_constant__ CUtensorMap mapC, const Args g) {
     extern __shared__ __align__(1024) unsigned char smem_raw[];
     __shared__ __align__(8) uint64_t raw_bar[MAX_STAGES], full_bar[MAX_STAGES], empty_bar[MAX_STAGES];
     __shared__ __align__(8) uint64_t tmem_full_bar[2], tmem_empty_bar[2];
-    __shared__ __align__(8) uint64_t mask_bar[EPI_WARPS];
     __shared__ uint32_t tmem_base_smem;
     __shared__ __align__(16) float s_bias[BIAS_SMEM];
 
     unsigned char* smem = reinterpret_cast<unsigned char*>((reinterpret_cast<uintptr_t>(smem_raw) + 1023) & ~(uintptr_t)1023);
     const int warp = threadIdx.x >> 5, lane = threadIdx.x & 31;
-    const bool bias_in_smem = g.bias != nullptr && g.n_tiles * g.n_tile <= BIAS_SMEM;
+    const int n_total = g.n_tiles * g.n_tile;
+    const bool bias_in_smem = g.bias != nullptr && n_total <= BIAS_SMEM;
     if (bias_in_smem)
-        for (int i = threadIdx.x; i < g.n_tiles * g.n_tile; i += THREADS) s_bias[i] = i < g.N ? __ldg(g.bias + i) : 0.f;
+        for (int i = threadIdx.x; i < n_total; i += THREADS) s_bias[i] = i < g.N ? __ldg(g.bias + i) : 0.f;
+    if (g.epi.out_w)
+        for (int i = threadIdx.x; i < n_total; i += THREADS) s_bias[n_total + i] = i < g.N ? __ldg(g.epi.out_w + i) : 0.f;
     const uint32_t b_bytes = (uint32_t)g.n_tile * (PAIR ? 64u : 128u);
     const uint32_t a_bytes = g.a_tmem ? A_TILE_BYTES : 2 * A_TILE_BYTES;
     const uint32_t stage_bytes = a_bytes + 2 * b_bytes;
@@ -559,7 +542,6 @@
             mbar_init(smem_u32(&full_bar[s]), (uint32_t)(CONV_WARPS * 32 * (PAIR ? 2 : 1)));
             mbar_init(smem_u32(&empty_bar[s]), (uint32_t)(PAIR ? 1 : g.cluster));
         }
-        for (int s = 0; s < EPI_WARPS; ++s) mbar_init(smem_u32(&mask_bar[s]), 1);
         for (int s = 0; s < 2; ++s) {
             mbar_init(smem_u32(&tmem_full_bar[s]), 1);
             mbar_init(smem_u32(&tmem_empty_bar[s]), (uint32_t)(EPI_WARPS * 32 * (PAIR ? 2 : 1)));
@@ -571,7 +553,6 @@
         tma_prefetch_desc(&mapB);
         if (g.b_presplit) tma_prefetch_desc(&mapBlo);
         if (g.c_tma) tma_prefetch_desc(&mapC);
-        if (g.m_tma) tma_prefetch_desc(&mapM);
     }
     if (warp == MMA_WARP) {
         if (PAIR) tmem_alloc2(smem_u32(&tmem_base_smem), TMEM_COLS);
@@ -596,6 +577,7 @@
         uint32_t phase = 0;
         TileWalk w{cluster_id, 0, 0, 0, 0, 0};
         const bool colsum = g.colsum_part != nullptr && g.a_mn;
+        uint32_t* const a_bits = g.splits == 1 ? g.epi.a_bits : nullptr;
         for (; tile_decode(w, g, total_tiles, rank); w.tile += n_clusters) {
             const bool sum_tile = colsum && w.nt == 0;
             float4 acc[BM / 32];
@@ -610,7 +592,10 @@
                 if (g.a_tmem) {
                     tc_fence_after();
                     const uint32_t ta = tmem_base + ((uint32_t)(warp * 32) << 16) + (uint32_t)(g.a_col0 + stage * 2 * BK);
-                    row_sum += split_row_to_tmem(st, g.a_mn != 0, tid, ta);
+                    uint32_t bits;
+                    const bool want_bits = a_bits && w.nt == 0;
+                    row_sum += split_row_to_tmem(st, g.a_mn != 0, tid, ta, want_bits ? &bits : nullptr);
+                    if (want_bits && w.mt * BM + tid < g.M) a_bits[(int64_t)kb * g.M + w.mt * BM + tid] = bits;
                     if (!g.b_presplit) split_tile(st + a_bytes, st + a_bytes + b_bytes, b_bytes, tid);
                     tc_fence_before();
                 } else {
@@ -819,13 +804,9 @@
         int acc = 0, dbg_tile = 0, cbuf = 0;
         const uint32_t cstage = smem_u32(smem + (size_t)g.stages * stage_bytes) + (uint32_t)q * 8192u;
         uint32_t acc_phase = 0;
-        uint32_t mphase = 0;
         TileWalk w{cluster_id, 0, 0, 0, 0, 0};
         for (; tile_decode(w, g, total_tiles, rank); w.tile += n_clusters) {
             const bool empty_split = w.kb1 <= w.kb0;
-            const uint32_t mbuf = (MASK && g.m_tma) ? cstage + (uint32_t)((EPI_WARPS - q) * 8192 + q * 4096) : 0u;
-            if (MASK && mbuf && w.nt * g.n_tile < g.N && g.n_tile >= 32)
-                mask_request(&mapM, mbuf, smem_u32(&mask_bar[q]), w.nt * g.n_tile, w.mt * BM + q * 32, lane);
             mbar_wait(smem_u32(&tmem_full_bar[acc]), acc_phase);
             tc_fence_after();
             if (warp == CONV_WARPS + 2 && lane == 0) DBG_STAMP(dbg_tile * (w.kb1 - w.kb0), 7);
@@ -841,18 +822,19 @@
             e.zero = empty_split;
             e.drop = g.epi.drop_state != nullptr && g.splits == 1;
             e.drop_seed = drop_seed;
-            e.drop_base = drop_ctr + (uint64_t)m * (uint64_t)g.N;
+            e.drop_base = drop_ctr + g.epi.drop_offset + (uint64_t)m * (uint64_t)g.N;
             e.drop_thresh = g.epi.drop_thresh;
             e.drop_scale = g.epi.drop_scale;
-            e.mask_row = (g.epi.mask_src && g.splits == 1) ? g.epi.mask_src + (int64_t)m * g.epi.mask_ld : nullptr;
-            e.mvec = g.epi.mvec;
+            e.M = g.M;
+            e.s_wout = (g.epi.out_w && g.splits == 1) ? s_bias + n_total : nullptr;
+            e.dot = 0.f;
+            e.mask_row = (g.epi.mask_bits && g.splits == 1) ? g.epi.mask_bits + m : nullptr;
             e.mask_scale = g.epi.mask_scale;
-            e.mbuf = mbuf;
             const uint32_t taddr = tmem_base + (uint32_t)(acc * g.acc_stride) + ((uint32_t)(q * 32) << 16);
-            if (g.c_tma) epilogue_tile_tma<MASK>(e, taddr, w.nt * g.n_tile, g.n_tile, &mapC, cstage, cbuf, w.mt * BM + q * 32, lane, &mapM,
-                                           smem_u32(&mask_bar[q]), mphase);
+            if (g.c_tma) epilogue_tile_tma(e, taddr, w.nt * g.n_tile, g.n_tile, &mapC, cstage, cbuf, w.mt * BM + q * 32, lane);
             else if (g.n_tile % 32 == 0) epilogue_tile<32>(e, taddr, w.nt * g.n_tile, g.n_tile);
             else epilogue_tile<16>(e, taddr, w.nt * g.n_tile, g.n_tile);
+            if (e.s_wout && e.row_ok) g.epi.out_part[(int64_t)w.nt * g.M + m] = e.dot;
             tc_fence_before();
             if (warp == CONV_WARPS + 2 && lane == 0) DBG_STAMP(dbg_tile * (w.kb1 - w.kb0) + 1, 7);
             ++dbg_tile;
@@ -936,7 +918,6 @@
     size_t smem;
 };
 constexpr size_t C_STAGE_BYTES = (size_t)EPI_WARPS * 2 * 4096;
-constexpr size_t M_STAGE_BYTES = (size_t)EPI_WARPS * 4096;
 static Plan make_plan(int M, int N, int K, bool b_mn, bool allow_split, bool c_tma_ok = false, bool b_presplit = false) {
     Plan p;
     const int nt_max = env_int("RLCTR_GEMM_NT_MAX", 160);
@@ -981,6 +962,7 @@
     return p;
 }
 int plan_splits(int M, int N, int K, bool b_mn) { return make_plan(M, N, K, b_mn, true).splits; }
+int plan_out_parts(int M, int N, int K) { return make_plan(M, N, K, false, false).n_tiles; }
 
 static int vec_of(const float* p, int64_t pitch) {
     const uintptr_t a = (uintptr_t)p;
@@ -1004,28 +986,23 @@
     if (A.lo) return RLCTR_EUNSUPPORTED;
     const Plan p = make_plan(M, N, K, B.mn_major, allow_split, tma_ok(C, ldc), B.lo != nullptr);
     if (p.n_tile > 256 || (B.mn_major && p.n_tile % 32 != 0)) return RLCTR_EUNSUPPORTED;
+    if (epi && epi->out_w && 2 * p.n_tiles * p.n_tile > BIAS_SMEM) return RLCTR_EUNSUPPORTED;
     CUtensorMap mA, mB, mBlo;
     bool ok = A.mn_major ? make_map(&mA, A.ptr, M, K, A.pitch, 32, true) : make_map(&mA, A.ptr, K, M, A.pitch, BM);
     const int b_box = p.n_tile / p.cluster;
     ok = ok && (B.mn_major ? make_map(&mB, B.ptr, N, K, B.pitch, 32, true) : make_map(&mB, B.ptr, K, N, B.pitch, b_box));
     if (B.lo) ok = ok && (B.mn_major ? make_map(&mBlo, B.lo, N, K, B.pitch, 32, true) : make_map(&mBlo, B.lo, K, N, B.pitch, b_box));
     else mBlo = mB;
-    CUtensorMap mC = mA, mM = mA;
+    CUtensorMap mC = mA;
     if (p.c_tma) ok = ok && make_map(&mC, C, N, M, ldc, 32);
     if (!ok) return RLCTR_EUNSUPPORTED;
-    size_t smem = p.smem;
-    int m_tma = 0;
-    if (epi && epi->mask_src && p.c_tma && p.splits == 1 && tma_ok(epi->mask_src, epi->mask_ld) && p.smem + M_STAGE_BYTES <= (size_t)(221 * 1024) &&
-        env_int("RLCTR_GEMM_M_TMA", 1) != 0 && make_map(&mM, epi->mask_src, N, M, epi->mask_ld, 32)) {
-        m_tma = 1;
-        smem += M_STAGE_BYTES;
-    }
+    const size_t smem = p.smem;
     Args g;
     g.C = C; g.ldc = ldc; g.cvec = vec_of(C, ldc); g.bias = bias;
     g.M = M; g.N = N; g.K = K;
     g.n_tile = p.n_tile; g.m_tiles = p.m_tiles; g.n_tiles = p.n_tiles; g.splits = p.splits; g.kb_per_split = p.kb_per_split;
     g.stages = p.stages;
-    g.a_tmem = p.a_tmem; g.acc_stride = p.acc_stride; g.a_col0 = p.a_col0; g.c_tma = p.c_tma; g.m_tma = m_tma;
+    g.a_tmem = p.a_tmem; g.acc_stride = p.acc_stride; g.a_col0 = p.a_col0; g.c_tma = p.c_tma;
     g.cluster = p.cluster; g.pair = p.pair;
     g.l2_ahead = env_int("RLCTR_GEMM_L2_AHEAD", 0);
     g.a_mn = A.mn_major ? 1 : 0; g.b_mn = B.mn_major ? 1 : 0; g.b_presplit = B.lo ? 1 : 0; g.relu = relu;
@@ -1036,11 +1013,10 @@
         g.dbg = (d && *d) ? reinterpret_cast<long long*>(strtoull(d, nullptr, 16)) : nullptr;
     }
     g.epi = epi ? *epi : Epilogue{};
-    if ((g.epi.drop_state || g.epi.mask_src) && p.splits != 1) return RLCTR_EUNSUPPORTED;
-    if (g.epi.mask_src) g.epi.mvec = vec_of(g.epi.mask_src, g.epi.mask_ld);
-    if (p.pair) RLCTR_CUDA(cudaFuncSetAttribute(gemm3x_tma_kernel<true, false>, cudaFuncAttributeMaxDynamicSharedMemorySize, (int)smem));
-    else if (m_tma) RLCTR_CUDA(cudaFuncSetAttribute(gemm3x_tma_kernel<false, true>, cudaFuncAttributeMaxDynamicSharedMemorySize, (int)smem));
-    else RLCTR_CUDA(cudaFuncSetAttribute(gemm3x_tma_kernel<false, false>, cudaFuncAttributeMaxDynamicSharedMemorySize, (int)smem));
+    if ((g.epi.drop_state || g.epi.mask_bits || g.epi.a_bits || g.epi.out_w) && p.splits != 1) return RLCTR_EUNSUPPORTED;
+    if (g.epi.a_bits && (!p.a_tmem || A.mn_major)) return RLCTR_EUNSUPPORTED;
+    if (p.pair) RLCTR_CUDA(cudaFuncSetAttribute(gemm3x_tma_kernel<true>, cudaFuncAttributeMaxDynamicSharedMemorySize, (int)smem));
+    else RLCTR_CUDA(cudaFuncSetAttribute(gemm3x_tma_kernel<false>, cudaFuncAttributeMaxDynamicSharedMemorySize, (int)smem));
     const int total = ((p.m_tiles + p.cluster - 1) / p.cluster) * p.n_tiles * p.splits;
     cudaLaunchConfig_t cfg = {};
     cfg.gridDim = dim3((unsigned)(RLCTR_SMS / p.cluster * p.cluster));
@@ -1059,8 +1035,8 @@
         static int cached_smem = -1, cached = 0;
         if (cached_smem != (int)smem * 2 + p.pair) {
             int n = 0;
-            if ((p.pair ? cudaOccupancyMaxActiveClusters(&n, gemm3x_tma_kernel<true, false>, &cfg)
-                        : cudaOccupancyMaxActiveClusters(&n, gemm3x_tma_kernel<false, false>, &cfg)) == cudaSuccess && n > 0) cached = n;
+            if ((p.pair ? cudaOccupancyMaxActiveClusters(&n, gemm3x_tma_kernel<true>, &cfg)
+                        : cudaOccupancyMaxActiveClusters(&n, gemm3x_tma_kernel<false>, &cfg)) == cudaSuccess && n > 0) cached = n;
             else cached = RLCTR_SMS / p.cluster;
             cached_smem = (int)smem * 2 + p.pair;
         }
@@ -1068,9 +1044,8 @@
     }
     const int grid = (total < max_clusters ? total : max_clusters) * p.cluster;
     cfg.gridDim = dim3((unsigned)grid);
-    if (p.pair) RLCTR_CUDA(cudaLaunchKernelEx(&cfg, gemm3x_tma_kernel<true, false>, mA, mB, mBlo, mC, mM, g));
-    else if (m_tma) RLCTR_CUDA(cudaLaunchKernelEx(&cfg, gemm3x_tma_kernel<false, true>, mA, mB, mBlo, mC, mM, g));
-    else RLCTR_CUDA(cudaLaunchKernelEx(&cfg, gemm3x_tma_kernel<false, false>, mA, mB, mBlo, mC, mM, g));
+    if (p.pair) RLCTR_CUDA(cudaLaunchKernelEx(&cfg, gemm3x_tma_kernel<true>, mA, mB, mBlo, mC, g));
+    else RLCTR_CUDA(cudaLaunchKernelEx(&cfg, gemm3x_tma_kernel<false>, mA, mB, mBlo, mC, g));
     RLCTR_LAUNCH_CHECK();
     return RLCTR_OK;
 }
diff --git a/rl_ctr_prediction_b200/csrc/mlp_tma.cuh b/rl_ctr_prediction_b200/csrc/mlp_tma.cuh
--- a/rl_ctr_prediction_b200/csrc/mlp_tma.cuh
+++ b/rl_ctr_prediction_b200/csrc/mlp_tma.cuh
@@ -14,16 +14,19 @@
 
 struct Epilogue {
     const uint64_t* drop_state = nullptr;
+    uint64_t drop_offset = 0;
     uint32_t drop_thresh = 0;
     float drop_scale = 1.f;
-    const float* mask_src = nullptr;
-    int64_t mask_ld = 0;
-    int mvec = 1;
+    uint32_t* a_bits = nullptr;
+    const float* out_w = nullptr;
+    float* out_part = nullptr;
+    const uint32_t* mask_bits = nullptr;
     float mask_scale = 1.f;
 };
 
 int enabled();
 int plan_splits(int M, int N, int K, bool b_mn);
+int plan_out_parts(int M, int N, int K);
 int split_weight(const float* w, float* hi, float* lo, int rows, int cols, int pitch, cudaStream_t st);
 int gemm(const Operand& A, const Operand& B, float* C, int64_t ldc, const float* bias, int M, int N, int K, int relu,
          bool allow_split, cudaStream_t st, const Epilogue* epi = nullptr, float* colsum_part = nullptr);
diff --git a/rl_ctr_prediction_b200/mlp.py b/rl_ctr_prediction_b200/mlp.py
--- a/rl_ctr_prediction_b200/mlp.py
+++ b/rl_ctr_prediction_b200/mlp.py
@@ -27,24 +27,25 @@
     return x2, K
 
 
-def _fwd(lib, x2, ldx, w, bias, relu, drop_p=0.0, rng=None, keep_ws=False):
+def _fwd(lib, x2, ldx, w, bias, relu, drop_p=0.0, rng=None, keep_ws=False, rng_offset=None, bits=None, w_out=None, out_part=None):
     B, K = x2.shape
     N = w.shape[0]
     y = torch.empty(B, N, dtype=torch.float32, device=x2.device)
     flags = (_lib.RLCTR_MLP_RELU if relu else 0) | (_lib.RLCTR_MLP_DROPOUT if drop_p > 0.0 else 0) | _fp32_flag(B)
     ws_bytes = lib.rlctr_mlp_ws_bytes(B, K, N)
     ws = torch.empty(ws_bytes, dtype=torch.uint8, device=x2.device)
-    _lib.call("rlctr_linear_fwd", lib.rlctr_linear_fwd, x2.data_ptr(), ldx, _lib.ptr(w), _lib.ptr(bias), _lib.ptr(y), B, K, N,
-              flags, float(drop_p), _lib.ptr(rng) if drop_p > 0.0 else None, _lib.ptr(ws), ws_bytes, _lib.stream(),
-              key=f"rlctr_linear_fwd[{K}x{N}]", meta={"B": B, "K": K, "N": N})
-    if drop_p > 0.0:
+    _lib.call("rlctr_linear_fwd", lib.rlctr_linear_fwd_ex, x2.data_ptr(), ldx, _lib.ptr(w), _lib.ptr(bias), _lib.ptr(y), B, K, N,
+              flags, float(drop_p), _lib.ptr(rng) if drop_p > 0.0 else None, int(rng_offset or 0), _lib.ptr(bits), _lib.ptr(w_out),
+              _lib.ptr(out_part), _lib.ptr(ws), ws_bytes, _lib.stream(), key=f"rlctr_linear_fwd[{K}x{N}]", meta={"B": B, "K": K, "N": N})
+    if drop_p > 0.0 and rng_offset is None:
         _lib.check(lib.rlctr_rng_advance(_lib.ptr(rng), B * N, _lib.stream()), "rlctr_rng_advance")
     if keep_ws:
         return y, (ws if (N > 1 and not (flags & _lib.RLCTR_MLP_FP32)) else None)
     return y
 
 
-def _bwd(lib, x2, ldx, w, y, gy2, need_dx, need_dw, need_db, relu, gy_scale=1.0, dx_mask=False, dx_scale=1.0, fwd_ws=None):
+def _bwd(lib, x2, ldx, w, y, gy2, need_dx, need_dw, need_db, relu, gy_scale=1.0, dx_mask=False, dx_scale=1.0, fwd_ws=None,
+         mask_bits=None):
     B, K = x2.shape
     N = w.shape[0]
     dev = x2.device
@@ -56,9 +57,9 @@
     ws = fwd_ws if reuse else torch.empty(ws_bytes, dtype=torch.uint8, device=dev)
     flags = ((_lib.RLCTR_MLP_RELU if relu else 0) | (_lib.RLCTR_MLP_DX_MASK if dx_mask else 0) | _fp32_flag(B) |
              (_lib.RLCTR_MLP_W_PRESPLIT if reuse else 0))
-    _lib.call("rlctr_linear_bwd", lib.rlctr_linear_bwd, x2.data_ptr(), ldx, _lib.ptr(w), _lib.ptr(y) if relu else None,
+    _lib.call("rlctr_linear_bwd", lib.rlctr_linear_bwd_ex, x2.data_ptr(), ldx, _lib.ptr(w), _lib.ptr(y) if relu else None,
               _lib.ptr(gy2), _lib.ptr(dx), _lib.ptr(dw), _lib.ptr(db), B, K, N, flags, float(gy_scale), float(dx_scale),
-              _lib.ptr(ws), ws_bytes, _lib.stream(), key=f"rlctr_linear_bwd[{K}x{N}]",
+              _lib.ptr(mask_bits) if dx_mask else None, _lib.ptr(ws), ws_bytes, _lib.stream(), key=f"rlctr_linear_bwd[{K}x{N}]",
               meta={"B": B, "K": K, "N": N, "dx": need_dx})
     return dx, dw, db
 
@@ -157,29 +158,64 @@
     return bn(x)
 
 
+def _fused_out(spec, params):
+    return (len(spec) >= 2 and params[-2].shape[0] == 1 and not spec[-1][0] and spec[-1][1] == 0.0 and spec[-2][0]
+            and params[-4].shape[0] > 1)
+
+
 class _TowerFn(torch.autograd.Function):
 
     @staticmethod
-    def forward(ctx, x, spec, rng, *params):
+    def forward(ctx, x, add, spec, rng, *params):
         lib = _lib.load()
         h, ld = _rows_view(x)
-        acts, lds, ws_, fwd_ws = [], [], [], []
+        B = h.shape[0]
+        L = len(spec)
+        fuse = _fused_out(spec, params)
+        acts, lds, ws_, fwd_ws, bits_ = [], [], [], [], []
+        offset, part = 0, None
         for i, (relu, drop_p, has_bias) in enumerate(spec):
             w = params[2 * i].detach().contiguous()
             b = params[2 * i + 1].detach() if has_bias else None
             acts.append(h)
             lds.append(ld)
             ws_.append(w)
-            h, fws = _fwd(lib, h, ld, w, b, relu, drop_p, rng, keep_ws=True)
+            if fuse and i == L - 1:
+                break
+            N, K = w.shape
+            bits = (torch.empty((K + 31) // 32, B, dtype=torch.int32, device=h.device)
+                    if i > 0 and spec[i - 1][0] and N > 1 else None)
+            w_out = None
+            if fuse and i == L - 2:
+                w_out = params[2 * L - 2].detach().reshape(-1).contiguous()
+                part = torch.empty(lib.rlctr_mlp_out_parts(B, w.shape[1], N), B, dtype=torch.float32, device=h.device)
+            h, fws = _fwd(lib, h, ld, w, b, relu, drop_p, rng, keep_ws=True, rng_offset=offset, bits=bits, w_out=w_out,
+                          out_part=part if w_out is not None else None)
+            if drop_p > 0.0:
+                offset += B * N
             fwd_ws.append(fws)
+            bits_.append(bits)
             ld = h.shape[1]
+        if offset:
+            _lib.check(lib.rlctr_rng_advance(_lib.ptr(rng), offset, _lib.stream()), "rlctr_rng_advance")
+        if fuse:
+            fwd_ws.append(None)
+            out = torch.empty(B, 1, dtype=torch.float32, device=h.device)
+            b_out = params[2 * L - 1].detach() if spec[-1][2] else None
+            a = add.detach().reshape(-1).contiguous() if add is not None else None
+            _lib.call("rlctr_tower_out", lib.rlctr_tower_out, _lib.ptr(part), part.shape[0], _lib.ptr(b_out), _lib.ptr(a), _lib.ptr(out),
+                      B, _lib.stream())
+        else:
+            out = h
         ctx.spec, ctx.lds = spec, lds
         ctx.fwd_ws = fwd_ws
+        ctx.bits = bits_
         ctx.in_shape = x.shape
-        ctx.n_layers = len(spec)
+        ctx.add_shape = add.shape if add is not None else None
+        ctx.n_layers = L
         last_relu = spec[-1][0]
         ctx.save_for_backward(*acts, *ws_, *( [h] if last_relu else [] ))
-        return h.reshape(*x.shape[:-1], h.shape[1])
+        return out.reshape(*x.shape[:-1], out.shape[1])
 
     @staticmethod
     def backward(ctx, gy):
@@ -190,6 +226,7 @@
         spec = ctx.spec
         B = acts[0].shape[0]
         g = gy.reshape(B, -1).contiguous().float()
+        dadd = gy.reshape(ctx.add_shape) if (ctx.add_shape is not None and ctx.needs_input_grad[1]) else None
         grads = [None] * (2 * L)
         for i in range(L - 1, -1, -1):
             relu, drop_p, has_bias = spec[i]
@@ -202,16 +239,19 @@
             if below is not None and not below[0] and below[1] > 0.0:
                 raise _lib.RlctrError("Dropout without a preceding ReLU is not fused; use separate modules")
             need_dx = i > 0 or ctx.needs_input_grad[0]
-            need_dw = ctx.needs_input_grad[3 + 2 * i]
-            need_db = has_bias and ctx.needs_input_grad[3 + 2 * i + 1]
+            need_dw = ctx.needs_input_grad[4 + 2 * i]
+            need_db = has_bias and ctx.needs_input_grad[4 + 2 * i + 1]
             gy_scale = 1.0 / (1.0 - drop_p) if (own_mask and drop_p > 0.0) else 1.0
             dx, dw, db = _bwd(lib, acts[i], ctx.lds[i], ws_[i], saved[2 * L] if own_mask else None, g, need_dx, need_dw,
-                              need_db, own_mask, gy_scale, dx_mask, dx_scale, fwd_ws=ctx.fwd_ws[i])
+                              need_db, own_mask, gy_scale, dx_mask, dx_scale, fwd_ws=ctx.fwd_ws[i],
+                              mask_bits=ctx.bits[i] if (dx_mask and i < len(ctx.bits)) else None)
             ctx.fwd_ws[i] = None
+            if i < len(ctx.bits):
+                ctx.bits[i] = None
             grads[2 * i], grads[2 * i + 1] = dw, db
             g = dx
         dx0 = g.reshape(ctx.in_shape) if (g is not None and ctx.needs_input_grad[0]) else None
-        return (dx0, None, None, *grads)
+        return (dx0, dadd, None, None, *grads)
 
 
 class Tower(nn.Sequential):
@@ -242,10 +282,11 @@
             self._rlctr_rng = st
         return st
 
-    def forward(self, x):
+    def forward(self, x, add=None):
         groups = self._groups()
         if groups is None or not x.is_cuda:
-            return self._forward_modules(x)
+            out = self._forward_modules(x)
+            return out if add is None else add + out
         spec, params, any_drop = [], [], False
         for lin, relu, drop in groups:
             p = float(drop.p) if (drop is not None and drop.training and drop.p > 0.0) else 0.0
@@ -253,7 +294,10 @@
             spec.append((relu, p, lin.bias is not None))
             params += [lin.weight, lin.bias]
         rng = self._rng_state(x.device) if any_drop else None
-        return _TowerFn.apply(x, tuple(spec), rng, *params)
+        spec = tuple(spec)
+        if add is not None and not _fused_out(spec, params):
+            return add + _TowerFn.apply(x, None, spec, rng, *params)
+        return _TowerFn.apply(x, add, spec, rng, *params)
 
     def _forward_modules(self, x):
         mods = list(self)
diff --git a/rl_ctr_prediction_b200/p_model.py b/rl_ctr_prediction_b200/p_model.py
--- a/rl_ctr_prediction_b200/p_model.py
+++ b/rl_ctr_prediction_b200/p_model.py
@@ -390,7 +390,7 @@
         self.mlp = _tower(self.field_nums * self.latent_dims, device)
 
     def _tail(self, z, rows):
-        return z + self.mlp(rows)
+        return self.mlp(rows, add=z)
 
     def logit(self, x):
         return self._tail(*self._run(x, True, False))
@@ -448,7 +448,7 @@
         return [("linear.weight", g.lin_col, 1), ("embedding.weight", g.emb_col, g.dim)]
 
     def _tail(self, z, rows):
-        return z + self.mlp(rows)
+        return self.mlp(rows, add=z)
 
     def logit(self, x):
         return self._tail(*self._run(x, True, False))
diff --git a/scratch/tower_glue_profile.py b/scratch/tower_glue_profile.py
--- /dev/null
+++ b/scratch/tower_glue_profile.py
@@ -0,0 +1,67 @@
+import argparse
+import json
+import os
+import sys
+
+import torch
+
+ROOT = os.path.dirname(os.path.dirname(os.path.abspath(__file__)))
+sys.path.insert(0, ROOT)
+
+from rl_ctr_prediction_b200 import colocated, optim, p_model
+
+
+def main():
+    ap = argparse.ArgumentParser()
+    ap.add_argument("--rows", type=int, default=10_000_000)
+    ap.add_argument("--batch", type=int, default=65536)
+    ap.add_argument("--steps", type=int, default=10)
+    ap.add_argument("--out", default=None)
+    a = ap.parse_args()
+    dev = torch.device("cuda:0")
+    F, D, N, B = 15, 10, a.rows, a.batch
+    torch.manual_seed(0)
+    members = [p_model.LR(N, device=dev), p_model.FM(N, D, device=dev), p_model.DeepFM(N, F, D, device=dev)]
+    with torch.no_grad():
+        for m in members:
+            m.table.mul_(0.1)
+            m.train()
+    group = colocated.colocate(members)
+    group.train()
+    opt = optim.Adam(group.parameters(), lr=1e-3, weight_decay=1e-5, mode="lazy")
+    gen = torch.Generator(device=dev).manual_seed(1)
+    per = N // F
+
+    def batch():
+        x = torch.randint(0, per, (B, F), generator=gen, device=dev) + torch.arange(F, device=dev) * per
+        y = (torch.rand(B, generator=gen, device=dev) < 0.05).long()
+        return x, y
+
+    for _ in range(3):
+        group.train_step(*batch(), opt)
+    torch.cuda.synchronize()
+    batches = [batch() for _ in range(a.steps)]
+    with torch.profiler.profile(activities=[torch.profiler.ProfilerActivity.CUDA]) as prof:
+        for x, y in batches:
+            group.train_step(x, y, opt)
+        torch.cuda.synchronize()
+    rows = {}
+    for e in prof.events():
+        if e.device_type == torch.autograd.DeviceType.CUDA:
+            r = rows.setdefault(e.name, [0, 0.0])
+            r[0] += 1
+            r[1] += e.device_time_total if hasattr(e, "device_time_total") else e.cuda_time_total
+    out = {k: {"per_step": v[0] / a.steps, "mean_us": v[1] / v[0]} for k, v in sorted(rows.items(), key=lambda kv: -kv[1][1])}
+    evs = sorted((e for e in prof.events() if e.device_type == torch.autograd.DeviceType.CUDA), key=lambda e: e.time_range.start)
+    per = len(evs) // a.steps
+    last = [(e.name[:90], round(e.time_range.end - e.time_range.start, 2)) for e in evs[-per:]]
+    text = json.dumps({"gpu": torch.cuda.get_device_name(0), "B": B, "rows": N, "steps": a.steps, "kernels": out, "last_step": last},
+                      indent=1)
+    if a.out:
+        with open(a.out, "w") as fh:
+            fh.write(text)
+    print(text)
+
+
+if __name__ == "__main__":
+    main()
```

Result: no change. 48.67 million, median of 6 (+0.2%).
